# lmb-freiburg/locov

Measured on AMD Instinct MI355X. Metric: proposals/sec through LSM ROI-head (1333x800, 1000 prop, 1203-class text bank), higher is better.
Workload: dtype f32 (Res5 GEMM products formed from f16x2 split operands on the f16 matrix pipe, f32 accumulate; error vs f64 <= 1.5 x the f32-MFMA kernel's + 6e-7 and <= 3e-6 on every tested shape, tests/test_gpu_split_gemm.py)

## Files before the change

### include/locov_hip.h

```cpp
#ifndef LOCOV_HIP_H
#define LOCOV_HIP_H

#include <stdint.h>

#ifdef __cplusplus
extern "C" {
#endif

#define LOCOV_ABI_VERSION 8

#define LOCOV_OK 0
#define LOCOV_ERR_INVALID_ARG (-1)
#define LOCOV_ERR_LAUNCH (-2)
#define LOCOV_ERR_UNSUPPORTED (-3)

#define LOCOV_F32 0
#define LOCOV_BF16 1

#define LOCOV_NORM_NONE 0
#define LOCOV_NORM_L2 1
#define LOCOV_NORM_STANDARDIZE 2

#define LOCOV_EPI_RELU 1u
#define LOCOV_GEMM_A_SPLIT 0x1000u
// ... 45 lines not shown
int64_t locov_roi_align_plan_bytes(int64_t R);
int locov_roi_align_from_nhwc_fwd_ex(const float *feat_nhwc, int N, int H, int W, int C,
                                     const float *rois, int64_t R, int pooled_h, int pooled_w,
                                     float spatial_scale, int sampling_ratio, int aligned, int mode,
                                     void *workspace, int64_t workspace_bytes, float *out,
                                     locov_stream_t stream);

int locov_roi_align_nhwc_fwd(const void *feat, int feat_dtype, int N, int H, int W, int C,
                             const float *rois, int64_t R, int pooled_h, int pooled_w,
                             float spatial_scale, int sampling_ratio, int aligned,
                             int bin_stride, int pos_major, void *out, int out_dtype,
                             locov_stream_t stream);

int locov_roi_align_nhwc_ld_fwd(const void *feat, int feat_dtype, int N, int H, int W, int C,
                                const float *rois, int64_t R, int pooled_h, int pooled_w,
                                float spatial_scale, int sampling_ratio, int aligned,
                                int bin_stride, int pos_major, void *out, int64_t out_ld,
                                int out_dtype, locov_stream_t stream);

int locov_roi_align_nhwc_affine_fwd(const void *feat, int feat_dtype, int N, int H, int W, int C,
                                    int64_t feat_ld, const float *rois, int64_t R, int pooled_h,
                                    int pooled_w, float spatial_scale, int sampling_ratio,
                                    int aligned, int bin_stride, int pos_major,
                                    const float *ch_scale, const float *ch_shift, int relu,
                                    void *out, int64_t out_ld, int out_dtype,
                                    locov_stream_t stream);

int locov_spatial_mean_fwd(const float *x, int64_t R, int C, int HW, int channels_last,
                           float *out, locov_stream_t stream);

int locov_gemm_nt_f32(const float *x, int64_t lda, const float *W, const float *scale,
                      const float *shift, const float *residual, float *y, int64_t ldc,
                      int64_t M, int N, int K, unsigned flags, locov_stream_t stream);

int locov_conv3x3_nhwc_f32(const float *x, int64_t R, int H, int W, int Cin, int pos_major,
                           const float *w_packed, const float *scale, const float *shift,
                           const float *residual, float *y, int N, unsigned flags,
                           locov_stream_t stream);

int locov_pack_conv3x3_weight(const float *w, int N, int Cin, void *out, int out_dtype,
                              locov_stream_t stream);

int64_t locov_winograd_workspace_bytes(int64_t R, int Cin, int N);

int locov_winograd_pack_weight(const float *w, int N, int Cin, float *U, locov_stream_t stream);

int locov_winograd_conv3x3_f32(const float *x, int64_t R, int Cin, const float *U,
                               const float *scale, const float *shift, float *y, int64_t ldy,
                               int N, unsigned flags, void *workspace, int64_t workspace_bytes,
                               locov_stream_t stream);

int locov_winograd_conv3x3_f32_split(const float *x, int64_t R, int Cin, const void *U_split,
                                     float u_scale, float v_scale, const float *scale,
                                     const float *shift, float *y, int64_t ldy, int N, unsigned flags,
                                     void *workspace, int64_t workspace_bytes, unsigned *overflow,
                                     locov_stream_t stream);

int locov_gemm_nt_batched_f32(const float *x, int64_t lda, int64_t stride_x, const float *W,
                              int64_t stride_w, float *y, int64_t ldc, int64_t stride_y,
                              int64_t M, int N, int K, int batch, locov_stream_t stream);

int locov_token_attention_fwd(const float *sim, int64_t R, int Ttot, const int *tok_off,
                              const int *num_tok, int K1, int Tmax, float temperature,
                              int cosine, int hardmax, const float *gmin, float *scores,
                              float *att, locov_stream_t stream);

int locov_token_attention_bwd(const float *sim, int64_t R, int Ttot, const int *tok_off,
                              const int *num_tok, int K1, int Tmax, float temperature,
                              int cosine, int hardmax, const float *gmin, const float *grad_scores,
                              const float *grad_att, float *grad_sim, locov_stream_t stream);

int locov_gemm_nt_bf16(const uint16_t *x, int64_t lda, const uint16_t *W, const float *scale,
                       const float *shift, const float *residual, float *y, int64_t ldc,
                       int64_t M, int N, int K, unsigned flags, locov_stream_t stream);

int locov_conv3x3_nhwc_bf16(const uint16_t *x, int64_t R, int H, int W, int Cin, int pos_major,
                            const uint16_t *w_packed, const float *scale, const float *shift,
                            const float *residual, float *y, int N, unsigned flags,
                            locov_stream_t stream);

int locov_split_f16x2_pack(const float *w, int64_t rows, int K, int64_t ld, float w_scale, void *out,
                           unsigned *overflow, locov_stream_t stream);

int locov_gemm_nt_f32_split(const float *x, int64_t lda, const void *W_split, const float *scale,
                            const float *shift, const float *residual, float *y, int64_t ldc,
                            int64_t M, int N, int K, unsigned flags, float x_scale, float w_scale,
                            unsigned *overflow, locov_stream_t stream);

int locov_gemm_segmean_supported(int64_t lda, int64_t M, int N, int K, int seg, unsigned flags);
int64_t locov_gemm_segmean_workspace_bytes(int64_t M, int N);
int locov_gemm_nt_f32_split_segmean(const float *x, int64_t lda, const void *W_split, const float *scale,
                                    const float *shift, const float *residual, float *out, int64_t M,
                                    int N, int K, int seg, unsigned flags, float x_scale, float w_scale,
                                    void *workspace, int64_t workspace_bytes, unsigned *overflow,
                                    locov_stream_t stream);

int locov_gemm_nt_batched_f32_split(const float *x, int64_t lda, int64_t stride_x, const void *W_split,
                                    int64_t stride_w, float *y, int64_t ldc, int64_t stride_y,
                                    int64_t M, int N, int K, int batch, float x_scale, float w_scale,
                                    unsigned *overflow, locov_stream_t stream);

int locov_gemm_timing_enable(int on);
int locov_gemm_timing_read(int cls, int64_t *launches, double *ms, double *flops);
int locov_gemm_timing_read_ex(int cls, int64_t *launches, double *ms, double *flops, double *bytes);

int locov_frozen_bn_fold(const float *weight, const float *bias, const float *running_mean,
                         const float *running_var, float eps, int C, float *scale, float *shift,
                         locov_stream_t stream);

int locov_rownorm_fwd(const float *x, int64_t R, int D, int mode, float eps, float *y,
                      locov_stream_t stream);

int locov_rownorm_bwd(const float *x, const float *grad_y, int64_t R, int D, int mode, float eps,
                      float *grad_x, locov_stream_t stream);

int locov_f32_to_bf16(const float *x, int64_t n, uint16_t *y, locov_stream_t stream);

int locov_sim_gemm_bf16(const uint16_t *emb, const uint16_t *bank, int64_t R, int D, int K1,
                        float *logits, int64_t ldc, locov_stream_t stream);

#define LOCOV_LABEL_MAX_IMAGES 64
#define LOCOV_LABEL_MAX_THRESHOLDS 6
int locov_label_proposals(const float *boxes, const int *prop_offsets, const float *gt_boxes, const int64_t *gt_classes,
                          const int *gt_offsets, int n_images, const float *thr_lo, const float *thr_hi, const int *thr_label,
                          int n_thresholds, int64_t num_classes, const double *rnd, int64_t *gt_index, int64_t *labels,
                          double *key_pos, double *key_neg, int64_t *rows, locov_stream_t stream);

int locov_sample_proposals(const double *key_pos, const double *key_neg, const int64_t *labels, const int64_t *gt_index,
                           const int64_t *rows, const float *boxes, const float *gt_boxes, const float *field,
                           const int *prop_offsets, const int *gt_offsets, int n_images, int budget, int max_pos,
                           int64_t num_classes, int64_t *picked, float *out_boxes, int64_t *out_classes, float *out_gt_boxes,
                           int64_t *out_fg, float *rois, float *field_out, locov_stream_t stream);

int locov_box_reg_loss(const float *proposal_boxes, const float *gt_boxes, const float *pred_deltas, int64_t ld,
                       const int64_t *gt_classes, int64_t R, int64_t num_classes, float wx, float wy, float ww, float wh,
                       float smooth_l1_beta, float *loss, float *dpred, locov_stream_t stream);

int64_t locov_nms_workspace_bytes(int64_t K);

int locov_nms_sorted(const float *boxes_sorted, int64_t K, float iou_threshold, void *workspace,
                     unsigned char *keep, int *num_keep, locov_stream_t stream);

#define LOCOV_DETECT_MAX_CANDIDATES 8192
#define LOCOV_DETECT_FLAG_NONFINITE 1
#define LOCOV_DETECT_FLAG_OVERFLOW 2
int64_t locov_detect_postprocess_workspace_bytes(int64_t R, int n_images);

int locov_detect_postprocess(const float *probs, int64_t ld_probs, int num_classes, const float *deltas, const float *proposal_boxes,
                             const int *row_offsets, const float *image_hw, int n_images, float wx, float wy, float ww, float wh,
                             float scale_clamp, float score_thresh, float nms_thresh, int topk, void *workspace, int64_t workspace_bytes,
                             float *out_boxes, float *out_scores, int64_t *out_classes, int64_t *out_rows, int *counts_and_flags,
                             locov_stream_t stream);

int64_t locov_detect_postprocess_wide_workspace_bytes(const int *row_offsets, int n_images, int num_classes, int per_class_above);

int locov_detect_postprocess_wide(const float *probs, int64_t ld_probs, int num_classes, const float *deltas, const float *proposal_boxes,
                                  const int *row_offsets, const float *image_hw, int n_images, float wx, float wy, float ww, float wh,
                                  float scale_clamp, float score_thresh, float nms_thresh, int topk, int per_class_above, void *workspace,
                                  int64_t workspace_bytes, float *out_boxes, float *out_scores, int64_t *out_classes, int64_t *out_rows,
                                  int *counts_and_flags, locov_stream_t stream);

int locov_grounding_fwd(const float *S, int B, int T, int NR, const float *caption_mask,
                        const float *region_mask, float temperature, float *cost_w2r,
                        float *cost_r2w, locov_stream_t stream);

int locov_grounding_bwd(const float *S, int B, int T, int NR, const float *caption_mask,
                        const float *region_mask, float temperature, const float *grad_w2r,
                        const float *grad_r2w, float *grad_S, locov_stream_t stream);

#define LOCOV_GROUNDING_CE_MAX_B 64
int locov_grounding_ce_fwd(const float *cost_w2r, const float *cost_r2w, const float *caption_mask, const float *region_mask, int B,
                           int T, int NR, float *out8, locov_stream_t stream);
int locov_grounding_ce_bwd(const float *cost_w2r, const float *cost_r2w, const float *caption_mask, const float *region_mask, int B,
                           int T, int NR, const float *g_w2r_caption, const float *g_w2r_image, const float *g_r2w_caption,
                           const float *g_r2w_image, float *dcost_w2r, float *dcost_r2w, locov_stream_t stream);

int locov_grounding_ce_dist_fwd(const float *cost_w2r, const float *cost_r2w, const float *caption_mask, const float *region_mask, int B,
                                int T, int NR, float *out8, float *pw_w2r, float *pw_r2w, locov_stream_t stream);
int locov_grounding_ce_dist_bwd(const float *cost_w2r, const float *cost_r2w, const float *caption_mask, const float *region_mask, int B,
                                int T, int NR, const float *g_w2r_caption, const float *g_w2r_image, const float *g_r2w_caption,
                                const float *g_r2w_image, const float *g_pw_w2r, const float *g_pw_r2w, float *dcost_w2r, float *dcost_r2w,
                                locov_stream_t stream);

#define LOCOV_DISTILL_KD 0
#define LOCOV_DISTILL_JS 1
#define LOCOV_DISTILL_MSE 2
#define LOCOV_DISTILL_MAX_B 64
int locov_distill_loss_fwd(const float *trans, const float *w2r, const float *r2w, int B, int kind, int transformer_teacher,
                           float temperature, float loss_weight, float *loss, locov_stream_t stream);
int locov_distill_loss_bwd(const float *trans, const float *w2r, const float *r2w, int B, int kind, int transformer_teacher,
                           float temperature, float loss_weight, const float *grad_loss, float *grad_trans, float *grad_w2r,
                           float *grad_r2w, locov_stream_t stream);

int64_t locov_pool_fc_bwd_workspace_bytes(int64_t R, int C5, int D);
int locov_pool_fc_bwd(const float *x, int64_t R, int C5, const float *emb_w, int D, const float *bbox_w,
                      const float *grad_emb, const float *grad_deltas, float *grad_x, float *grad_emb_w,
                      float *grad_emb_b, float *grad_bbox_w, float *grad_bbox_b, void *workspace,
                      int64_t workspace_bytes, locov_stream_t stream);
int64_t locov_sim_gemm_bwd_workspace_bytes(int64_t R, int D, int K1);
int locov_sim_gemm_bwd(const float *grad_logits, const float *emb, const float *bank, int64_t R, int D, int K1,
                       float *grad_emb, float *grad_bank, void *workspace, int64_t workspace_bytes,
                       locov_stream_t stream);

int locov_box_head_fwd(const float *x, int64_t R, int C5, int HW, int channels_last,
                       const float *emb_w, const float *emb_b, const float *bbox_w,
                       const float *bbox_b, const float *bank, const uint16_t *bank_bf16,
                       int D, int K1, int norm_mode, int sim_dtype, float *pooled,
                       float *deltas, float *emb, uint16_t *emb_bf16, float *logits,
                       locov_stream_t stream);

int locov_gemm_nt_f32_ex(const float *x, int64_t lda, const float *W, int64_t ldb, const float *scale,
                         const float *shift, const float *residual, const float *mask, float *y, int64_t ldc,
                         int64_t M, int N, int K, unsigned flags, locov_stream_t stream);

int locov_conv3x3_nhwc_f32_ex(const float *x, int64_t R, int H, int W, int Cin, int pos_major,
                              const float *w_packed, const float *scale, const float *shift,
                              const float *residual, const float *mask, float *y, int N, unsigned flags,
                              locov_stream_t stream);

int locov_winograd_conv3x3_f32_ex(const float *x, int64_t R, int Cin, const float *U, const float *scale,
                                  const float *shift, const float *mask, float *y, int64_t ldy, int N,
                                  unsigned flags, void *workspace, int64_t workspace_bytes,
                                  locov_stream_t stream);

int64_t locov_gemm_tn_workspace_bytes(int64_t M, int N, int K, int batch);
int locov_gemm_tn_f32(const float *a, int64_t lda, int64_t stride_a, const float *b, int64_t ldb,
                      int64_t stride_b, float *out, int64_t ldo, int64_t stride_o, int64_t M, int N, int K,
                      int batch, const float *row_scale, void *workspace, int64_t workspace_bytes,
                      locov_stream_t stream);

int locov_split_scale_from_amax(const float *x, int64_t n, float target_log2, float *scale_out,
                                locov_stream_t stream);
#define LOCOV_AMAX_BOUND_MAX 4
int locov_amax_bound(const float *const *xs, const int64_t *ns, const float *muls, int count, float *slot,
                     locov_stream_t stream);
int locov_split_scale_from_amax_zeroed(const float *x, int64_t n, float target_log2, float *scale_out,
                                       locov_stream_t stream);
int locov_gemm_nt_f32_split_ex(const float *x, int64_t lda, const void *W_split, const float *scale,
                               const float *shift, const float *residual, const float *mask, float *y,
                               int64_t ldc, int64_t M, int N, int K, unsigned flags, float x_scale,
                               const float *x_scale_dev, float w_scale, unsigned *overflow,
                               float *amax_out, locov_stream_t stream);
int locov_gemm_tn_f32_split(const float *a, int64_t lda, int64_t stride_a, const float *b, int64_t ldb,
                            int64_t stride_b, float *out, int64_t ldo, int64_t stride_o, int64_t M, int N,
                            int K, int batch, const float *row_scale, const float *a_scale_dev,
                            float b_scale, unsigned *overflow, void *workspace, int64_t workspace_bytes,
                            locov_stream_t stream);
int locov_winograd_conv3x3_f32_split_ex(const float *x, int64_t R, int Cin, const void *U_split, float u_scale,
                                        float v_scale, int v_scale_auto, const float *scale, const float *shift,
                                        const float *mask, float *y, int64_t ldy, int N, unsigned flags,
                                        float y_split_scale, void *workspace, int64_t workspace_bytes,
                                        unsigned *overflow, float *amax_out, locov_stream_t stream);
int locov_winograd_wgrad_f32_split(const float *x, const float *g, int64_t R, int Cin, int N, unsigned flags,
                                   const float *row_scale, float *dw, unsigned *overflow, void *workspace,
                                   int64_t workspace_bytes, locov_stream_t stream);
int locov_winograd_wgrad_f32_split_v(const float *v_split, const float *g, int64_t R, int Cin, int N, unsigned flags,
                                     const float *row_scale, float *dw, unsigned *overflow, void *workspace,
                                     int64_t workspace_bytes, locov_stream_t stream);
int locov_gemm_tn_f32_split_b(const float *a, int64_t lda, int64_t stride_a, const float *b_split, int64_t ldb,
                              int64_t stride_b, float *out, int64_t ldo, int64_t stride_o, int64_t M, int N,
                              int K, int batch, const float *row_scale, const float *a_scale_dev,
                              float b_scale, unsigned *overflow, void *workspace, int64_t workspace_bytes,
                              locov_stream_t stream);
int64_t locov_conv1x1_winograd_workspace_bytes(int64_t R, int C, int N);
int64_t locov_conv1x1_winograd_workspace_bytes_for(int64_t R, int K, int C, int N, int64_t ldx);
int64_t locov_roi_align_winograd_workspace_bytes(int64_t R, int C, int N);
int locov_roi_align_winograd_conv3x3_f32_split(const float *feat_nhwc, int Nimg, int H, int W, int C, int64_t feat_ld,
                                               const float *rois, int64_t R, int pooled, float spatial_scale,
                                               int sampling_ratio, int aligned, const float *scale1, const float *shift1,
                                               const void *U_split, float u_scale, float v_scale, const float *scale2,
                                               const float *shift2, float *y, int64_t ldy, int N, unsigned flags,
                                               float y_split_scale, void *workspace, int64_t workspace_bytes,
                                               unsigned *overflow, locov_stream_t stream);
int locov_conv1x1_winograd_conv3x3_f32_split(const float *x_split, int64_t ldx, int K, float x_scale, const void *W1_split,
                                             float w1_scale, const float *scale1, const float *shift1, int64_t R, int C,
                                             const void *U_split, float u_scale, float v_scale, const float *scale2,
                                             const float *shift2, float *y, int64_t ldy, int N, unsigned flags,
                                             float y_split_scale, void *workspace, int64_t workspace_bytes,
                                             unsigned *overflow, locov_stream_t stream);

int64_t locov_winograd_wgrad_workspace_bytes(int64_t R, int Cin, int N);
int locov_winograd_wgrad_f32(const float *x, const float *g, int64_t R, int Cin, int N, unsigned flags,
                             const float *row_scale, float *dw, void *workspace, int64_t workspace_bytes,
                             locov_stream_t stream);

#define LOCOV_WEIGHT_PREP_MAX_JOBS 32
enum {
    LOCOV_PREP_PLAIN = 0,
    LOCOV_PREP_TRANSPOSE = 1,
    LOCOV_PREP_IM2COL = 2,
    LOCOV_PREP_IM2COL_FLIP = 3,
    LOCOV_PREP_WINO = 4,
    LOCOV_PREP_WINO_FLIP = 5
};
typedef struct locov_weight_prep_job {
    const float *w;
    const float *row_scale;
    void *out;
    float scale;
    int kind, N, K;
} locov_weight_prep_job;
int locov_res5_weight_prep(const locov_weight_prep_job *jobs, int n_jobs, unsigned *overflow, locov_stream_t stream);

int locov_weight_transpose_scale(const float *w, int N, int K, const float *row_scale, float *out,
                                 locov_stream_t stream);
int locov_conv3x3_weight_flip(const float *w, int N, int Cin, const float *row_scale, float *out,
                              locov_stream_t stream);
int locov_im2col3x3_nhwc(const float *x, int64_t R, int H, int W, int C, float *col, locov_stream_t stream);
int locov_conv3x3_wgrad_unpack(const float *dw_packed, int N, int Cin, const float *row_scale, float *dw,
                               locov_stream_t stream);
int locov_relu_mask(const float *g, const float *act, int64_t n, float *out, float *amax_out, locov_stream_t stream);
#define LOCOV_ZERO_LIST_MAX 24
int locov_zero_if_raised(float *const *tensors, const int64_t *counts, int n_tensors, const unsigned *flag,
                         locov_stream_t stream);

int locov_spatial_mean_bwd(const float *g, const float *act, int64_t R, int C, int HW, float *out,
                           float *amax_out, locov_stream_t stream);
int locov_rows_stride2(const float *src, int N, int H, int W, int C, int forward, float *dst,
                       locov_stream_t stream);
int locov_roi_align_nhwc_bwd(const float *grad_rows, int64_t grad_ld, int N, int H, int W, int C,
                             const float *rois, int64_t R, int pooled_h, int pooled_w, float spatial_scale,
                             int sampling_ratio, int aligned, int bin_stride, int pos_major, float *grad_feat,
                             locov_stream_t stream);

#define LOCOV_REGIONS_MAX_B 64
#define LOCOV_REGIONS_MAX_CANDIDATES 4096
#define LOCOV_REGIONS_GRID 0
#define LOCOV_REGIONS_GRID_ALL 1
#define LOCOV_REGIONS_BOXES 2
#define LOCOV_REGIONS_ROWS 0
#define LOCOV_REGIONS_NCHW 1
int locov_regions_select(const double *keys, int mode, int B, const int *count_host, const int *ext_a_host,
                         const int *ext_b_host, int grid_w, const float *const *boxes_host, int n, int limit, int mask_w,
                         int mvm_w, int64_t *indices, int *src_row, int *inv, uint8_t *mask, float *loc, float *mvm,
                         locov_stream_t stream);
int locov_regions_gather_fwd(const float *src, int layout, int64_t ld, int B, int n, int C, int64_t hw, const int *src_row,
                             float *out, locov_stream_t stream);
int locov_regions_gather_bwd(const float *grad_out, int layout, int64_t ld, int64_t rows, int C, int64_t hw, const int *inv,
                             float *grad_src, locov_stream_t stream);

#ifdef __cplusplus
}
#endif
#endif
```

### locov_amd/_lib.py

```python
from __future__ import annotations

import ctypes
import os
from ctypes import c_char_p, c_float, c_int, c_int64, c_uint, c_void_p, POINTER

HERE = os.path.dirname(os.path.abspath(__file__))
LIB_PATH = os.environ.get("LOCOV_HIP_LIB") or os.path.join(HERE, "liblocov_hip.so")

OK = 0
F32, BF16 = 0, 1
NORM_NONE, NORM_L2, NORM_STANDARDIZE = 0, 1, 2
EPI_RELU = 1
WINO_OUT_ROI_MAJOR = 0x100
WINO_IN_ROI_MAJOR = 0x200
SEGMEAN_RES_ROI_MAJOR = 0x400
GEMM_A_SPLIT = 0x1000
EPI_OUT_SPLIT = 0x2000
EPI_RES_SPLIT = 0x4000
MAX_LEVELS = 8
ZERO_LIST_MAX = 24
LABEL_MAX_IMAGES, LABEL_MAX_THRESHOLDS, SAMPLE_MAX_PROPOSALS = 64, 6, 4096
ABI_VERSION = 8
DETECT_MAX_CANDIDATES, DETECT_FLAG_NONFINITE, DETECT_FLAG_OVERFLOW = 8192, 1, 2
DISTILL_KD, DISTILL_JS, DISTILL_MSE, DISTILL_MAX_B = 0, 1, 2, 64
REGIONS_MAX_B, REGIONS_MAX_CANDIDATES = 64, 4096
REGIONS_GRID, REGIONS_GRID_ALL, REGIONS_BOXES = 0, 1, 2
REGIONS_ROWS, REGIONS_NCHW = 0, 1

_p = c_void_p

WEIGHT_PREP_MAX_JOBS = 32
AMAX_BOUND_MAX = 4
PREP_PLAIN, PREP_TRANSPOSE, PREP_IM2COL, PREP_IM2COL_FLIP, PREP_WINO, PREP_WINO_FLIP = range(6)


class WeightPrepJob(ctypes.Structure):
    _fields_ = [("w", c_void_p), ("row_scale", c_void_p), ("out", c_void_p), ("scale", c_float), ("kind", c_int), ("N", c_int), ("K", c_int)]


SIGNATURES = {
    "locov_abi_version": (c_int, []),
    "locov_last_error": (c_char_p, []),
    "locov_launch_count": (c_int64, []),
    "locov_device_info": (c_int, [POINTER(c_int), POINTER(c_int), POINTER(c_int)]),
    "locov_level_assign": (c_int, [_p, c_int64, c_int, c_int, c_int, c_int, _p, _p]),
    "locov_roi_align_fwd": (c_int, [_p, c_int, c_int, c_int, c_int, _p, c_int64, c_int, c_int, c_float,
                                    c_int, c_int, _p, _p]),
    "locov_roi_align_bwd": (c_int, [_p, c_int, c_int, c_int, c_int, _p, c_int64, c_int, c_int, c_float,
                                    c_int, c_int, _p, _p]),
    "locov_roi_align_levels_fwd": (c_int, [POINTER(c_void_p), POINTER(c_int), POINTER(c_int), POINTER(c_float),
                                           c_int, c_int, c_int, _p, _p, c_int64, c_int, c_int, c_int, c_int,
                                           _p, _p]),
    "locov_nchw_to_nhwc": (c_int, [_p, c_int, c_int, c_int, c_int, _p, c_int, _p]),
    "locov_roi_align_nhwc_fwd": (c_int, [_p, c_int, c_int, c_int, c_int, c_int, _p, c_int64, c_int, c_int,
                                         c_float, c_int, c_int, c_int, c_int, _p, c_int, _p]),
    "locov_roi_align_nhwc_ld_fwd": (c_int, [_p, c_int, c_int, c_int, c_int, c_int, _p, c_int64, c_int, c_int,
                                            c_float, c_int, c_int, c_int, c_int, _p, c_int64, c_int, _p]),
    "locov_roi_align_nhwc_affine_fwd": (c_int, [_p, c_int, c_int, c_int, c_int, c_int, c_int64, _p, c_int64, c_int, c_int,
                                                c_float, c_int, c_int, c_int, c_int, _p, _p, c_int, _p, c_int64, c_int, _p]),
    "locov_roi_align_from_nhwc_fwd": (c_int, [_p, c_int, c_int, c_int, c_int, _p, c_int64, c_int, c_int, c_float,
                                              c_int, c_int, _p, _p]),
    "locov_roi_align_plan_bytes": (c_int64, [c_int64]),
    "locov_roi_align_from_nhwc_fwd_ex": (c_int, [_p, c_int, c_int, c_int, c_int, _p, c_int64, c_int, c_int, c_float,
                                                 c_int, c_int, c_int, _p, c_int64, _p, _p]),
    "locov_spatial_mean_fwd": (c_int, [_p, c_int64, c_int, c_int, c_int, _p, _p]),
    "locov_gemm_nt_f32": (c_int, [_p, c_int64, _p, _p, _p, _p, _p, c_int64, c_int64, c_int, c_int, c_uint, _p]),
    "locov_conv3x3_nhwc_f32": (c_int, [_p, c_int64, c_int, c_int, c_int, c_int, _p, _p, _p, _p, _p, c_int, c_uint,
                                       _p]),
    "locov_pack_conv3x3_weight": (c_int, [_p, c_int, c_int, _p, c_int, _p]),
    "locov_winograd_workspace_bytes": (c_int64, [c_int64, c_int, c_int]),
    "locov_winograd_pack_weight": (c_int, [_p, c_int, c_int, _p, _p]),
    "locov_winograd_conv3x3_f32": (c_int, [_p, c_int64, c_int, _p, _p, _p, _p, c_int64, c_int, c_uint, _p, c_int64, _p]),
    "locov_winograd_conv3x3_f32_split": (c_int, [_p, c_int64, c_int, _p, c_float, c_float, _p, _p, _p, c_int64, c_int, c_uint,
                                                 _p, c_int64, _p, _p]),
    "locov_gemm_nt_batched_f32": (c_int, [_p, c_int64, c_int64, _p, c_int64, _p, c_int64, c_int64, c_int64, c_int,
                                          c_int, c_int, _p]),
    "locov_gemm_timing_enable": (c_int, [c_int]),
    "locov_gemm_timing_read": (c_int, [c_int, _p, _p, _p]),
    "locov_gemm_timing_read_ex": (c_int, [c_int, _p, _p, _p, _p]),
    "locov_frozen_bn_fold": (c_int, [_p, _p, _p, _p, c_float, c_int, _p, _p, _p]),
    "locov_label_proposals": (c_int, [_p, POINTER(c_int), _p, _p, POINTER(c_int), c_int, POINTER(c_float), POINTER(c_float),
                                      POINTER(c_int), c_int, c_int64, _p, _p, _p, _p, _p, _p, _p]),
    "locov_sample_proposals": (c_int, [_p, _p, _p, _p, _p, _p, _p, _p, POINTER(c_int), POINTER(c_int), c_int, c_int, c_int, c_int64,
                                       _p, _p, _p, _p, _p, _p, _p, _p]),
    "locov_box_reg_loss": (c_int, [_p, _p, _p, c_int64, _p, c_int64, c_int64, c_float, c_float, c_float, c_float, c_float, _p, _p, _p]),
    "locov_grounding_ce_fwd": (c_int, [_p, _p, _p, _p, c_int, c_int, c_int, _p, _p]),
    "locov_grounding_ce_bwd": (c_int, [_p, _p, _p, _p, c_int, c_int, c_int, _p, _p, _p, _p, _p, _p, _p]),
    "locov_grounding_ce_dist_fwd": (c_int, [_p, _p, _p, _p, c_int, c_int, c_int, _p, _p, _p, _p]),
    "locov_grounding_ce_dist_bwd": (c_int, [_p, _p, _p, _p, c_int, c_int, c_int, _p, _p, _p, _p, _p, _p, _p, _p, _p]),
    "locov_distill_loss_fwd": (c_int, [_p, _p, _p, c_int, c_int, c_int, c_float, c_float, _p, _p]),
    "locov_distill_loss_bwd": (c_int, [_p, _p, _p, c_int, c_int, c_int, c_float, c_float, _p, _p, _p, _p, _p]),
    "locov_nms_workspace_bytes": (c_int64, [c_int64]),
    "locov_nms_sorted": (c_int, [_p, c_int64, c_float, _p, _p, _p, _p]),
    "locov_detect_postprocess_workspace_bytes": (c_int64, [c_int64, c_int]),
    "locov_detect_postprocess": (c_int, [_p, c_int64, c_int, _p, _p, POINTER(c_int), POINTER(c_float), c_int, c_float, c_float, c_float,
                                         c_float, c_float, c_float, c_float, c_int, _p, c_int64, _p, _p, _p, _p, _p, _p]),
    "locov_detect_postprocess_wide_workspace_bytes": (c_int64, [POINTER(c_int), c_int, c_int, c_int]),
    "locov_detect_postprocess_wide": (c_int, [_p, c_int64, c_int, _p, _p, POINTER(c_int), POINTER(c_float), c_int, c_float, c_float, c_float,
                                              c_float, c_float, c_float, c_float, c_int, c_int, _p, c_int64, _p, _p, _p, _p, _p, _p]),
    "locov_grounding_fwd": (c_int, [_p, c_int, c_int, c_int, _p, _p, c_float, _p, _p, _p]),
    "locov_grounding_bwd": (c_int, [_p, c_int, c_int, c_int, _p, _p, c_float, _p, _p, _p, _p]),
    "locov_token_attention_fwd": (c_int, [_p, c_int64, c_int, _p, _p, c_int, c_int, c_float, c_int, c_int, _p, _p, _p, _p]),
    "locov_token_attention_bwd": (c_int, [_p, c_int64, c_int, _p, _p, c_int, c_int, c_float, c_int, c_int, _p, _p, _p, _p, _p]),
    "locov_rownorm_fwd": (c_int, [_p, c_int64, c_int, c_int, c_float, _p, _p]),
    "locov_rownorm_bwd": (c_int, [_p, _p, c_int64, c_int, c_int, c_float, _p, _p]),
    "locov_pool_fc_bwd_workspace_bytes": (c_int64, [c_int64, c_int, c_int]),
    "locov_pool_fc_bwd": (c_int, [_p, c_int64, c_int, _p, c_int, _p, _p, _p, _p, _p, _p, _p, _p, _p, c_int64, _p]),
    "locov_sim_gemm_bwd_workspace_bytes": (c_int64, [c_int64, c_int, c_int]),
    "locov_sim_gemm_bwd": (c_int, [_p, _p, _p, c_int64, c_int, c_int, _p, _p, _p, c_int64, _p]),
    "locov_f32_to_bf16": (c_int, [_p, c_int64, _p, _p]),
    "locov_gemm_nt_bf16": (c_int, [_p, c_int64, _p, _p, _p, _p, _p, c_int64, c_int64, c_int, c_int, c_uint, _p]),
    "locov_conv3x3_nhwc_bf16": (c_int, [_p, c_int64, c_int, c_int, c_int, c_int, _p, _p, _p, _p, _p, c_int, c_uint, _p]),
    "locov_split_f16x2_pack": (c_int, [_p, c_int64, c_int, c_int64, c_float, _p, _p, _p]),
    "locov_gemm_nt_f32_split": (c_int, [_p, c_int64, _p, _p, _p, _p, _p, c_int64, c_int64, c_int, c_int, c_uint, c_float,
                                        c_float, _p, _p]),
    "locov_gemm_segmean_supported": (c_int, [c_int64, c_int64, c_int, c_int, c_int, c_uint]),
    "locov_gemm_segmean_workspace_bytes": (c_int64, [c_int64, c_int]),
    "locov_gemm_nt_f32_split_segmean": (c_int, [_p, c_int64, _p, _p, _p, _p, _p, c_int64, c_int, c_int, c_int, c_uint, c_float,
                                                c_float, _p, c_int64, _p, _p]),
    "locov_gemm_nt_batched_f32_split": (c_int, [_p, c_int64, c_int64, _p, c_int64, _p, c_int64, c_int64, c_int64, c_int,
                                                c_int, c_int, c_float, c_float, _p, _p]),
    "locov_sim_gemm_bf16": (c_int, [_p, _p, c_int64, c_int, c_int, _p, c_int64, _p]),
    "locov_gemm_nt_f32_ex": (c_int, [_p, c_int64, _p, c_int64, _p, _p, _p, _p, _p, c_int64, c_int64, c_int, c_int, c_uint, _p]),
    "locov_conv3x3_nhwc_f32_ex": (c_int, [_p, c_int64, c_int, c_int, c_int, c_int, _p, _p, _p, _p, _p, _p, c_int, c_uint, _p]),
    "locov_winograd_conv3x3_f32_ex": (c_int, [_p, c_int64, c_int, _p, _p, _p, _p, _p, c_int64, c_int, c_uint, _p, c_int64, _p]),
    "locov_gemm_tn_workspace_bytes": (c_int64, [c_int64, c_int, c_int, c_int]),
    "locov_gemm_tn_f32": (c_int, [_p, c_int64, c_int64, _p, c_int64, c_int64, _p, c_int64, c_int64, c_int64, c_int, c_int, c_int,
                                  _p, _p, c_int64, _p]),
    "locov_split_scale_from_amax": (c_int, [_p, c_int64, c_float, _p, _p]),
    "locov_amax_bound": (c_int, [POINTER(c_void_p), POINTER(c_int64), POINTER(c_float), c_int, _p, _p]),
    "locov_split_scale_from_amax_zeroed": (c_int, [_p, c_int64, c_float, _p, _p]),
    "locov_gemm_nt_f32_split_ex": (c_int, [_p, c_int64, _p, _p, _p, _p, _p, _p, c_int64, c_int64, c_int, c_int, c_uint, c_float, _p,
                                           c_float, _p, _p, _p]),
    "locov_gemm_tn_f32_split": (c_int, [_p, c_int64, c_int64, _p, c_int64, c_int64, _p, c_int64, c_int64, c_int64, c_int, c_int, c_int,
                                        _p, _p, c_float, _p, _p, c_int64, _p]),
    "locov_gemm_tn_f32_split_b": (c_int, [_p, c_int64, c_int64, _p, c_int64, c_int64, _p, c_int64, c_int64, c_int64, c_int, c_int, c_int,
                                        _p, _p, c_float, _p, _p, c_int64, _p]),
    "locov_winograd_conv3x3_f32_split_ex": (c_int, [_p, c_int64, c_int, _p, c_float, c_float, c_int, _p, _p, _p, _p, c_int64, c_int,
                                                    c_uint, c_float, _p, c_int64, _p, _p, _p]),
    "locov_winograd_wgrad_f32_split": (c_int, [_p, _p, c_int64, c_int, c_int, c_uint, _p, _p, _p, _p, c_int64, _p]),
    "locov_winograd_wgrad_f32_split_v": (c_int, [_p, _p, c_int64, c_int, c_int, c_uint, _p, _p, _p, _p, c_int64, _p]),
    "locov_conv1x1_winograd_workspace_bytes": (c_int64, [c_int64, c_int, c_int]),
    "locov_conv1x1_winograd_workspace_bytes_for": (c_int64, [c_int64, c_int, c_int, c_int, c_int64]),
    "locov_roi_align_winograd_workspace_bytes": (c_int64, [c_int64, c_int, c_int]),
    "locov_roi_align_winograd_conv3x3_f32_split": (c_int, [_p, c_int, c_int, c_int, c_int, c_int64, _p, c_int64, c_int, c_float, c_int, c_int,
                                                           _p, _p, _p, c_float, c_float, _p, _p, _p, c_int64, c_int, c_uint, c_float, _p, c_int64,
                                                           _p, _p]),
    "locov_conv1x1_winograd_conv3x3_f32_split": (c_int, [_p, c_int64, c_int, c_float, _p, c_float, _p, _p, c_int64, c_int, _p, c_float, c_float,
                                                         _p, _p, _p, c_int64, c_int, c_uint, c_float, _p, c_int64, _p, _p]),
    "locov_winograd_wgrad_workspace_bytes": (c_int64, [c_int64, c_int, c_int]),
    "locov_winograd_wgrad_f32": (c_int, [_p, _p, c_int64, c_int, c_int, c_uint, _p, _p, _p, c_int64, _p]),
    "locov_res5_weight_prep": (c_int, [POINTER(WeightPrepJob), c_int, _p, _p]),
    "locov_weight_transpose_scale": (c_int, [_p, c_int, c_int, _p, _p, _p]),
    "locov_conv3x3_weight_flip": (c_int, [_p, c_int, c_int, _p, _p, _p]),
    "locov_im2col3x3_nhwc": (c_int, [_p, c_int64, c_int, c_int, c_int, _p, _p]),
    "locov_conv3x3_wgrad_unpack": (c_int, [_p, c_int, c_int, _p, _p, _p]),
    "locov_relu_mask": (c_int, [_p, _p, c_int64, _p, _p, _p]),
    "locov_zero_if_raised": (c_int, [POINTER(c_void_p), POINTER(c_int64), c_int, _p, _p]),
    "locov_spatial_mean_bwd": (c_int, [_p, _p, c_int64, c_int, c_int, _p, _p, _p]),
    "locov_rows_stride2": (c_int, [_p, c_int, c_int, c_int, c_int, c_int, _p, _p]),
    "locov_roi_align_nhwc_bwd": (c_int, [_p, c_int64, c_int, c_int, c_int, c_int, _p, c_int64, c_int, c_int, c_float, c_int, c_int,
                                         c_int, c_int, _p, _p]),
    "locov_box_head_fwd": (c_int, [_p, c_int64, c_int, c_int, c_int, _p, _p, _p, _p, _p, _p, c_int, c_int,
                                   c_int, c_int, _p, _p, _p, _p, _p, _p]),
    "locov_regions_select": (c_int, [_p, c_int, c_int, POINTER(c_int), POINTER(c_int), POINTER(c_int), c_int, POINTER(c_void_p), c_int, c_int,
                                     c_int, c_int, _p, _p, _p, _p, _p, _p, _p]),
    "locov_regions_gather_fwd": (c_int, [_p, c_int, c_int64, c_int, c_int, c_int, c_int64, _p, _p, _p]),
    "locov_regions_gather_bwd": (c_int, [_p, c_int, c_int64, c_int64, c_int, c_int64, _p, _p, _p]),
}

_lib = None


class LocovError(RuntimeError):
    pass


def load() -> ctypes.CDLL:
    global _lib
    if _lib is not None:
        return _lib
    if not os.path.exists(LIB_PATH):
        raise LocovError(
            f"{LIB_PATH} not found: build it with `python -m locov_amd.build` "
            "(or __graft_entry__.build()).  The LSM ROI-head path has no fallback.")
    lib = ctypes.CDLL(LIB_PATH)
    for name, (restype, argtypes) in SIGNATURES.items():
        try:
            fn = getattr(lib, name)
        except AttributeError as e:
            raise LocovError(f"{LIB_PATH} does not export {name}") from e
        fn.restype = restype
        fn.argtypes = argtypes
    if lib.locov_abi_version() != ABI_VERSION:
        raise LocovError(f"ABI version mismatch: library {lib.locov_abi_version()} != binding {ABI_VERSION}")
    _lib = lib
    return lib


def check(rc: int, what: str = "") -> None:
    if rc != OK:
        msg = load().locov_last_error()
        raise LocovError(f"{what or 'liblocov_hip'} failed (code {rc}): {msg.decode() if msg else ''}")
```

### locov_amd/csrc/gemm_nt.h

```cpp
#pragma once
#include "common.h"

namespace locov {

struct Epilogue {
    const float *scale;
    const float *shift;
    const float *residual;
    unsigned flags;
    const float *mask;
    float *amax_out;
};

__device__ __forceinline__ void split_scale_of(const float *slot, float &s, float &inv)
{
    s = slot[0];
    inv = slot[1];
    if (s == 0.f) {
        const float amax = __uint_as_float(reinterpret_cast<const unsigned *>(slot)[2]);
        s = 1.f;
        if (amax > 0.f && amax < 3.0e38f) {
            int e;
            frexpf(amax, &e);
            s = ldexpf(1.f, 13 - e);
        }
        inv = 1.f / s;
    }
}

__device__ __forceinline__ void amax_fold(float *slot, float m)
{
#pragma unroll
    for (int o = 32; o > 0; o >>= 1) m = fmaxf(m, __shfl_xor(m, o));
    if ((threadIdx.x & 63) == 0 && m > 0.f) {
        unsigned *w = reinterpret_cast<unsigned *>(slot) + 2;
        const unsigned bits = __float_as_uint(m);
        if (bits > __hip_atomic_load(w, __ATOMIC_RELAXED, __HIP_MEMORY_SCOPE_AGENT)) atomicMax(w, bits);
    }
}

struct ConvGeom {
    int H, W, Cin, R, group;
};

struct Batch {
    int count;
    int64_t sa, sb, sc;
};

template <typename T, typename TOut>
int launch_gemm_nt(const T *A, int64_t lda, const T *B, int64_t ldb, TOut *C, int64_t ldc, int64_t M, int N, int K,
                   const Epilogue &epi, hipStream_t s, const char *what, const ConvGeom &cg = ConvGeom{0, 0, 0, 0, 0},
                   const Batch &bt = Batch{1, 0, 0, 0});

int timing_begin(hipStream_t s, int cls, double flops, double bytes = 0.0);
void timing_end(int idx, hipStream_t s);

int launch_gemm_split(const float *A, int64_t lda, const void *Wsplit, float *C, int64_t ldc, int64_t M, int N, int K,
                      const Epilogue &epi, float a_scale, float w_scale, hipStream_t s, const char *what,
                      const Batch &bt = Batch{1, 0, 0, 0}, unsigned *overflow = nullptr, const float *a_scale_dev = nullptr);

bool gemm_split_big_applicable(int64_t lda, int64_t ldc, int64_t M, int N, int K, const Epilogue &epi, const Batch &bt,
                               const float *a_scale_dev);
int launch_gemm_split_big(const float *A, int64_t lda, const void *Wsplit, float *C, int64_t ldc, int64_t M, int N, int K,
                          const Epilogue &epi, float a_scale, float w_scale, hipStream_t s, const char *what, const Batch &bt,
                          unsigned *overflow);

bool gemm_split_big_segmean_applicable(int64_t lda, int64_t M, int N, int K, const Epilogue &epi, int seg);
int64_t gemm_split_big_segmean_workspace_bytes(int64_t M, int N);
int launch_gemm_split_big_segmean(const float *A, int64_t lda, const void *Wsplit, int64_t M, int N, int K, const Epilogue &epi, int seg,
                                  float a_scale, float w_scale, float *partial, float *out, hipStream_t s, const char *what, unsigned *overflow);

bool gemm_split_big_wino_applicable(int64_t lda, int64_t M, int N, int K, const Epilogue &epi);
int launch_gemm_split_big_wino(const float *A, int64_t lda, const void *Wsplit, int64_t M, int N, int K, const Epilogue &epi, float a_scale,
                               float w_scale, float *V, float v_scale, hipStream_t s, const char *what, unsigned *overflow);

bool roi_align_nhwc_wino_applicable(int C, int64_t R);
int launch_roi_align_nhwc_wino(const float *feat, int N, int H, int W, int C, int64_t feat_ld, const float *rois, int64_t R, int pooled,
                               float spatial_scale, int sampling_ratio, int aligned, const float *ch_scale, const float *ch_shift, int relu,
                               float *V, float v_scale, unsigned *overflow, hipStream_t s);

int launch_gemm_tn(const float *A, int64_t lda, int64_t sa, const float *B, int64_t ldb, int64_t sb, float *out, int64_t ldo,
                   int64_t so, int64_t M, int N, int K, int batch, const float *row_scale, float *ws, int64_t ws_bytes,
                   hipStream_t s, const char *what);
int64_t gemm_tn_workspace_bytes(int64_t M, int N, int K, int batch);
int launch_gemm_tn_split(const float *A, int64_t lda, int64_t sa, const float *B, int64_t ldb, int64_t sb, float *out, int64_t ldo,
                         int64_t so, int64_t M, int N, int K, int batch, const float *row_scale, const float *a_scale_dev, float b_scale,
                         unsigned *overflow, float *ws, int64_t ws_bytes, hipStream_t s, const char *what, bool b_split = false);

}
```

### locov_amd/csrc/gemm_tn.hip

```cpp
#include "gemm_nt.h"

#include <cstdlib>

namespace locov {

namespace {

typedef float f32x16 __attribute__((ext_vector_type(16)));
typedef float f32x4 __attribute__((ext_vector_type(4)));

constexpr int TBM = 128, TBN = 128, TBK = 32, TNT = 256;
constexpr int PITCH = TBM + 32;
constexpr int TSTAGE = 2 * TBK * PITCH;

__device__ __forceinline__ int tn_xcd_remap(int bid, int nwg)
{
    const int xcd = bid & 7, q = nwg >> 3, r = nwg & 7;
    const int base = xcd < r ? xcd * (q + 1) : r * (q + 1) + (xcd - r) * q;
    return base + (bid >> 3);
}

}

__global__ __launch_bounds__(TNT, 2) void gemm_tn_kernel(const float *__restrict__ A, int64_t lda, const float *__restrict__ B,
                                                         int64_t ldb, float *__restrict__ P, int64_t M, int N, int K,
                                                         int splits, int64_t m_chunk, int64_t sa, int64_t sb)
{
    __shared__ f32x4 lds4[2 * TSTAGE / 4];
    float *const lds = reinterpret_cast<float *>(lds4);

    const int tiles_n = (N + TBM - 1) / TBM, tiles_k = (K + TBN - 1) / TBN, tiles = tiles_n * tiles_k;
    int wg = tn_xcd_remap(blockIdx.x, gridDim.x);
    const int bs = wg / tiles;
    wg -= bs * tiles;
    const int b = bs / splits, s = bs - b * splits;
    const int n0 = (wg / tiles_k) * TBM, k0 = (wg % tiles_k) * TBN;
    const int64_t m_lo = (int64_t)s * m_chunk;
    const int64_t rows = M - m_lo < m_chunk ? M - m_lo : m_chunk;
    const char *a_base = reinterpret_cast<const char *>(A + b * sa + m_lo * lda);
    const char *b_base = reinterpret_cast<const char *>(B + b * sb + m_lo * ldb);
    int64_t a_left = rows * lda * 4, b_left = rows * ldb * 4;

    const int tid = threadIdx.x, lane = tid & 63, wave = tid >> 6;
    const int wm = (wave >> 1) * 64, wn = (wave & 1) * 64;

    unsigned a_off[4], b_off[4];
    int s_off[4];
#pragma unroll
    for (int i = 0; i < 4; i++) {
        const int idx = tid + i * TNT, row = idx >> 5, ch = idx & 31;
        int ca = n0 + ch * 4, cb = k0 + ch * 4;
        ca = ca + 4 <= N ? ca : N - 4;
        cb = cb + 4 <= K ? cb : K - 4;
        a_off[i] = (unsigned)(((int64_t)row * lda + ca) * 4);
        b_off[i] = (unsigned)(((int64_t)row * ldb + cb) * 4);
        s_off[i] = row * PITCH + ch * 4;
    }
    f32x4 ra[4], rb[4];
    auto load = [&]() {
        const unsigned na = a_left > 0 ? (unsigned)a_left : 0u, nb = b_left > 0 ? (unsigned)b_left : 0u;
        const __amdgpu_buffer_rsrc_t r_a = __builtin_amdgcn_make_buffer_rsrc(const_cast<char *>(a_base), 0, na, 0x00020000);
        const __amdgpu_buffer_rsrc_t r_b = __builtin_amdgcn_make_buffer_rsrc(const_cast<char *>(b_base), 0, nb, 0x00020000);
#pragma unroll
        for (int i = 0; i < 4; i++) ra[i] = __builtin_bit_cast(f32x4, __builtin_amdgcn_raw_buffer_load_b128(r_a, a_off[i], 0, 0));
#pragma unroll
        for (int i = 0; i < 4; i++) rb[i] = __builtin_bit_cast(f32x4, __builtin_amdgcn_raw_buffer_load_b128(r_b, b_off[i], 0, 0));
        a_base += (int64_t)TBK * lda * 4;
        b_base += (int64_t)TBK * ldb * 4;
        a_left -= (int64_t)TBK * lda * 4;
        b_left -= (int64_t)TBK * ldb * 4;
    };
    auto store = [&](int stage) {
        float *As = lds + stage * TSTAGE, *Bs = As + TBK * PITCH;
#pragma unroll
        for (int i = 0; i < 4; i++) *reinterpret_cast<f32x4 *>(As + s_off[i]) = ra[i];
#pragma unroll
        for (int i = 0; i < 4; i++) *reinterpret_cast<f32x4 *>(Bs + s_off[i]) = rb[i];
    };

    f32x16 acc[2][2];
#pragma unroll
    for (int i = 0; i < 2; i++)
#pragma unroll
        for (int j = 0; j < 2; j++) acc[i][j] = f32x16{};

    const int fr = lane & 31, fh = lane >> 5;
    auto compute = [&](int stage) {
        const float *As = lds + stage * TSTAGE + fh * PITCH + wm + fr;
        const float *Bs = lds + stage * TSTAGE + TBK * PITCH + fh * PITCH + wn + fr;
#pragma unroll
        for (int kk = 0; kk < TBK / 2; kk++) {
            const float a0 = As[2 * kk * PITCH], a1 = As[2 * kk * PITCH + 32];
            const float b0 = Bs[2 * kk * PITCH], b1 = Bs[2 * kk * PITCH + 32];
            acc[0][0] = __builtin_amdgcn_mfma_f32_32x32x2f32(a0, b0, acc[0][0], 0, 0, 0);
            acc[0][1] = __builtin_amdgcn_mfma_f32_32x32x2f32(a0, b1, acc[0][1], 0, 0, 0);
            acc[1][0] = __builtin_amdgcn_mfma_f32_32x32x2f32(a1, b0, acc[1][0], 0, 0, 0);
            acc[1][1] = __builtin_amdgcn_mfma_f32_32x32x2f32(a1, b1, acc[1][1], 0, 0, 0);
        }
    };

    const int steps = (int)((rows + TBK - 1) / TBK);
    load();
    store(0);
    if (steps > 1) load();
    __syncthreads();
    for (int t = 0; t < steps; t++) {
        const int st = t & 1;
        compute(st);
        if (t + 1 < steps) {
            store(st ^ 1);
            if (t + 2 < steps) load();
        }
        __syncthreads();
    }

    float *out = P + (int64_t)bs * N * K;
#pragma unroll
    for (int i = 0; i < 2; i++)
#pragma unroll
        for (int j = 0; j < 2; j++) {
            const int kc = k0 + wn + j * 32 + fr;
#pragma unroll
            for (int r = 0; r < 16; r++) {
                const int n = n0 + wm + i * 32 + (r & 3) + 8 * (r >> 2) + 4 * fh;
                if (n < N && kc < K) out[(int64_t)n * K + kc] = acc[i][j][r];
            }
        }
}

__global__ __launch_bounds__(256) void gemm_tn_reduce_kernel(const float *__restrict__ P, int N, int K, int splits, int batch,
                                                             const float *__restrict__ row_scale, float *__restrict__ out,
                                                             int64_t ldo, int64_t so)
{
    const int k4 = K >> 2;
    const int64_t per = (int64_t)N * k4, total = per * batch;
    for (int64_t i = (int64_t)blockIdx.x * blockDim.x + threadIdx.x; i < total; i += (int64_t)gridDim.x * blockDim.x) {
        const int64_t b = i / per, rem = i - b * per;
        const int n = (int)(rem / k4), k = (int)(rem - (int64_t)n * k4) * 4;
        f32x4 a = {0.f, 0.f, 0.f, 0.f};
        const float *p = P + (b * splits) * (int64_t)N * K + (int64_t)n * K + k;
        for (int s = 0; s < splits; s++) a += *reinterpret_cast<const f32x4 *>(p + (int64_t)s * N * K);
        if (row_scale) a *= row_scale[n];
        *reinterpret_cast<f32x4 *>(out + b * so + (int64_t)n * ldo + k) = a;
    }
}

void tn_split_plan(int64_t M, int N, int K, int batch, int *splits, int64_t *m_chunk)
{
    const int64_t tiles = ceil_div(N, TBM) * ceil_div(K, TBN) * batch;
    static const int64_t target = [] { const char *e = getenv("LOCOV_TN_WGS"); return e && atoll(e) > 0 ? (int64_t)atoll(e) : (int64_t)1024; }();
    int64_t s = ceil_div(target, tiles);
    const int64_t smax = ceil_div(M, 256);
    if (s > smax) s = smax;
    if (s < 1) s = 1;
    int64_t mc = ceil_div(ceil_div(M, s), TBK) * TBK;
    *m_chunk = mc;
    *splits = (int)ceil_div(M, mc);
}

int launch_tn_reduce(const float *ws, int N, int K, int splits, int batch, const float *row_scale, float *out, int64_t ldo, int64_t so,
                     hipStream_t s, const char *what)
{
    const int64_t total = (int64_t)batch * N * (K / 4);
    const unsigned blocks = (unsigned)(ceil_div(total, 256) < 8192 ? ceil_div(total, 256) : 8192);
    hipLaunchKernelGGL(gemm_tn_reduce_kernel, dim3(blocks), dim3(256), 0, s, ws, N, K, splits, batch, row_scale, out, ldo, so);
    return check_launch(what);
}

int launch_gemm_tn(const float *A, int64_t lda, int64_t sa, const float *B, int64_t ldb, int64_t sb, float *out, int64_t ldo,
                   int64_t so, int64_t M, int N, int K, int batch, const float *row_scale, float *ws, int64_t ws_bytes,
                   hipStream_t s, const char *what)
{
    int splits;
    int64_t m_chunk;
    tn_split_plan(M, N, K, batch, &splits, &m_chunk);
    const int64_t need = (int64_t)batch * splits * N * K * 4;
    if (ws_bytes < need) return set_error(LOCOV_ERR_INVALID_ARG, "%s: workspace too small (%lld < %lld bytes)", what, (long long)ws_bytes, (long long)need);
    if (N % 4 || K % 4 || lda % 4 || ldb % 4 || ldo % 4 || so % 4 || sa % 4 || sb % 4 || N < 4 || K < 4)
        return set_error(LOCOV_ERR_UNSUPPORTED, "%s: N, K, the row pitches and the batch strides must be multiples of 4", what);
    if (((uintptr_t)A | (uintptr_t)B | (uintptr_t)out | (uintptr_t)ws) % 16)
        return set_error(LOCOV_ERR_UNSUPPORTED, "%s: pointers must be 16-byte aligned", what);
    if ((m_chunk + TBK) * (lda > ldb ? lda : ldb) * 4 > 0x7fffffffLL)
        return set_error(LOCOV_ERR_INVALID_ARG, "%s: row pitch too large for 32-bit chunk offsets", what);
    const int64_t wgs = ceil_div(N, TBM) * ceil_div(K, TBN) * splits * batch;
    if (wgs > 0x7fffffffLL) return set_error(LOCOV_ERR_INVALID_ARG, "%s: problem too large", what);
    const bool direct = splits == 1 && row_scale == nullptr && ldo == K && (batch == 1 || so == (int64_t)N * K);
    const int trec = timing_begin(s, 6, 2.0 * (double)M * N * K * batch);
    hipLaunchKernelGGL(gemm_tn_kernel, dim3((unsigned)wgs), dim3(TNT), 0, s, A, lda, B, ldb, direct ? out : ws, M, N, K, splits, m_chunk, sa, sb);
    timing_end(trec, s);
    int rc = check_launch(what);
    if (rc || direct) return rc;
    return launch_tn_reduce(ws, N, K, splits, batch, row_scale, out, ldo, so, s, what);
}

int64_t gemm_tn_workspace_bytes(int64_t M, int N, int K, int batch)
{
    if (M <= 0 || N <= 0 || K <= 0 || batch <= 0) return 0;
    int splits;
    int64_t m_chunk;
    tn_split_plan(M, N, K, batch, &splits, &m_chunk);
    return (int64_t)batch * splits * N * K * 4;
}

}

using namespace locov;

extern "C" {

int64_t locov_gemm_tn_workspace_bytes(int64_t M, int N, int K, int batch) { return gemm_tn_workspace_bytes(M, N, K, batch); }

int locov_gemm_tn_f32(const float *a, int64_t lda, int64_t stride_a, const float *b, int64_t ldb, int64_t stride_b, float *out,
                      int64_t ldo, int64_t stride_o, int64_t M, int N, int K, int batch, const float *row_scale, void *workspace,
                      int64_t workspace_bytes, locov_stream_t stream)
{
    LOCOV_REQUIRE(M >= 0 && N > 0 && K > 0 && batch > 0, "locov_gemm_tn_f32: bad shape M=%lld N=%d K=%d batch=%d", (long long)M, N, K, batch);
    LOCOV_REQUIRE(out, "locov_gemm_tn_f32: null output");
    LOCOV_REQUIRE(lda >= N && ldb >= K && ldo >= K, "locov_gemm_tn_f32: lda < N, ldb < K or ldo < K");
    if (M == 0) {
        for (int bi = 0; bi < batch; bi++) {
            hipError_t e = hipMemset2DAsync(out + bi * stride_o, (size_t)ldo * 4, 0, (size_t)K * 4, (size_t)N, as_stream(stream));
            if (e != hipSuccess) return set_error(LOCOV_ERR_LAUNCH, "locov_gemm_tn_f32: memset failed: %s", hipGetErrorString(e));
        }
        return LOCOV_OK;
    }
    LOCOV_REQUIRE(a && b && workspace, "locov_gemm_tn_f32: null pointer");
    return launch_gemm_tn(a, lda, stride_a, b, ldb, stride_b, out, ldo, stride_o, M, N, K, batch, row_scale,
                          static_cast<float *>(workspace), workspace_bytes, as_stream(stream), "locov_gemm_tn_f32");
}

}
```

### locov_amd/csrc/gemm_tn_split.hip

```cpp
#include "gemm_nt.h"

namespace locov {

namespace {

typedef float f32x4 __attribute__((ext_vector_type(4)));
typedef _Float16 f16x8 __attribute__((ext_vector_type(8)));
typedef unsigned u32x4 __attribute__((ext_vector_type(4)));
typedef unsigned u32x2 __attribute__((ext_vector_type(2)));

constexpr int SBM = 128, SBN = 128, SBK = 32, SNT = 256;
constexpr int SROWB = 128;
constexpr int SSTAGEB = (SBM + SBN) * SROWB;

__device__ __forceinline__ int swz(int row) { return (int)((0x75642031u >> (4 * ((row >> 1) & 7))) & 7u); }

__device__ __forceinline__ int tns_xcd_remap(int bid, int nwg)
{
    const int xcd = bid & 7, q = nwg >> 3, r = nwg & 7;
    const int base = xcd < r ? xcd * (q + 1) : r * (q + 1) + (xcd - r) * q;
    return base + (bid >> 3);
}

__device__ __forceinline__ void split2(float x0, float x1, float s, unsigned &hi, unsigned &lo)
{
    unsigned h, l;
    asm("v_fma_mixlo_f16 %0, %1, %2, 0" : "=v"(h) : "v"(x0), "v"(s));
    asm("v_fma_mixhi_f16 %0, %1, %2, 0" : "+v"(h) : "v"(x1), "v"(s));
    asm("v_fma_mixlo_f16 %0, %1, %2, -%3 op_sel_hi:[0,0,1]" : "=v"(l) : "v"(x0), "v"(s), "v"(h));
    asm("v_fma_mixhi_f16 %0, %1, %2, -%3 op_sel:[0,0,1] op_sel_hi:[0,0,1]" : "+v"(l) : "v"(x1), "v"(s), "v"(h));
    hi = h;
    lo = l;
}

}

template <bool B_SPLIT>
__global__ __launch_bounds__(SNT, 2) void gemm_tn_split_kernel(const float *__restrict__ A, int64_t lda, const float *__restrict__ B,
                                                               int64_t ldb, float *__restrict__ P, int64_t M, int N, int K,
                                                               int splits, int64_t m_chunk, int64_t sa, int64_t sb,
                                                               const float *__restrict__ a_scale_dev, float b_scale,
                                                               unsigned *overflow)
{
    __shared__ u32x4 lds[2 * SSTAGEB / 16];
    char *const ldsb = reinterpret_cast<char *>(lds);

    const int tiles_n = (N + SBM - 1) / SBM, tiles_k = (K + SBN - 1) / SBN, tiles = tiles_n * tiles_k;
    int wg = tns_xcd_remap(blockIdx.x, gridDim.x);
    const int bs = wg / tiles;
    wg -= bs * tiles;
    const int b = bs / splits, s = bs - b * splits;
    const int n0 = (wg / tiles_k) * SBM, k0 = (wg % tiles_k) * SBN;
    const int64_t m_lo = (int64_t)s * m_chunk;
    const int64_t rows = M - m_lo < m_chunk ? M - m_lo : m_chunk;

    const int tid = threadIdx.x, lane = tid & 63, wave = tid >> 6;
    const int wm = (wave >> 1) * 64, wn = (wave & 1) * 64;
    float a_scale, a_inv;
    split_scale_of(a_scale_dev, a_scale, a_inv);
    const float out_scale = a_inv / b_scale;

    const bool is_a = __builtin_amdgcn_readfirstlane(tid >> 6) < 2;
    const int t = tid & 127, cg = t & 31, mg = t >> 5;
    const int ld = (int)(is_a ? lda : ldb);
    const int ncol = is_a ? N : K, c0 = is_a ? n0 : k0;
    int col = c0 + cg * 4;
    col = col + 4 <= ncol ? col : ncol - 4;
    const char *base = reinterpret_cast<const char *>((is_a ? A + b * sa : B + b * sb) + m_lo * (int64_t)ld);
    int64_t left = rows * (int64_t)ld * 4;
    const bool pre = B_SPLIT && !is_a;
    const unsigned voff = (unsigned)((int64_t)(mg * 8) * ld * 4 + (pre ? (col >> 3) * 32 + (col & 4) * 2 : col * 4));
    const unsigned rstep = (unsigned)ld * 4u;
    const float scale = is_a ? a_scale : b_scale;
    int dst[4][2];
#pragma unroll
    for (int j = 0; j < 4; j++) {
        const int row = cg * 4 + j;
#pragma unroll
        for (int hl = 0; hl < 2; hl++) dst[j][hl] = (is_a ? 0 : SBM * SROWB) + row * SROWB + (((2 * mg + hl) ^ swz(row)) * 16);
    }
    f32x4 r[8];
    float amax = 0.f;
    auto load = [&]() {
        const unsigned nrec = left > 0 ? (unsigned)left : 0u;
        const __amdgpu_buffer_rsrc_t rs = __builtin_amdgcn_make_buffer_rsrc(const_cast<char *>(base), 0, nrec, 0x00020000);
        if (B_SPLIT && pre) {
#pragma unroll
            for (int i = 0; i < 8; i++) {
                const u32x2 h = __builtin_bit_cast(u32x2, __builtin_amdgcn_raw_buffer_load_b64(rs, voff + i * rstep, 0, 0));
                const u32x2 l = __builtin_bit_cast(u32x2, __builtin_amdgcn_raw_buffer_load_b64(rs, voff + i * rstep + 16, 0, 0));
                r[i] = __builtin_bit_cast(f32x4, u32x4{h[0], h[1], l[0], l[1]});
            }
        } else {
#pragma unroll
            for (int i = 0; i < 8; i++) r[i] = __builtin_bit_cast(f32x4, __builtin_amdgcn_raw_buffer_load_b128(rs, voff + i * rstep, 0, 0));
        }
        base += (int64_t)SBK * ld * 4;
        left -= (int64_t)SBK * ld * 4;
    };
    auto store_pre = [&](int stage) {
        char *d = ldsb + stage * SSTAGEB;
#pragma unroll
        for (int j = 0; j < 4; j++) {
            u32x4 hi, lo;
            const unsigned sel = (j & 1) ? 0x07060302u : 0x05040100u;
#pragma unroll
            for (int p = 0; p < 4; p++) {
                const u32x4 e = __builtin_bit_cast(u32x4, r[2 * p]), o = __builtin_bit_cast(u32x4, r[2 * p + 1]);
                hi[p] = __builtin_amdgcn_perm(o[j >> 1], e[j >> 1], sel);
                lo[p] = __builtin_amdgcn_perm(o[2 + (j >> 1)], e[2 + (j >> 1)], sel);
            }
            *reinterpret_cast<u32x4 *>(d + dst[j][0]) = hi;
            *reinterpret_cast<u32x4 *>(d + dst[j][1]) = lo;
        }
    };
    auto store = [&](int stage) {
        char *d = ldsb + stage * SSTAGEB;
#pragma unroll
        for (int j = 0; j < 4; j++) {
            u32x4 hi, lo;
#pragma unroll
            for (int p = 0; p < 4; p++) {
                const float x0 = r[2 * p][j], x1 = r[2 * p + 1][j];
                amax = fmaxf(fmaxf(amax, fabsf(x0)), fabsf(x1));
                unsigned h, l;
                split2(x0, x1, scale, h, l);
                hi[p] = h;
                lo[p] = l;
            }
            *reinterpret_cast<u32x4 *>(d + dst[j][0]) = hi;
            *reinterpret_cast<u32x4 *>(d + dst[j][1]) = lo;
        }
    };

    f32x4 acc[4][4];
#pragma unroll
    for (int i = 0; i < 4; i++)
#pragma unroll
        for (int j = 0; j < 4; j++) acc[i][j] = f32x4{0.f, 0.f, 0.f, 0.f};

    const int l16 = lane & 15, kg = lane >> 4;
    int fo[2];
#pragma unroll
    for (int hl = 0; hl < 2; hl++) fo[hl] = l16 * SROWB + (((2 * kg + hl) ^ swz(l16)) * 16);
    auto compute = [&](int stage) {
        const char *As = ldsb + stage * SSTAGEB + wm * SROWB;
        const char *Bs = ldsb + stage * SSTAGEB + SBM * SROWB + wn * SROWB;
        f16x8 fa[4][2], fb[4][2];
#pragma unroll
        for (int i = 0; i < 4; i++) {
            fa[i][0] = *reinterpret_cast<const f16x8 *>(As + i * 16 * SROWB + fo[0]);
            fa[i][1] = *reinterpret_cast<const f16x8 *>(As + i * 16 * SROWB + fo[1]);
            fb[i][0] = *reinterpret_cast<const f16x8 *>(Bs + i * 16 * SROWB + fo[0]);
            fb[i][1] = *reinterpret_cast<const f16x8 *>(Bs + i * 16 * SROWB + fo[1]);
        }
#pragma unroll
        for (int i = 0; i < 4; i++)
#pragma unroll
            for (int j = 0; j < 4; j++) {
                acc[i][j] = __builtin_amdgcn_mfma_f32_16x16x32_f16(fa[i][0], fb[j][0], acc[i][j], 0, 0, 0);
                acc[i][j] = __builtin_amdgcn_mfma_f32_16x16x32_f16(fa[i][0], fb[j][1], acc[i][j], 0, 0, 0);
                acc[i][j] = __builtin_amdgcn_mfma_f32_16x16x32_f16(fa[i][1], fb[j][0], acc[i][j], 0, 0, 0);
            }
    };

    const int steps = (int)((rows + SBK - 1) / SBK);
    load();
    if (pre)
        store_pre(0);
    else
        store(0);
    if (steps > 1) load();
    __syncthreads();
#ifndef LOCOV_TNS_INTERLEAVE
#define LOCOV_TNS_INTERLEAVE 1
#endif
    int tt = 0;
    if (pre) {
        for (; tt + 2 < steps; tt++) {
            const int st = tt & 1;
            compute(st);
            store_pre(st ^ 1);
            if (LOCOV_TNS_INTERLEAVE) {
#pragma unroll
                for (int i = 0; i < 16; i++) __builtin_amdgcn_sched_group_barrier(0x100, 1, 0);
#pragma unroll
                for (int i = 0; i < 48; i++) {
                    __builtin_amdgcn_sched_group_barrier(0x008, 1, 0);
                    __builtin_amdgcn_sched_group_barrier(0x002, 1, 0);
                }
            }
            load();
            __syncthreads();
        }
        for (; tt < steps; tt++) {
            const int st = tt & 1;
            compute(st);
            if (tt + 1 < steps) store_pre(st ^ 1);
            __syncthreads();
        }
    } else {
    for (; tt + 2 < steps; tt++) {
        const int st = tt & 1;
        compute(st);
        store(st ^ 1);
        if (LOCOV_TNS_INTERLEAVE) {
#pragma unroll
            for (int i = 0; i < 16; i++) __builtin_amdgcn_sched_group_barrier(0x100, 1, 0);
#pragma unroll
            for (int i = 0; i < 48; i++) {
                __builtin_amdgcn_sched_group_barrier(0x008, 1, 0);
                __builtin_amdgcn_sched_group_barrier(0x002, 3, 0);
            }
        }
        load();
        __syncthreads();
    }
    for (; tt < steps; tt++) {
        const int st = tt & 1;
        compute(st);
        if (tt + 1 < steps) store(st ^ 1);
        __syncthreads();
    }
    }
    if (overflow != nullptr && amax * scale >= 65504.f) atomicOr(overflow, 1u);

    float *out = P + (int64_t)bs * N * K;
#pragma unroll
    for (int i = 0; i < 4; i++)
#pragma unroll
        for (int j = 0; j < 4; j++) {
            const int kc = k0 + wn + j * 16 + l16;
#pragma unroll
            for (int rg = 0; rg < 4; rg++) {
                const int n = n0 + wm + i * 16 + 4 * kg + rg;
                if (n < N && kc < K) out[(int64_t)n * K + kc] = acc[i][j][rg] * out_scale;
            }
        }
}

void tn_split_plan(int64_t M, int N, int K, int batch, int *splits, int64_t *m_chunk);
int launch_tn_reduce(const float *ws, int N, int K, int splits, int batch, const float *row_scale, float *out, int64_t ldo, int64_t so,
                     hipStream_t s, const char *what);

int launch_gemm_tn_split(const float *A, int64_t lda, int64_t sa, const float *B, int64_t ldb, int64_t sb, float *out, int64_t ldo,
                         int64_t so, int64_t M, int N, int K, int batch, const float *row_scale, const float *a_scale_dev, float b_scale,
                         unsigned *overflow, float *ws, int64_t ws_bytes, hipStream_t s, const char *what, bool b_split)
{
    int splits;
    int64_t m_chunk;
    tn_split_plan(M, N, K, batch, &splits, &m_chunk);
    const int64_t need = (int64_t)batch * splits * N * K * 4;
    if (ws_bytes < need) return set_error(LOCOV_ERR_INVALID_ARG, "%s: workspace too small (%lld < %lld bytes)", what, (long long)ws_bytes, (long long)need);
    if (N % 4 || K % 4 || lda % 4 || ldb % 4 || ldo % 4 || so % 4 || sa % 4 || sb % 4 || N < 4 || K < 4)
        return set_error(LOCOV_ERR_UNSUPPORTED, "%s: N, K, the row pitches and the batch strides must be multiples of 4", what);
    if (((uintptr_t)A | (uintptr_t)B | (uintptr_t)out | (uintptr_t)ws) % 16)
        return set_error(LOCOV_ERR_UNSUPPORTED, "%s: pointers must be 16-byte aligned", what);
    if (!a_scale_dev || !(b_scale > 0.f)) return set_error(LOCOV_ERR_INVALID_ARG, "%s: operand scales missing", what);
    if ((m_chunk + SBK) * (lda > ldb ? lda : ldb) * 4 > 0x7fffffffLL)
        return set_error(LOCOV_ERR_INVALID_ARG, "%s: row pitch too large for 32-bit chunk offsets", what);
    const int64_t wgs = ceil_div(N, SBM) * ceil_div(K, SBN) * splits * batch;
    if (wgs > 0x7fffffffLL) return set_error(LOCOV_ERR_INVALID_ARG, "%s: problem too large", what);
    const bool direct = splits == 1 && row_scale == nullptr && ldo == K && (batch == 1 || so == (int64_t)N * K);
    const int trec = timing_begin(s, 7, 2.0 * (double)M * N * K * batch);
    if (b_split) {
        if (K % 8 || ldb % 8 || sb % 8) return set_error(LOCOV_ERR_UNSUPPORTED, "%s: a pre-split b needs K, ldb and its batch stride to be multiples of 8", what);
        hipLaunchKernelGGL(gemm_tn_split_kernel<true>, dim3((unsigned)wgs), dim3(SNT), 0, s, A, lda, B, ldb, direct ? out : ws, M, N, K, splits, m_chunk, sa,
                           sb, a_scale_dev, b_scale, overflow);
    } else
        hipLaunchKernelGGL(gemm_tn_split_kernel<false>, dim3((unsigned)wgs), dim3(SNT), 0, s, A, lda, B, ldb, direct ? out : ws, M, N, K, splits, m_chunk, sa,
                           sb, a_scale_dev, b_scale, overflow);
    timing_end(trec, s);
    int rc = check_launch(what);
    if (rc || direct) return rc;
    return launch_tn_reduce(ws, N, K, splits, batch, row_scale, out, ldo, so, s, what);
}

}

using namespace locov;

extern "C" {

int locov_gemm_tn_f32_split(const float *a, int64_t lda, int64_t stride_a, const float *b, int64_t ldb, int64_t stride_b, float *out,
                            int64_t ldo, int64_t stride_o, int64_t M, int N, int K, int batch, const float *row_scale,
                            const float *a_scale_dev, float b_scale, unsigned *overflow, void *workspace, int64_t workspace_bytes,
                            locov_stream_t stream)
{
    LOCOV_REQUIRE(M > 0 && N > 0 && K > 0 && batch > 0, "locov_gemm_tn_f32_split: bad shape M=%lld N=%d K=%d batch=%d", (long long)M, N, K, batch);
    LOCOV_REQUIRE(a && b && out && workspace && a_scale_dev, "locov_gemm_tn_f32_split: null pointer");
    LOCOV_REQUIRE(lda >= N && ldb >= K && ldo >= K, "locov_gemm_tn_f32_split: lda < N, ldb < K or ldo < K");
    return launch_gemm_tn_split(a, lda, stride_a, b, ldb, stride_b, out, ldo, stride_o, M, N, K, batch, row_scale, a_scale_dev, b_scale,
                                overflow, static_cast<float *>(workspace), workspace_bytes, as_stream(stream), "locov_gemm_tn_f32_split", false);
}

int locov_gemm_tn_f32_split_b(const float *a, int64_t lda, int64_t stride_a, const float *b_split, int64_t ldb, int64_t stride_b, float *out,
                              int64_t ldo, int64_t stride_o, int64_t M, int N, int K, int batch, const float *row_scale,
                              const float *a_scale_dev, float b_scale, unsigned *overflow, void *workspace, int64_t workspace_bytes,
                              locov_stream_t stream)
{
    LOCOV_REQUIRE(M > 0 && N > 0 && K > 0 && batch > 0, "locov_gemm_tn_f32_split_b: bad shape M=%lld N=%d K=%d batch=%d", (long long)M, N, K, batch);
    LOCOV_REQUIRE(a && b_split && out && workspace && a_scale_dev, "locov_gemm_tn_f32_split_b: null pointer");
    LOCOV_REQUIRE(lda >= N && ldb >= K && ldo >= K, "locov_gemm_tn_f32_split_b: lda < N, ldb < K or ldo < K");
    return launch_gemm_tn_split(a, lda, stride_a, b_split, ldb, stride_b, out, ldo, stride_o, M, N, K, batch, row_scale, a_scale_dev, b_scale,
                                overflow, static_cast<float *>(workspace), workspace_bytes, as_stream(stream), "locov_gemm_tn_f32_split_b", true);
}

}
```

### locov_amd/csrc/winograd.hip

```cpp
#include "winograd_transform.h"
#include "winograd_filter.h"

#include <cstdlib>

#ifndef LOCOV_WINO_THREADS
#define LOCOV_WINO_THREADS 256
#endif
#ifndef LOCOV_WINO_OUT_MINW
#define LOCOV_WINO_OUT_MINW 1
#endif
#ifndef LOCOV_WINO_IN_MINW
#define LOCOV_WINO_IN_MINW 1
#endif

namespace locov {

using wino::AT;
using wino::BT;
using wino::G;
using wino::NF;

__global__ __launch_bounds__(256) void wino_pack_weight_kernel(const float *__restrict__ w, int64_t NC,
                                                               float *__restrict__ U)
{
// ... 179 lines not shown
        for (int b = 0; b < 3; b++) dw[i * 9 + a * 3 + b] = (float)(sc * g[a][b]);
}

static int64_t chunk_rois(int64_t R, int Cin, int N)
{
    static const int64_t forced = [] {
        const char *e = getenv("LOCOV_WINO_CHUNK");
        return e ? (int64_t)atoll(e) : (int64_t)-1;
    }();
    int64_t c = forced >= 0 ? forced : 0;
    if (c <= 0 || c > R) c = R;
    (void)Cin;
    (void)N;
    return c;
}

}

using namespace locov;

extern "C" {

int64_t locov_winograd_workspace_bytes(int64_t R, int Cin, int N)
{
    if (R <= 0 || Cin <= 0 || N <= 0) return 0;
    const int64_t c = chunk_rois(R, Cin, N);
    return (int64_t)NF * NF * c * ((int64_t)Cin + N) * (int64_t)sizeof(float) + 16;
}

int locov_winograd_pack_weight(const float *w, int N, int Cin, float *U, locov_stream_t stream)
{
    LOCOV_REQUIRE(N > 0 && Cin > 0, "locov_winograd_pack_weight: bad shape");
    LOCOV_REQUIRE(w && U, "locov_winograd_pack_weight: null pointer");
    const int64_t NC = (int64_t)N * Cin;
    hipLaunchKernelGGL(wino_pack_weight_kernel, dim3((unsigned)ceil_div(NC, 256)), dim3(256), 0, as_stream(stream), w, NC, U);
    return check_launch("locov_winograd_pack_weight");
}

struct PreConv {
    const float *x;
    int64_t ldx;
    int K;
    float x_scale;
    const void *W;
    float w_scale;
    const float *scale, *shift;
    float *y1;
};

struct PrePool {
    const float *feat;
    int N, H, W;
    int64_t feat_ld;
    const float *rois;
    int pooled;
    float spatial_scale;
    int sampling_ratio, aligned;
    const float *scale, *shift;
    float *y1;
};

static int winograd_conv3x3(const float *x, int64_t R, int Cin, const float *U, float u_scale, float v_scale,
                            const float *scale, const float *shift, float *y, int64_t ldy, int N, unsigned flags,
                            void *workspace, int64_t workspace_bytes, locov_stream_t stream, const float *mask = nullptr,
                            unsigned *overflow = nullptr, bool v_scale_auto = false, float y_split_scale = 0.f,
                            float *amax_out = nullptr, const PreConv *pre = nullptr, const PrePool *pool = nullptr);

int locov_winograd_conv3x3_f32_ex(const float *x, int64_t R, int Cin, const float *U, const float *scale, const float *shift,
                                  const float *mask, float *y, int64_t ldy, int N, unsigned flags, void *workspace,
                                  int64_t workspace_bytes, locov_stream_t stream)
{
    return winograd_conv3x3(x, R, Cin, U, 0.f, 0.f, scale, shift, y, ldy, N, flags, workspace, workspace_bytes, stream, mask);
}

int locov_winograd_conv3x3_f32_split_ex(const float *x, int64_t R, int Cin, const void *U_split, float u_scale, float v_scale,
                                        int v_scale_auto, const float *scale, const float *shift, const float *mask, float *y,
                                        int64_t ldy, int N, unsigned flags, float y_split_scale, void *workspace,
                                        int64_t workspace_bytes, unsigned *overflow, float *amax_out, locov_stream_t stream)
{
    LOCOV_REQUIRE(u_scale > 0.f && (v_scale_auto || v_scale > 0.f), "locov_winograd_conv3x3_f32_split_ex: operand scales must be positive");
    LOCOV_REQUIRE(!amax_out || !(y_split_scale > 0.f), "locov_winograd_conv3x3_f32_split_ex: amax_out is for an fp32 output");
    return winograd_conv3x3(x, R, Cin, static_cast<const float *>(U_split), u_scale, v_scale_auto ? 1.f : v_scale, scale, shift, y, ldy, N,
                            flags, workspace, workspace_bytes, stream, mask, overflow, v_scale_auto != 0, y_split_scale, amax_out);
}

int locov_winograd_conv3x3_f32(const float *x, int64_t R, int Cin, const float *U, const float *scale,
                               const float *shift, float *y, int64_t ldy, int N, unsigned flags, void *workspace,
                               int64_t workspace_bytes, locov_stream_t stream)
{
    return winograd_conv3x3(x, R, Cin, U, 0.f, 0.f, scale, shift, y, ldy, N, flags, workspace, workspace_bytes, stream);
}

int locov_winograd_conv3x3_f32_split(const float *x, int64_t R, int Cin, const void *U_split, float u_scale, float v_scale,
                                     const float *scale, const float *shift, float *y, int64_t ldy, int N,
                                     unsigned flags, void *workspace, int64_t workspace_bytes, unsigned *overflow,
                                     locov_stream_t stream)
{
    LOCOV_REQUIRE(u_scale > 0.f && v_scale > 0.f, "locov_winograd_conv3x3_f32_split: operand scales must be positive");
    return winograd_conv3x3(x, R, Cin, static_cast<const float *>(U_split), u_scale, v_scale, scale, shift, y, ldy, N, flags,
                            workspace, workspace_bytes, stream, nullptr, overflow);
}

int locov_roi_align_winograd_conv3x3_f32_split(const float *feat_nhwc, int Nimg, int H, int W, int C, int64_t feat_ld, const float *rois,
                                               int64_t R, int pooled, float spatial_scale, int sampling_ratio, int aligned,
                                               const float *scale1, const float *shift1, const void *U_split, float u_scale, float v_scale,
                                               const float *scale2, const float *shift2, float *y, int64_t ldy, int N, unsigned flags,
                                               float y_split_scale, void *workspace, int64_t workspace_bytes, unsigned *overflow,
                                               locov_stream_t stream)
{
    LOCOV_REQUIRE(R >= 0 && Nimg > 0 && H > 0 && W > 0 && C > 0 && N > 0, "locov_roi_align_winograd_conv3x3_f32_split: bad shape");
    if (R == 0) return LOCOV_OK;
    LOCOV_REQUIRE(feat_nhwc && rois && U_split && y && workspace, "locov_roi_align_winograd_conv3x3_f32_split: null pointer");
    LOCOV_REQUIRE(pooled == 14 || pooled == 13, "locov_roi_align_winograd_conv3x3_f32_split: the even bins of the pooler must form a 7 x 7 tile");
    LOCOV_REQUIRE(u_scale > 0.f && v_scale > 0.f && spatial_scale > 0.f, "locov_roi_align_winograd_conv3x3_f32_split: scales must be positive");
    LOCOV_REQUIRE(feat_ld >= C && feat_ld % 4 == 0 && C % 4 == 0 && (uintptr_t)feat_nhwc % 16 == 0 && (int64_t)H * W * feat_ld * 4 < 0xffffffffLL,
                  "locov_roi_align_winograd_conv3x3_f32_split: feat_ld >= C, both %% 4, 16-byte pointer, one image below 4 GiB");
    LOCOV_REQUIRE((flags & LOCOV_WINO_IN_ROI_MAJOR) != 0, "locov_roi_align_winograd_conv3x3_f32_split: rows are ROI-major (LOCOV_WINO_IN_ROI_MAJOR)");
    LOCOV_REQUIRE(chunk_rois(R, C, N) == R, "locov_roi_align_winograd_conv3x3_f32_split: one pass only (LOCOV_WINO_CHUNK is set)");
    const int64_t wb = locov_winograd_workspace_bytes(R, C, N);
    LOCOV_REQUIRE(workspace_bytes >= locov_roi_align_winograd_workspace_bytes(R, C, N),
                  "locov_roi_align_winograd_conv3x3_f32_split: workspace too small (%lld bytes)", (long long)workspace_bytes);
    PrePool pool{feat_nhwc, Nimg, H, W, feat_ld, rois, pooled, spatial_scale, sampling_ratio, aligned, scale1, shift1,
                 reinterpret_cast<float *>(static_cast<char *>(workspace) + ((wb + 15) & ~(int64_t)15))};
    return winograd_conv3x3(nullptr, R, C, static_cast<const float *>(U_split), u_scale, v_scale, scale2, shift2, y, ldy, N, flags, workspace, wb,
                            stream, nullptr, overflow, false, y_split_scale, nullptr, nullptr, &pool);
}

int64_t locov_conv1x1_winograd_workspace_bytes(int64_t R, int C, int N)
{
    if (R <= 0 || C <= 0 || N <= 0) return 0;
    return locov_winograd_workspace_bytes(R, C, N) + R * 49 * (int64_t)C * (int64_t)sizeof(float);
}

static bool conv1x1_wino_fused(int64_t R, int K, int C, int64_t ldx)
{
    return gemm_split_big_wino_applicable(ldx, R * 49, C, K, Epilogue{nullptr, nullptr, nullptr, LOCOV_EPI_RELU | LOCOV_GEMM_A_SPLIT});
}

int64_t locov_conv1x1_winograd_workspace_bytes_for(int64_t R, int K, int C, int N, int64_t ldx)
{
    if (R <= 0 || C <= 0 || N <= 0 || K <= 0) return 0;
    const int64_t wb = locov_winograd_workspace_bytes(R, C, N);
    return chunk_rois(R, C, N) == R && conv1x1_wino_fused(R, K, C, ldx) ? wb : locov_conv1x1_winograd_workspace_bytes(R, C, N);
}

int64_t locov_roi_align_winograd_workspace_bytes(int64_t R, int C, int N)
{
    if (R <= 0 || C <= 0 || N <= 0) return 0;
    const int64_t wb = locov_winograd_workspace_bytes(R, C, N);
    return chunk_rois(R, C, N) == R && roi_align_nhwc_wino_applicable(C, R) ? wb : locov_conv1x1_winograd_workspace_bytes(R, C, N);
}

int locov_conv1x1_winograd_conv3x3_f32_split(const float *x_split, int64_t ldx, int K, float x_scale, const void *W1_split, float w1_scale,
                                             const float *scale1, const float *shift1, int64_t R, int C, const void *U_split,
                                             float u_scale, float v_scale, const float *scale2, const float *shift2, float *y,
                                             int64_t ldy, int N, unsigned flags, float y_split_scale, void *workspace,
                                             int64_t workspace_bytes, unsigned *overflow, locov_stream_t stream)
{
    LOCOV_REQUIRE(R >= 0 && K > 0 && C > 0 && N > 0, "locov_conv1x1_winograd_conv3x3_f32_split: bad shape");
    if (R == 0) return LOCOV_OK;
    LOCOV_REQUIRE(x_split && W1_split && U_split && y && workspace, "locov_conv1x1_winograd_conv3x3_f32_split: null pointer");
    LOCOV_REQUIRE(x_scale > 0.f && w1_scale > 0.f && u_scale > 0.f && v_scale > 0.f,
                  "locov_conv1x1_winograd_conv3x3_f32_split: operand scales must be positive");
    LOCOV_REQUIRE(K % 32 == 0 && ldx >= K && ldx % 4 == 0 && (uintptr_t)x_split % 16 == 0 && (uintptr_t)W1_split % 16 == 0,
                  "locov_conv1x1_winograd_conv3x3_f32_split: K %% 32, ldx >= K, ldx %% 4 and 16-byte pointers required");
    LOCOV_REQUIRE((flags & LOCOV_WINO_IN_ROI_MAJOR) != 0, "locov_conv1x1_winograd_conv3x3_f32_split: rows are ROI-major (LOCOV_WINO_IN_ROI_MAJOR)");
    LOCOV_REQUIRE(chunk_rois(R, C, N) == R, "locov_conv1x1_winograd_conv3x3_f32_split: one pass only (LOCOV_WINO_CHUNK is set)");
    const int64_t wb = locov_winograd_workspace_bytes(R, C, N);
    LOCOV_REQUIRE(workspace_bytes >= locov_conv1x1_winograd_workspace_bytes_for(R, K, C, N, ldx),
                  "locov_conv1x1_winograd_conv3x3_f32_split: workspace too small (%lld bytes)", (long long)workspace_bytes);
    PreConv pre{x_split, ldx, K, x_scale, W1_split, w1_scale, scale1, shift1,
                reinterpret_cast<float *>(static_cast<char *>(workspace) + ((wb + 15) & ~(int64_t)15))};
    return winograd_conv3x3(nullptr, R, C, static_cast<const float *>(U_split), u_scale, v_scale, scale2, shift2, y, ldy, N, flags, workspace, wb,
                            stream, nullptr, overflow, false, y_split_scale, nullptr, &pre);
}

static int winograd_conv3x3(const float *x, int64_t R, int Cin, const float *U, float u_scale, float v_scale,
                            const float *scale, const float *shift, float *y, int64_t ldy, int N, unsigned flags,
                            void *workspace, int64_t workspace_bytes, locov_stream_t stream, const float *mask, unsigned *overflow,
                            bool v_scale_auto, float y_split_scale, float *amax_out, const PreConv *pre, const PrePool *pool)
{
    LOCOV_REQUIRE(ldy >= N && ldy % 2 == 0, "locov_winograd_conv3x3_f32: ldy must be >= N and even");
    LOCOV_REQUIRE(R >= 0 && Cin > 0 && N > 0, "locov_winograd_conv3x3_f32: bad shape");
    if (R == 0) return LOCOV_OK;
    LOCOV_REQUIRE((x || pre || pool) && U && y && workspace, "locov_winograd_conv3x3_f32: null pointer");
    LOCOV_REQUIRE(Cin % 32 == 0 && N % 4 == 0, "locov_winograd_conv3x3_f32: Cin %% 32 and N %% 4 must be 0 (got %d, %d)",
                  Cin, N);
    LOCOV_REQUIRE(((uintptr_t)x | (uintptr_t)U | (uintptr_t)y | (uintptr_t)workspace) % 16 == 0,
                  "locov_winograd_conv3x3_f32: misaligned pointer");
    LOCOV_REQUIRE(!(flags & ~(unsigned)(LOCOV_EPI_RELU | LOCOV_WINO_OUT_ROI_MAJOR | LOCOV_WINO_IN_ROI_MAJOR)),
                  "locov_winograd_conv3x3_f32: unsupported flags 0x%x",
                  flags);
    LOCOV_REQUIRE(!(y_split_scale > 0.f) || (N % 32 == 0 && ldy == N && !mask),
                  "locov_winograd_conv3x3_f32_split: a split-layout output needs N %% 32 == 0, ldy == N and no mask");
    LOCOV_REQUIRE(workspace_bytes >= locov_winograd_workspace_bytes(R, Cin, N),
                  "locov_winograd_conv3x3_f32: workspace too small (%lld bytes)", (long long)workspace_bytes);
    const int64_t chunk = chunk_rois(R, Cin, N);
    float *V = static_cast<float *>(workspace);
    float *Mv = V + (int64_t)NF * NF * chunk * Cin;
    hipStream_t s = as_stream(stream);
    for (int64_t r0 = 0; r0 < R; r0 += chunk) {
        const int64_t rc = R - r0 < chunk ? R - r0 : chunk;
        const int64_t tin = rc * (Cin / 2), tout = rc * (N / 2);
        const bool in_roi_major = (flags & LOCOV_WINO_IN_ROI_MAJOR) != 0;
        const bool v_split = u_scale > 0.f && !v_scale_auto;
        bool v_done = false;
        if (pre) {
            Epilogue e1{pre->scale, pre->shift, nullptr, LOCOV_EPI_RELU | LOCOV_GEMM_A_SPLIT};
            int rc1;
            if (gemm_split_big_wino_applicable(pre->ldx, rc * 49, Cin, pre->K, e1)) {
                rc1 = launch_gemm_split_big_wino(pre->x, pre->ldx, pre->W, rc * 49, Cin, pre->K, e1, pre->x_scale, pre->w_scale, V, v_scale, s,
                                                 "locov_conv1x1_winograd_conv3x3_f32_split (1x1 + input transform)", overflow);
                v_done = true;
            } else {
                rc1 = launch_gemm_split(pre->x, pre->ldx, pre->W, pre->y1, (int64_t)Cin, rc * 49, Cin, pre->K, e1, pre->x_scale, pre->w_scale, s,
                                        "locov_conv1x1_winograd_conv3x3_f32_split (1x1)", Batch{1, 0, 0, 0}, overflow);
                x = pre->y1;
            }
            if (rc1) return rc1;
        }
        if (pool) {
            int rc1;
            if (roi_align_nhwc_wino_applicable(Cin, rc)) {
                rc1 = launch_roi_align_nhwc_wino(pool->feat, pool->N, pool->H, pool->W, Cin, pool->feat_ld, pool->rois, rc, pool->pooled,
                                                 pool->spatial_scale, pool->sampling_ratio, pool->aligned, pool->scale, pool->shift, 1, V, v_scale,
                                                 overflow, s);
                v_done = true;
            } else {
                rc1 = locov_roi_align_nhwc_affine_fwd(pool->feat, LOCOV_F32, pool->N, pool->H, pool->W, Cin, pool->feat_ld, pool->rois, rc,
                                                      pool->pooled, pool->pooled, pool->spatial_scale, pool->sampling_ratio, pool->aligned, 2, 0,
                                                      pool->scale, pool->shift, 1, pool->y1, (int64_t)Cin, LOCOV_F32, stream);
                x = pool->y1;
            }
            if (rc1) return rc1;
        }
        if (v_done)
            ;
        else if (v_split)
            hipLaunchKernelGGL((wino_input_kernel<false, true>), dim3((unsigned)ceil_div(tin, 256)), dim3(256), 0, s,
                               x + r0 * (in_roi_major ? 49 : 1) * Cin, in_roi_major ? (int64_t)1 : R,
                               in_roi_major ? (int64_t)49 : (int64_t)1, rc, Cin, V, v_scale, overflow);
        else {
            float *scw = u_scale > 0.f && v_scale_auto ? reinterpret_cast<float *>(static_cast<char *>(workspace) + workspace_bytes - 16) : nullptr;
            if (scw && hipMemsetAsync(scw, 0, 16, s) != hipSuccess) return set_error(LOCOV_ERR_LAUNCH, "locov_winograd_conv3x3_f32_split: memset failed");
            hipLaunchKernelGGL((wino_input_kernel<false, false>), dim3((unsigned)ceil_div(tin, 256)), dim3(256), 0, s,
                               x + r0 * (in_roi_major ? 49 : 1) * Cin, in_roi_major ? (int64_t)1 : R,
                               in_roi_major ? (int64_t)49 : (int64_t)1, rc, Cin, V, 1.f, static_cast<unsigned *>(nullptr), scw);
        }
        int rcode = check_launch("locov_winograd_conv3x3_f32 (input transform)");
        if (rcode) return rcode;
        Epilogue epi{nullptr, nullptr, nullptr, v_split ? LOCOV_GEMM_A_SPLIT : 0u};
        if (u_scale > 0.f) {
            const float *sc = nullptr;
            if (v_scale_auto)
                sc = reinterpret_cast<float *>(static_cast<char *>(workspace) + workspace_bytes - 16);
            rcode = launch_gemm_split(V, (int64_t)Cin, U, Mv, (int64_t)N, rc, N, Cin, epi, v_scale, u_scale, s,
                                      "locov_winograd_conv3x3_f32_split (batched GEMM)",
                                      Batch{NF * NF, rc * Cin, (int64_t)N * Cin, rc * N}, overflow, sc);
        }
        else
            rcode = launch_gemm_nt<float, float>(V, (int64_t)Cin, U, (int64_t)Cin, Mv, (int64_t)N, rc, N, Cin, epi, s,
                                                 "locov_winograd_conv3x3_f32 (batched GEMM)", ConvGeom{0, 0, 0, 0, 0},
                                                 Batch{NF * NF, rc * Cin, (int64_t)N * Cin, rc * N});
        if (rcode) return rcode;
        const bool roi_major = (flags & LOCOV_WINO_OUT_ROI_MAJOR) != 0;
        const bool wide = (uint64_t)rc * N * 4u * NF > 0xffffffffull ||
                          (uint64_t)(roi_major ? rc : R) * 49u * (uint64_t)ldy * 4u > 0xffffffffull;
        const int64_t lp = roi_major ? (int64_t)1 : R, lr = roi_major ? (int64_t)49 : (int64_t)1;
        float *yo = y + r0 * (roi_major ? 49 : 1) * ldy;
        const float *mo = mask ? mask + r0 * (roi_major ? 49 : 1) * ldy : nullptr;
        const int relu_i = (flags & LOCOV_EPI_RELU) ? 1 : 0;
        const dim3 og((unsigned)ceil_div(tout, 256));
#define LOCOV_WINO_OUT(SP, WD, ...) hipLaunchKernelGGL((wino_output_kernel<SP, WD>), og, dim3(256), 0, s, Mv, lp, lr, rc, N, scale, shift, relu_i, yo, ldy, __VA_ARGS__)
#define LOCOV_WINO_OUT_MASKED(WD, ...) hipLaunchKernelGGL((wino_output_kernel<false, WD, true>), og, dim3(256), 0, s, Mv, lp, lr, rc, N, scale, shift, relu_i, yo, ldy, __VA_ARGS__)
        if (y_split_scale > 0.f) {
            if (wide) LOCOV_WINO_OUT(true, true, static_cast<const float *>(nullptr), y_split_scale, overflow, static_cast<float *>(nullptr));
            else LOCOV_WINO_OUT(true, false, static_cast<const float *>(nullptr), y_split_scale, overflow, static_cast<float *>(nullptr));
        } else if (mo != nullptr) {
            if (wide) LOCOV_WINO_OUT_MASKED(true, mo, 1.f, static_cast<unsigned *>(nullptr), amax_out);
            else LOCOV_WINO_OUT_MASKED(false, mo, 1.f, static_cast<unsigned *>(nullptr), amax_out);
        } else {
            unsigned *const chk = y_split_scale < 0.f ? overflow : nullptr;
            const float chk_scale = y_split_scale < 0.f ? -y_split_scale : 1.f;
            if (wide) LOCOV_WINO_OUT(false, true, mo, chk_scale, chk, amax_out);
            else LOCOV_WINO_OUT(false, false, mo, chk_scale, chk, amax_out);
        }
#undef LOCOV_WINO_OUT_MASKED
#undef LOCOV_WINO_OUT
        rcode = check_launch("locov_winograd_conv3x3_f32 (output transform)");
        if (rcode) return rcode;
    }
    return LOCOV_OK;
}

int64_t locov_winograd_wgrad_workspace_bytes(int64_t R, int Cin, int N)
{
    if (R <= 0 || Cin <= 0 || N <= 0) return 0;
    return (int64_t)NF * NF * (R * ((int64_t)Cin + N) + (int64_t)N * Cin) * (int64_t)sizeof(float) +
           gemm_tn_workspace_bytes(R, N, Cin, NF * NF) + 16;
}

static int winograd_wgrad(const float *x, const float *g, int64_t R, int Cin, int N, unsigned flags, const float *row_scale,
                          float *dw, void *workspace, int64_t workspace_bytes, locov_stream_t stream, bool split, unsigned *overflow,
                          const float *v_split = nullptr);

int locov_winograd_wgrad_f32(const float *x, const float *g, int64_t R, int Cin, int N, unsigned flags, const float *row_scale,
                             float *dw, void *workspace, int64_t workspace_bytes, locov_stream_t stream)
{
    return winograd_wgrad(x, g, R, Cin, N, flags, row_scale, dw, workspace, workspace_bytes, stream, false, nullptr);
}

int locov_winograd_wgrad_f32_split(const float *x, const float *g, int64_t R, int Cin, int N, unsigned flags, const float *row_scale,
                                   float *dw, unsigned *overflow, void *workspace, int64_t workspace_bytes, locov_stream_t stream)
{
    return winograd_wgrad(x, g, R, Cin, N, flags, row_scale, dw, workspace, workspace_bytes, stream, true, overflow);
}

int locov_winograd_wgrad_f32_split_v(const float *v_split, const float *g, int64_t R, int Cin, int N, unsigned flags, const float *row_scale,
                                     float *dw, unsigned *overflow, void *workspace, int64_t workspace_bytes, locov_stream_t stream)
{
    LOCOV_REQUIRE(v_split != nullptr || R == 0, "locov_winograd_wgrad_f32_split_v: null transformed input");
    LOCOV_REQUIRE(Cin % 8 == 0, "locov_winograd_wgrad_f32_split_v: Cin must be a multiple of 8 (got %d)", Cin);
    return winograd_wgrad(v_split, g, R, Cin, N, flags, row_scale, dw, workspace, workspace_bytes, stream, true, overflow, v_split);
}

static int winograd_wgrad(const float *x, const float *g, int64_t R, int Cin, int N, unsigned flags, const float *row_scale,
                          float *dw, void *workspace, int64_t workspace_bytes, locov_stream_t stream, bool split, unsigned *overflow,
                          const float *v_split)
{
    LOCOV_REQUIRE(R >= 0 && Cin > 0 && N > 0, "locov_winograd_wgrad_f32: bad shape");
    LOCOV_REQUIRE(dw, "locov_winograd_wgrad_f32: null output");
    hipStream_t s = as_stream(stream);
    if (R == 0) {
        hipError_t e = hipMemsetAsync(dw, 0, (size_t)N * Cin * 9 * sizeof(float), s);
        return e == hipSuccess ? LOCOV_OK : set_error(LOCOV_ERR_LAUNCH, "locov_winograd_wgrad_f32: memset failed");
    }
    LOCOV_REQUIRE(x && g && workspace, "locov_winograd_wgrad_f32: null pointer");
    LOCOV_REQUIRE(Cin % 4 == 0 && N % 4 == 0, "locov_winograd_wgrad_f32: Cin and N must be multiples of 4 (got %d, %d)", Cin, N);
    LOCOV_REQUIRE(((uintptr_t)x | (uintptr_t)g | (uintptr_t)dw | (uintptr_t)workspace) % 16 == 0, "locov_winograd_wgrad_f32: misaligned pointer");
    LOCOV_REQUIRE(!(flags & ~(unsigned)LOCOV_WINO_IN_ROI_MAJOR), "locov_winograd_wgrad_f32: unsupported flags 0x%x", flags);
    LOCOV_REQUIRE(workspace_bytes >= locov_winograd_wgrad_workspace_bytes(R, Cin, N), "locov_winograd_wgrad_f32: workspace too small (%lld bytes)",
                  (long long)workspace_bytes);
    float *V = static_cast<float *>(workspace);
    float *dM = V + (int64_t)NF * NF * R * Cin;
    float *dU = dM + (int64_t)NF * NF * R * N;
    float *tn_ws = dU + (int64_t)NF * NF * N * Cin;
    const bool rm = (flags & LOCOV_WINO_IN_ROI_MAJOR) != 0;
    const int64_t ld_pos = rm ? 1 : R, ld_roi = rm ? 49 : 1;
    int rc = LOCOV_OK;
    if (v_split == nullptr) {
        hipLaunchKernelGGL(wino_input_kernel<false>, dim3((unsigned)ceil_div(R * (Cin / 2), 256)), dim3(256), 0, s, x, ld_pos, ld_roi, R, Cin, V);
        rc = check_launch("locov_winograd_wgrad_f32 (input transform)");
        if (rc) return rc;
    } else
        LOCOV_REQUIRE((uintptr_t)v_split % 16 == 0, "locov_winograd_wgrad_f32_split_v: misaligned transformed input");
    float *dm_slot = split ? reinterpret_cast<float *>(static_cast<char *>(workspace) + workspace_bytes - 16) : nullptr;
    if (dm_slot && hipMemsetAsync(dm_slot, 0, 16, s) != hipSuccess) return set_error(LOCOV_ERR_LAUNCH, "locov_winograd_wgrad_f32_split: memset failed");
    hipLaunchKernelGGL(wino_input_kernel<true>, dim3((unsigned)ceil_div(R * (N / 2), 256)), dim3(256), 0, s, g, ld_pos, ld_roi, R, N, dM, 1.f,
                       static_cast<unsigned *>(nullptr), dm_slot);
    rc = check_launch("locov_winograd_wgrad_f32 (gradient transform)");
    if (rc) return rc;
    const int64_t tn_bytes = workspace_bytes - (int64_t)((char *)tn_ws - (char *)workspace) - 16;
    if (split) {
        float *sc = dm_slot;
        rc = launch_gemm_tn_split(dM, (int64_t)N, R * N, v_split ? v_split : V, (int64_t)Cin, R * Cin, dU, (int64_t)Cin, (int64_t)N * Cin, R, N, Cin,
                                  NF * NF, nullptr, sc, 0.25f, overflow, tn_ws, tn_bytes, s, "locov_winograd_wgrad_f32_split (batched TN GEMM)",
                                  v_split != nullptr);
    } else
        rc = launch_gemm_tn(dM, (int64_t)N, R * N, V, (int64_t)Cin, R * Cin, dU, (int64_t)Cin, (int64_t)N * Cin, R, N, Cin, NF * NF, nullptr,
                            tn_ws, tn_bytes, s, "locov_winograd_wgrad_f32 (batched TN GEMM)");
    if (rc) return rc;
    const int64_t NC = (int64_t)N * Cin;
    hipLaunchKernelGGL(wino_unpack_wgrad_kernel, dim3((unsigned)ceil_div(NC, 256)), dim3(256), 0, s, dU, NC, Cin, row_scale, dw);
    return check_launch("locov_winograd_wgrad_f32 (filter transform)");
}

int locov_gemm_nt_batched_f32(const float *x, int64_t lda, int64_t stride_x, const float *W, int64_t stride_w, float *y,
                              int64_t ldc, int64_t stride_y, int64_t M, int N, int K, int batch, locov_stream_t stream)
{
    LOCOV_REQUIRE(M >= 0 && N > 0 && K > 0 && batch > 0, "locov_gemm_nt_batched_f32: bad shape");
    if (M == 0) return LOCOV_OK;
    LOCOV_REQUIRE(x && W && y, "locov_gemm_nt_batched_f32: null pointer");
    LOCOV_REQUIRE(K % 4 == 0 && lda % 4 == 0 && stride_x % 4 == 0 && stride_w % 4 == 0,
                  "locov_gemm_nt_batched_f32: K, lda and the operand strides must be multiples of 4");
    LOCOV_REQUIRE(lda >= K && ldc >= N, "locov_gemm_nt_batched_f32: lda < K or ldc < N");
    LOCOV_REQUIRE((uintptr_t)x % 16 == 0 && (uintptr_t)W % 16 == 0, "locov_gemm_nt_batched_f32: misaligned pointer");
    Epilogue epi{nullptr, nullptr, nullptr, 0u};
    return launch_gemm_nt<float, float>(x, lda, W, (int64_t)K, y, ldc, M, N, K, epi, as_stream(stream),
                                        "locov_gemm_nt_batched_f32", ConvGeom{0, 0, 0, 0, 0},
                                        Batch{batch, stride_x, stride_w, stride_y});
}

}
```

### locov_amd/ops.py

```python
from __future__ import annotations

import ctypes
import itertools
import math
import threading
from typing import NamedTuple, Optional, Sequence, Tuple

import torch
from torch.autograd.function import once_differentiable

from . import _lib
from ._lib import BF16, F32, NORM_L2, NORM_NONE, NORM_STANDARDIZE, LocovError, check

__all__ = [
    "level_assign", "roi_align", "roi_align_levels", "nchw_to_nhwc", "roi_align_nhwc", "spatial_mean",
    "linear", "rownorm", "to_bf16", "sim_gemm_bf16", "box_head", "NORM_NONE", "NORM_L2",
    "NORM_STANDARDIZE", "F32", "BF16",
]


def _dev(t: torch.Tensor, name: str, dtype=torch.float32) -> torch.Tensor:
    if not isinstance(t, torch.Tensor):
        raise TypeError(f"{name} must be a torch.Tensor")
    if not t.is_cuda:
# ... 644 lines not shown
    if K == 0:
        return torch.zeros((0,), dtype=torch.int64, device=boxes.device)
    order = torch.argsort(scores, descending=True, stable=True)
    sorted_boxes = boxes[order].contiguous()
    lib = _lib.load()
    ws = _workspace("nms", boxes, int(lib.locov_nms_workspace_bytes(K)))
    keep = torch.empty((K,), dtype=torch.uint8, device=boxes.device)
    num = torch.empty((1,), dtype=torch.int32, device=boxes.device)
    with torch.cuda.device(boxes.device):
        check(lib.locov_nms_sorted(_ptr(sorted_boxes), K, float(iou_threshold), _ptr(ws), _ptr(keep), _ptr(num),
                                   _stream(boxes)), "locov_nms_sorted")
    return order[keep.bool()]


DETECT_MAX_IMAGES = _lib.LABEL_MAX_IMAGES
DETECT_MAX_ROWS_PER_IMAGE, DETECT_MAX_CLASSES, DETECT_MAX_TOPK = (1 << 14) - 1, (1 << 15) - 1, _lib.DETECT_MAX_CANDIDATES
_DETECT_PINNED = {}


def detect_postprocess(probs: torch.Tensor, deltas: torch.Tensor, proposal_boxes: torch.Tensor, sizes, image_shapes, weights,
                       scale_clamp: float, score_thresh: float, nms_thresh: float, topk: int):
    out, flags = _detect_postprocess_flags(probs, deltas, proposal_boxes, sizes, image_shapes, weights, scale_clamp, score_thresh,
                                           nms_thresh, topk)
    return None if flags else out


def _detect_postprocess_flags(probs, deltas, proposal_boxes, sizes, image_shapes, weights, scale_clamp, score_thresh, nms_thresh, topk,
                              per_class_above=None):
    probs, deltas, proposal_boxes = _dev(probs, "probs"), _dev(deltas, "deltas"), _dev(proposal_boxes, "proposal_boxes")
    B, R, K = len(sizes), probs.shape[0], probs.shape[1] - 1
    if not (tuple(deltas.shape) == (R, 4) and tuple(proposal_boxes.shape) == (R, 4) and sum(sizes) == R and len(image_shapes) == B):
        raise ValueError("detect_postprocess: inconsistent shapes")
    if not (0 < B <= DETECT_MAX_IMAGES and 1 <= K <= DETECT_MAX_CLASSES and 1 <= topk <= DETECT_MAX_TOPK
            and max(sizes, default=0) <= DETECT_MAX_ROWS_PER_IMAGE):
        raise ValueError("detect_postprocess: outside the kernels' limits (images, classes, rows per image or top-k)")
    lib = _lib.load()
    dev = probs.device
    offs = (ctypes.c_int * (B + 1))(0, *itertools.accumulate(int(n) for n in sizes))
    hw = (ctypes.c_float * (2 * B))(*[float(v) for shape in image_shapes for v in shape[:2]])
    if per_class_above is None:
        nbytes = int(lib.locov_detect_postprocess_workspace_bytes(max(R, 1), B))
    else:
        per_class_above = max(min(int(per_class_above), 2 ** 31 - 1), -2 ** 31)
        nbytes = int(lib.locov_detect_postprocess_wide_workspace_bytes(offs, B, K, per_class_above))
        if nbytes < 0:
            check(nbytes, "locov_detect_postprocess_wide_workspace_bytes")
    ws = _workspace("detect", probs, nbytes)
    out_boxes = torch.empty((B, topk, 4), dtype=torch.float32, device=dev)
    out_scores = torch.empty((B, topk), dtype=torch.float32, device=dev)
    out_classes = torch.empty((B, topk), dtype=torch.int64, device=dev)
    out_rows = torch.empty((B, topk), dtype=torch.int64, device=dev)
    counts = torch.empty((B + 1,), dtype=torch.int32, device=dev)
    wx, wy, ww, wh = (float(w) for w in weights)
    with torch.cuda.device(dev):
        if per_class_above is None:
            check(lib.locov_detect_postprocess(_ptr(probs), probs.stride(0), K, _ptr(deltas), _ptr(proposal_boxes), offs, hw, B, wx, wy, ww,
                                               wh, float(scale_clamp), float(score_thresh), float(nms_thresh), int(topk), _ptr(ws),
                                               ws.numel(), _ptr(out_boxes), _ptr(out_scores), _ptr(out_classes), _ptr(out_rows),
                                               _ptr(counts), _stream(probs)), "locov_detect_postprocess")
        else:
            check(lib.locov_detect_postprocess_wide(_ptr(probs), probs.stride(0), K, _ptr(deltas), _ptr(proposal_boxes), offs, hw, B, wx,
                                                    wy, ww, wh, float(scale_clamp), float(score_thresh), float(nms_thresh), int(topk),
                                                    per_class_above, _ptr(ws), ws.numel(), _ptr(out_boxes), _ptr(out_scores),
                                                    _ptr(out_classes), _ptr(out_rows), _ptr(counts), _stream(probs)),
                  "locov_detect_postprocess_wide")
    key = (dev, torch.cuda.current_stream(dev).cuda_stream)
    host = _DETECT_PINNED.get(key)
    if host is None or host.numel() < B + 1:
        host = _DETECT_PINNED[key] = torch.empty(max(B + 1, DETECT_MAX_IMAGES + 1), dtype=torch.int32).pin_memory()
    host[:B + 1].copy_(counts, non_blocking=True)
    ev = torch.cuda.Event()
    ev.record(torch.cuda.current_stream(dev))
    ev.synchronize()
    vals = host[:B + 1].tolist()
    return (out_boxes, out_scores, out_classes, out_rows, vals[:B]), vals[B]


def detect_postprocess_wide(probs: torch.Tensor, deltas: torch.Tensor, proposal_boxes: torch.Tensor, sizes, image_shapes, weights,
                            scale_clamp: float, score_thresh: float, nms_thresh: float, topk: int, per_class_above: int):
    out, flags = _detect_postprocess_flags(probs, deltas, proposal_boxes, sizes, image_shapes, weights, scale_clamp, score_thresh,
                                           nms_thresh, topk, per_class_above=per_class_above)
    return None if flags else out


_WS = {}


def _workspace(tag: str, ref: torch.Tensor, nbytes: int) -> torch.Tensor:
    key = (tag, ref.device, torch.cuda.current_stream(ref.device).cuda_stream)
    ws = _WS.get(key)
    if ws is None or ws.numel() < nbytes:
        _WS.pop(key, None)
        ws = _WS[key] = torch.empty(max(int(nbytes), 16), dtype=torch.uint8, device=ref.device)
    return ws


def linear_ex(x: torch.Tensor, weight: torch.Tensor, bias: Optional[torch.Tensor] = None, *, scale=None, residual=None,
              mask=None, relu: bool = False, out: Optional[torch.Tensor] = None) -> torch.Tensor:
    x = _rows(x, "x")
    weight = _rows(weight, "weight")
    M, K = x.shape
    N = weight.shape[0]
    if weight.shape[1] != K or K % 4:
        raise ValueError(f"linear_ex: x {tuple(x.shape)} weight {tuple(weight.shape)} (K must be a multiple of 4)")
    bias = _dev(bias, "bias") if bias is not None else None
    scale = _dev(scale, "scale") if scale is not None else None
    residual = _dev(residual, "residual") if residual is not None else None
    mask = _dev(mask, "mask") if mask is not None else None
    for t, name in ((residual, "residual"), (mask, "mask")):
        if t is not None and tuple(t.shape) != (M, N):
            raise ValueError(f"linear_ex: {name} must be [M,N]")
    y = torch.empty((M, N), dtype=torch.float32, device=x.device) if out is None else out
    if tuple(y.shape) != (M, N) or not y.is_contiguous():
        raise ValueError("linear_ex: out must be a contiguous [M,N] tensor")
    with torch.cuda.device(x.device):
        check(_lib.load().locov_gemm_nt_f32_ex(_ptr(x), x.stride(0) if M else K, _ptr(weight), weight.stride(0), _ptr(scale),
                                               _ptr(bias), _ptr(residual), _ptr(mask), _ptr(y), N, M, N, K,
                                               _lib.EPI_RELU if relu else 0, _stream(x)), "locov_gemm_nt_f32_ex")
    return y


def conv3x3_nhwc_ex(x: torch.Tensor, w_packed: torch.Tensor, H: int, W: int, *, scale=None, shift=None, residual=None,
                    mask=None, relu: bool = False, pos_major: bool = False) -> torch.Tensor:
    x = _dev(x, "x")
    w_packed = _dev(w_packed, "w_packed")
    M, Cin = x.shape
    N = w_packed.shape[0]
    if w_packed.shape[1] != 9 * Cin or M % (H * W) != 0:
        raise ValueError("conv3x3_nhwc_ex: inconsistent shapes")
    scale = _dev(scale, "scale") if scale is not None else None
    shift = _dev(shift, "shift") if shift is not None else None
    residual = _dev(residual, "residual") if residual is not None else None
    mask = _dev(mask, "mask") if mask is not None else None
    y = torch.empty((M, N), dtype=torch.float32, device=x.device)
    with torch.cuda.device(x.device):
        check(_lib.load().locov_conv3x3_nhwc_f32_ex(_ptr(x), M // (H * W), H, W, Cin, int(pos_major), _ptr(w_packed), _ptr(scale),
                                                    _ptr(shift), _ptr(residual), _ptr(mask), _ptr(y), N,
                                                    _lib.EPI_RELU if relu else 0, _stream(x)), "locov_conv3x3_nhwc_f32_ex")
    return y


def winograd_conv3x3_ex(x: torch.Tensor, U: torch.Tensor, *, scale=None, shift=None, mask=None, relu: bool = False,
                        roi_major: bool = True, out: Optional[torch.Tensor] = None) -> torch.Tensor:
    x = _dev(x, "x")
    U = _dev(U, "U")
    M, Cin = x.shape
    if U.dim() != 3 or U.shape[0] != 121 or U.shape[2] != Cin or M % 49 != 0:
        raise ValueError("winograd_conv3x3_ex: inconsistent shapes")
    N, R = U.shape[1], M // 49
    scale = _dev(scale, "scale") if scale is not None else None
    shift = _dev(shift, "shift") if shift is not None else None
    mask = _dev(mask, "mask") if mask is not None else None
    if mask is not None and tuple(mask.shape) != (M, N):
        raise ValueError("winograd_conv3x3_ex: mask must be [49*R, N]")
    y = _out(out, (M, N), x, "winograd_conv3x3_ex")
    lib = _lib.load()
    ws = _workspace("wino", x, int(lib.locov_winograd_workspace_bytes(R, Cin, N)))
    flags = (_lib.EPI_RELU if relu else 0) | ((_lib.WINO_OUT_ROI_MAJOR | _lib.WINO_IN_ROI_MAJOR) if roi_major else 0)
    with torch.cuda.device(x.device):
        check(lib.locov_winograd_conv3x3_f32_ex(_ptr(x), R, Cin, _ptr(U), _ptr(scale), _ptr(shift), _ptr(mask), _ptr(y), N, N,
                                                flags, _ptr(ws), ws.numel(), _stream(x)), "locov_winograd_conv3x3_f32_ex")
    return y


def gemm_tn(a: torch.Tensor, b: torch.Tensor, row_scale: Optional[torch.Tensor] = None) -> torch.Tensor:
    a, b = _rows(a, "a"), _rows(b, "b")
    M, N = a.shape
    K = b.shape[1]
    if b.shape[0] != M or N % 4 or K % 4:
        raise ValueError(f"gemm_tn: a {tuple(a.shape)} b {tuple(b.shape)} (N, K must be multiples of 4)")
    row_scale = _dev(row_scale, "row_scale") if row_scale is not None else None
    out = torch.empty((N, K), dtype=torch.float32, device=a.device)
    lib = _lib.load()
    ws = _workspace("tn", a, int(lib.locov_gemm_tn_workspace_bytes(M, N, K, 1)))
    with torch.cuda.device(a.device):
        check(lib.locov_gemm_tn_f32(_ptr(a), a.stride(0) if M else N, 0, _ptr(b), b.stride(0) if M else K, 0, _ptr(out), K, 0,
                                    M, N, K, 1, _ptr(row_scale), _ptr(ws), ws.numel(), _stream(a)), "locov_gemm_tn_f32")
    return out


def winograd_wgrad(x: torch.Tensor, g: torch.Tensor, row_scale: Optional[torch.Tensor] = None,
                   roi_major: bool = True, split: bool = False, v_split: Optional[torch.Tensor] = None) -> torch.Tensor:
    x, g = _dev(x, "x"), _dev(g, "g")
    M, Cin = x.shape
    N = g.shape[1]
    if g.shape[0] != M or M % 49 or Cin % 4 or N % 4:
        raise ValueError("winograd_wgrad: inconsistent shapes")
    R = M // 49
    if v_split is not None and not (split and R > 0 and Cin % 8 == 0 and v_split.is_cuda and v_split.device == x.device
                                    and v_split.numel() * v_split.element_size() >= 121 * R * Cin * 4 and v_split.data_ptr() % 16 == 0):
        raise ValueError("winograd_wgrad: v_split needs the split arithmetic, Cin % 8 == 0 and the forward's workspace of the same x")
    row_scale = _dev(row_scale, "row_scale") if row_scale is not None else None
    dw = torch.empty((N, Cin, 3, 3), dtype=torch.float32, device=x.device)
    lib = _lib.load()
    ws = _workspace("wino_wgrad", x, int(lib.locov_winograd_wgrad_workspace_bytes(R, Cin, N)))
    with torch.cuda.device(x.device):
        if v_split is not None:
            check(lib.locov_winograd_wgrad_f32_split_v(_ptr(v_split), _ptr(g), R, Cin, N, _lib.WINO_IN_ROI_MAJOR if roi_major else 0,
                                                       _ptr(row_scale), _ptr(dw), _ptr(_overflow_word(x)), _ptr(ws), ws.numel(),
                                                       _stream(x)), "locov_winograd_wgrad_f32_split_v")
        elif split and R > 0:
            check(lib.locov_winograd_wgrad_f32_split(_ptr(x), _ptr(g), R, Cin, N, _lib.WINO_IN_ROI_MAJOR if roi_major else 0,
                                                     _ptr(row_scale), _ptr(dw), _ptr(_overflow_word(x)), _ptr(ws), ws.numel(),
                                                     _stream(x)), "locov_winograd_wgrad_f32_split")
        else:
            check(lib.locov_winograd_wgrad_f32(_ptr(x), _ptr(g), R, Cin, N, _lib.WINO_IN_ROI_MAJOR if roi_major else 0,
                                               _ptr(row_scale), _ptr(dw), _ptr(ws), ws.numel(), _stream(x)),
                  "locov_winograd_wgrad_f32")
    return dw


def split_scale_from_amax(x: torch.Tensor, target_log2: float = 13.0) -> torch.Tensor:
    x = _dev(x, "x")
    if x.numel() % 4:
        raise ValueError("split_scale_from_amax: numel must be a multiple of 4")
    out = _scale_slot(x)
    with torch.cuda.device(x.device):
        check(_lib.load().locov_split_scale_from_amax_zeroed(_ptr(x), x.numel(), float(target_log2), _ptr(out), _stream(x)),
              "locov_split_scale_from_amax_zeroed")
    return out


def amax_bound(tensors, muls, slot: Optional[torch.Tensor] = None) -> torch.Tensor:
    ts = [(_dev(t, "tensor"), float(m)) for t, m in zip(tensors, muls) if t is not None and t.numel() > 0]
    if not ts:
        raise ValueError("amax_bound: no tensor")
    if len(ts) > _lib.AMAX_BOUND_MAX or any(t.numel() % 4 for t, _ in ts):
        raise ValueError(f"amax_bound: at most {_lib.AMAX_BOUND_MAX} tensors, numel % 4 == 0")
    if slot is None:
        slot = _scale_slot(ts[0][0], lazy=True)
    ptrs = (ctypes.c_void_p * len(ts))(*[t.data_ptr() for t, _ in ts])
    ns = (ctypes.c_int64 * len(ts))(*[t.numel() for t, _ in ts])
    ms = (ctypes.c_float * len(ts))(*[m for _, m in ts])
    with torch.cuda.device(slot.device):
        check(_lib.load().locov_amax_bound(ptrs, ns, ms, len(ts), _ptr(slot), _stream(slot)), "locov_amax_bound")
    return slot


_SCALE_SLOTS = {}


def _scale_slot(ref: torch.Tensor, lazy: bool = False) -> torch.Tensor:
    key = (ref.device, torch.cuda.current_stream(ref.device).cuda_stream)
    ring = _SCALE_SLOTS.get(key)
    if ring is None:
        ring = _SCALE_SLOTS[key] = [torch.zeros(2048, 4, dtype=torch.float32, device=ref.device), 0, False]
    i = ring[1]
    if i == 0 and ring[2]:
        ring[0].zero_()
        ring[2] = False
    ring[1] = (i + 1) % ring[0].shape[0]
    ring[2] = True
    return ring[0][i]


def scale_slot(ref: torch.Tensor) -> torch.Tensor:
    return _scale_slot(_dev(ref, "ref"), lazy=True)


def linear_split_ex(x: torch.Tensor, weight: SplitWeight, bias: Optional[torch.Tensor] = None, *, scale=None, residual=None,
                    mask=None, relu: bool = False, x_scale: float = 16.0, x_scale_dev: Optional[torch.Tensor] = None,
                    amax_out: Optional[torch.Tensor] = None, out: Optional[torch.Tensor] = None) -> torch.Tensor:
    x = _rows(x, "x")
    wd = _dev(weight.data, "weight")
    M, K = x.shape
    N = wd.shape[0]
    if wd.shape[1] != K or K % 32 or N % 4:
        raise ValueError(f"linear_split_ex: x {tuple(x.shape)} weight {tuple(wd.shape)} (K % 32 == 0, N % 4 == 0)")
    bias = _dev(bias, "bias") if bias is not None else None
    scale = _dev(scale, "scale") if scale is not None else None
    residual = _dev(residual, "residual") if residual is not None else None
    mask = _dev(mask, "mask") if mask is not None else None
    for t_, name in ((residual, "residual"), (mask, "mask")):
        if t_ is not None and tuple(t_.shape) != (M, N):
            raise ValueError(f"linear_split_ex: {name} must be [M,N]")
    y = _out(out, (M, N), x, "linear_split_ex")
    with torch.cuda.device(x.device):
        check(_lib.load().locov_gemm_nt_f32_split_ex(_ptr(x), x.stride(0) if M else K, _ptr(wd), _ptr(scale), _ptr(bias), _ptr(residual),
                                                     _ptr(mask), _ptr(y), N, M, N, K, _lib.EPI_RELU if relu else 0, float(x_scale),
                                                     _ptr(x_scale_dev), weight.scale, _ptr(_overflow_word(x)), _ptr(amax_out), _stream(x)),
              "locov_gemm_nt_f32_split_ex")
    return y


def gemm_tn_split(a: torch.Tensor, b: torch.Tensor, row_scale: Optional[torch.Tensor], a_scale_dev: torch.Tensor,
                  b_scale: float = 16.0, b_is_split: bool = False) -> torch.Tensor:
    a, b = _rows(a, "a"), _rows(b, "b")
    M, N = a.shape
    K = b.shape[1]
    if b.shape[0] != M or N % 4 or K % 4 or M == 0 or (b_is_split and (K % 8 or b.stride(0) % 8)):
        raise ValueError(f"gemm_tn_split: a {tuple(a.shape)} b {tuple(b.shape)} (N, K multiples of 4 -- 8 for a pre-split b --, M > 0)")
    row_scale = _dev(row_scale, "row_scale") if row_scale is not None else None
    out = torch.empty((N, K), dtype=torch.float32, device=a.device)
    lib = _lib.load()
    ws = _workspace("tn", a, int(lib.locov_gemm_tn_workspace_bytes(M, N, K, 1)))
    with torch.cuda.device(a.device):
        fn = lib.locov_gemm_tn_f32_split_b if b_is_split else lib.locov_gemm_tn_f32_split
        check(fn(_ptr(a), a.stride(0), 0, _ptr(b), b.stride(0), 0, _ptr(out), K, 0, M, N, K, 1, _ptr(row_scale),
                 _ptr(a_scale_dev), float(b_scale), _ptr(_overflow_word(a)), _ptr(ws), ws.numel(), _stream(a)),
              "locov_gemm_tn_f32_split_b" if b_is_split else "locov_gemm_tn_f32_split")
    return out


def winograd_conv3x3_split_ex(x: torch.Tensor, U: SplitWeight, *, scale=None, shift=None, mask=None, relu: bool = False,
                              roi_major: bool = True, v_scale: Optional[float] = None,
                              amax_out: Optional[torch.Tensor] = None, out: Optional[torch.Tensor] = None) -> torch.Tensor:
    x = _dev(x, "x")
    Ud = _dev(U.data, "U")
    M, Cin = x.shape
    if Ud.dim() != 3 or Ud.shape[0] != 121 or Ud.shape[2] != Cin or M % 49 != 0:
        raise ValueError("winograd_conv3x3_split_ex: inconsistent shapes")
    N, R = Ud.shape[1], M // 49
    scale = _dev(scale, "scale") if scale is not None else None
    shift = _dev(shift, "shift") if shift is not None else None
    mask = _dev(mask, "mask") if mask is not None else None
    if mask is not None and tuple(mask.shape) != (M, N):
        raise ValueError("winograd_conv3x3_split_ex: mask must be [49*R, N]")
    y = _out(out, (M, N), x, "winograd_conv3x3_split_ex")
    lib = _lib.load()
    ws = _workspace("wino", x, int(lib.locov_winograd_workspace_bytes(R, Cin, N)))
    flags = (_lib.EPI_RELU if relu else 0) | ((_lib.WINO_OUT_ROI_MAJOR | _lib.WINO_IN_ROI_MAJOR) if roi_major else 0)
    with torch.cuda.device(x.device):
        check(lib.locov_winograd_conv3x3_f32_split_ex(_ptr(x), R, Cin, _ptr(Ud), U.scale, float(v_scale or 1.0), int(v_scale is None),
                                                      _ptr(scale), _ptr(shift), _ptr(mask), _ptr(y), N, N, flags, 0.0, _ptr(ws), ws.numel(),
                                                      _ptr(_overflow_word(x)), _ptr(amax_out), _stream(x)), "locov_winograd_conv3x3_f32_split_ex")
    return y


def winograd_scale_slot(x: torch.Tensor, R: int, Cin: int, N: int, wgrad: bool = False) -> torch.Tensor:
    lib = _lib.load()
    if wgrad:
        ws = _workspace("wino_wgrad", x, int(lib.locov_winograd_wgrad_workspace_bytes(R, Cin, N)))
    else:
        ws = _workspace("wino", x, int(lib.locov_winograd_workspace_bytes(R, Cin, N)))
    return ws[ws.numel() - 16:].view(torch.float32)


PREP_KINDS = {"plain": _lib.PREP_PLAIN, "t": _lib.PREP_TRANSPOSE, "col": _lib.PREP_IM2COL, "flip9": _lib.PREP_IM2COL_FLIP,
              "wino": _lib.PREP_WINO, "uflip": _lib.PREP_WINO_FLIP}


def prep_shape(kind: str, w: torch.Tensor) -> Tuple[int, ...]:
    N, C = w.shape[0], w.shape[1]
    return {"plain": (N, C), "t": (C, N), "col": (N, 9 * C), "flip9": (C, 9 * N), "wino": (121, N, C), "uflip": (121, C, N)}[kind]


def res5_weight_prep(jobs) -> None:
    if not jobs:
        return
    lib = _lib.load()
    ref = jobs[0][1]
    for i in range(0, len(jobs), _lib.WEIGHT_PREP_MAX_JOBS):
        chunk = jobs[i:i + _lib.WEIGHT_PREP_MAX_JOBS]
        arr = (_lib.WeightPrepJob * len(chunk))()
        for a, (kind, w, rs, out, scale) in zip(arr, chunk):
            w = _dev(w, "weight")
            if tuple(out.shape) != prep_shape(kind, w) or out.dtype != torch.float32 or not out.is_contiguous() or out.device != w.device:
                raise ValueError(f"res5_weight_prep: out of a {kind!r} job must be a contiguous fp32 {prep_shape(kind, w)} tensor")
            a.w, a.row_scale, a.out = w.data_ptr(), (_dev(rs, "row_scale").data_ptr() if rs is not None else None), out.data_ptr()
            a.scale, a.kind, a.N, a.K = float(scale), PREP_KINDS[kind], int(w.shape[0]), int(w.shape[1])
        with torch.cuda.device(ref.device):
            check(lib.locov_res5_weight_prep(arr, len(chunk), _ptr(_overflow_word(ref)), _stream(ref)), "locov_res5_weight_prep")


def weight_transpose_scale(w: torch.Tensor, row_scale: Optional[torch.Tensor] = None) -> torch.Tensor:
    w = _dev(w, "w")
    N, K = w.shape
    row_scale = _dev(row_scale, "row_scale") if row_scale is not None else None
    out = torch.empty((K, N), dtype=torch.float32, device=w.device)
    with torch.cuda.device(w.device):
        check(_lib.load().locov_weight_transpose_scale(_ptr(w), N, K, _ptr(row_scale), _ptr(out), _stream(w)),
              "locov_weight_transpose_scale")
    return out


def conv3x3_weight_flip(w: torch.Tensor, row_scale: Optional[torch.Tensor] = None) -> torch.Tensor:
    w = _dev(w, "w")
    N, Cin = w.shape[:2]
    row_scale = _dev(row_scale, "row_scale") if row_scale is not None else None
    out = torch.empty((Cin, N, 3, 3), dtype=torch.float32, device=w.device)
    with torch.cuda.device(w.device):
        check(_lib.load().locov_conv3x3_weight_flip(_ptr(w), N, Cin, _ptr(row_scale), _ptr(out), _stream(w)),
              "locov_conv3x3_weight_flip")
    return out


def im2col3x3(x: torch.Tensor, H: int, W: int) -> torch.Tensor:
    x = _dev(x, "x")
    M, C = x.shape
    if M % (H * W) or C % 4:
        raise ValueError("im2col3x3: inconsistent shapes")
    col = torch.empty((M, 9 * C), dtype=torch.float32, device=x.device)
    with torch.cuda.device(x.device):
        check(_lib.load().locov_im2col3x3_nhwc(_ptr(x), M // (H * W), H, W, C, _ptr(col), _stream(x)), "locov_im2col3x3_nhwc")
    return col


def conv3x3_wgrad_unpack(dw_packed: torch.Tensor, row_scale: Optional[torch.Tensor] = None) -> torch.Tensor:
    dw_packed = _dev(dw_packed, "dw_packed")
    N, K9 = dw_packed.shape
    Cin = K9 // 9
    row_scale = _dev(row_scale, "row_scale") if row_scale is not None else None
    dw = torch.empty((N, Cin, 3, 3), dtype=torch.float32, device=dw_packed.device)
    with torch.cuda.device(dw.device):
        check(_lib.load().locov_conv3x3_wgrad_unpack(_ptr(dw_packed), N, Cin, _ptr(row_scale), _ptr(dw), _stream(dw)),
              "locov_conv3x3_wgrad_unpack")
    return dw


def relu_mask(g: torch.Tensor, act: torch.Tensor, amax_out: Optional[torch.Tensor] = None, out: Optional[torch.Tensor] = None) -> torch.Tensor:
    g, act = _dev(g, "g"), _dev(act, "act")
    if g.shape != act.shape or g.numel() % 4:
        raise ValueError("relu_mask: shapes must match, numel % 4 == 0")
    out = _out(out, tuple(g.shape), g, "relu_mask")
    with torch.cuda.device(g.device):
        check(_lib.load().locov_relu_mask(_ptr(g), _ptr(act), g.numel(), _ptr(out), _ptr(amax_out), _stream(g)), "locov_relu_mask")
    return out


LABEL_MAX_IMAGES, LABEL_MAX_THRESHOLDS = _lib.LABEL_MAX_IMAGES, _lib.LABEL_MAX_THRESHOLDS
AMAX_BOUND_MAX = _lib.AMAX_BOUND_MAX


def label_proposals(boxes: torch.Tensor, n_props, gt_boxes: torch.Tensor, gt_classes: torch.Tensor, n_gt, thresholds, labels_of,
                    num_classes: int, rnd: torch.Tensor):
    boxes = _dev(boxes, "boxes")
    B, total = len(n_props), int(sum(n_props))
    if B > _lib.LABEL_MAX_IMAGES or len(labels_of) > _lib.LABEL_MAX_THRESHOLDS or boxes.shape[0] != total:
        raise ValueError("label_proposals: too many images / matcher intervals, or counts that do not add up")
    dev = boxes.device
    gt_boxes = _dev(gt_boxes, "gt_boxes") if sum(n_gt) else None
    gt_classes = _dev(gt_classes, "gt_classes", torch.int64) if sum(n_gt) else None
    rnd = _dev(rnd, "rnd", torch.float64)
    gt_index = torch.empty(total, dtype=torch.int64, device=dev)
    labels = torch.empty(total, dtype=torch.int64, device=dev)
    keys = torch.empty((2, total), dtype=torch.float64, device=dev)
    rows = torch.zeros((B, 4), dtype=torch.int64, device=dev)
    roff = (ctypes.c_int * (B + 1))(*([0] + list(itertools.accumulate(int(n) for n in n_props))))
    goff = (ctypes.c_int * (B + 1))(*([0] + list(itertools.accumulate(int(n) for n in n_gt))))
    nt = len(labels_of)
    lo = (ctypes.c_float * max(nt, 1))(*[float(v) for v in thresholds[:-1]])
    hi = (ctypes.c_float * max(nt, 1))(*[float(v) for v in thresholds[1:]])
    lab = (ctypes.c_int * max(nt, 1))(*[int(v) for v in labels_of])
    with torch.cuda.device(dev):
        check(_lib.load().locov_label_proposals(_ptr(boxes), roff, _ptr(gt_boxes), _ptr(gt_classes), goff, B, lo, hi, lab, nt,
                                                int(num_classes), _ptr(rnd), _ptr(gt_index), _ptr(labels), _ptr(keys[0]), _ptr(keys[1]),
                                                _ptr(rows), _stream(boxes)), "locov_label_proposals")
    return gt_index, labels, keys[0], keys[1], rows


SAMPLE_MAX_PROPOSALS = _lib.SAMPLE_MAX_PROPOSALS


def sample_proposals(key_pos: torch.Tensor, key_neg: torch.Tensor, labels: torch.Tensor, gt_index: torch.Tensor, rows: torch.Tensor,
                     boxes: torch.Tensor, gt_boxes: Optional[torch.Tensor], n_props, n_gt, budget: int, max_pos: int, num_classes: int,
                     field: Optional[torch.Tensor] = None):
    boxes = _dev(boxes, "boxes")
    B, total = len(n_props), int(sum(n_props))
    if B > _lib.LABEL_MAX_IMAGES or boxes.shape[0] != total or not n_props or max(n_props) > SAMPLE_MAX_PROPOSALS or min(n_props) < 1:
        raise ValueError("sample_proposals: 1..64 images of 1..4096 proposals each, counts that add up")
    dev = boxes.device
    key_pos, key_neg = _dev(key_pos, "key_pos", torch.float64), _dev(key_neg, "key_neg", torch.float64)
    labels, gt_index, rows = _dev(labels, "labels", torch.int64), _dev(gt_index, "gt_index", torch.int64), _dev(rows, "rows", torch.int64)
    gt_boxes = _dev(gt_boxes, "gt_boxes") if sum(n_gt) else None
    field = _dev(field, "field") if field is not None else None
    n = B * int(budget)
    picked = torch.empty(n, dtype=torch.int64, device=dev)
    out_boxes = torch.empty((n, 4), dtype=torch.float32, device=dev)
    classes = torch.empty(n, dtype=torch.int64, device=dev)
    out_gt = torch.empty((n, 4), dtype=torch.float32, device=dev)
    fg = torch.empty(n, dtype=torch.int64, device=dev)
    rois = torch.empty((n, 5), dtype=torch.float32, device=dev)
    field_out = torch.empty(n, dtype=torch.float32, device=dev) if field is not None else None
    roff = (ctypes.c_int * (B + 1))(*([0] + list(itertools.accumulate(int(v) for v in n_props))))
    goff = (ctypes.c_int * (B + 1))(*([0] + list(itertools.accumulate(int(v) for v in n_gt))))
    with torch.cuda.device(dev):
        check(_lib.load().locov_sample_proposals(_ptr(key_pos), _ptr(key_neg), _ptr(labels), _ptr(gt_index), _ptr(rows), _ptr(boxes),
                                                 _ptr(gt_boxes), _ptr(field), roff, goff, B, int(budget), int(max_pos), int(num_classes),
                                                 _ptr(picked), _ptr(out_boxes), _ptr(classes), _ptr(out_gt), _ptr(fg), _ptr(rois),
                                                 _ptr(field_out), _stream(boxes)), "locov_sample_proposals")
    return picked, out_boxes, classes, out_gt, fg, rois, field_out


def zero_if_raised(tensors, word: torch.Tensor) -> None:
    ts = [t for t in tensors if t is not None and t.numel() > 0]
    if not ts:
        return
    for t in ts:
        if not (t.is_cuda and t.dtype == torch.float32 and t.is_contiguous()):
            raise LocovError("zero_if_raised: contiguous fp32 device tensors only")
    lib = _lib.load()
    with torch.cuda.device(word.device):
        for i in range(0, len(ts), _lib.ZERO_LIST_MAX):
            chunk = ts[i:i + _lib.ZERO_LIST_MAX]
            ptrs = (ctypes.c_void_p * len(chunk))(*[t.data_ptr() for t in chunk])
            counts = (ctypes.c_int64 * len(chunk))(*[t.numel() for t in chunk])
            check(lib.locov_zero_if_raised(ptrs, counts, len(chunk), _ptr(word), _stream(word)), "locov_zero_if_raised")


def spatial_mean_bwd(g: torch.Tensor, act: Optional[torch.Tensor], hw: int, amax_out: Optional[torch.Tensor] = None,
                     out: Optional[torch.Tensor] = None) -> torch.Tensor:
    g = _dev(g, "g")
    R, C = g.shape
    act = _dev(act, "act") if act is not None else None
    if act is not None and tuple(act.shape) != (R * hw, C):
        raise ValueError("spatial_mean_bwd: act must be [R*hw, C]")
    out = _out(out, (R * hw, C), g, "spatial_mean_bwd")
    with torch.cuda.device(g.device):
        check(_lib.load().locov_spatial_mean_bwd(_ptr(g), _ptr(act), R, C, hw, _ptr(out), _ptr(amax_out), _stream(g)), "locov_spatial_mean_bwd")
    return out


def rows_stride2(src: torch.Tensor, N: int, H: int, W: int, forward: bool, out: Optional[torch.Tensor] = None) -> torch.Tensor:
    src = _dev(src, "src")
    C = src.shape[-1]
    OH, OW = (H + 1) // 2, (W + 1) // 2
    out = _out(out, (N * OH * OW, C) if forward else (N, H, W, C), src, "rows_stride2")
    with torch.cuda.device(src.device):
        check(_lib.load().locov_rows_stride2(_ptr(src), N, H, W, C, int(forward), _ptr(out), _stream(src)), "locov_rows_stride2")
    return out


def roi_align_nhwc_bwd(grad_rows: torch.Tensor, feat_shape, rois: torch.Tensor, output_size: int, spatial_scale: float,
                       sampling_ratio: int = 0, aligned: bool = True, bin_stride: int = 1, pos_major: bool = False,
                       accumulate_into: Optional[torch.Tensor] = None) -> torch.Tensor:
    grad_rows = _rows(grad_rows, "grad_rows")
    rois = _dev(rois, "rois")
    N, H, W, C = feat_shape
    if accumulate_into is None:
        gf = torch.zeros((N, H, W, C), dtype=torch.float32, device=grad_rows.device)
    else:
        gf = _out(accumulate_into, (N, H, W, C), grad_rows, "roi_align_nhwc_bwd")
    with torch.cuda.device(gf.device):
        check(_lib.load().locov_roi_align_nhwc_bwd(_ptr(grad_rows), grad_rows.stride(0) if grad_rows.shape[0] else C, N, H, W, C,
                                                   _ptr(rois), rois.shape[0], output_size, output_size, float(spatial_scale),
                                                   int(sampling_ratio), int(aligned), int(bin_stride), int(pos_major), _ptr(gf),
                                                   _stream(gf)), "locov_roi_align_nhwc_bwd")
    return gf


def nhwc_to_nchw(x: torch.Tensor) -> torch.Tensor:
    x = _dev(x, "x")
    N, H, W, C = x.shape
    out = torch.empty((N, C, H, W), dtype=torch.float32, device=x.device)
    with torch.cuda.device(x.device):
        check(_lib.load().locov_nchw_to_nhwc(_ptr(x), N, H * W, C, 1, _ptr(out), F32, _stream(x)), "locov_nchw_to_nhwc")
    return out


class _LinearFn(torch.autograd.Function):

    @staticmethod
    def forward(ctx, x, weight, bias):
        ctx.save_for_backward(x, weight)
        ctx.has_bias = bias is not None
        return linear(x, weight, bias)

    @staticmethod
    def backward(ctx, g):
        x, weight = ctx.saved_tensors
        g = g.contiguous()
        gx = gw = gb = None
        N, K = weight.shape
        if ctx.needs_input_grad[0]:
            gx = linear(g, weight_transpose_scale(weight.detach()))
        if ctx.needs_input_grad[1]:
            if N % 4 == 0 and K % 4 == 0:
                gw = gemm_tn(g, x)
            else:
                gw = linear(g.t().contiguous(), x.t().contiguous())
        if ctx.has_bias and ctx.needs_input_grad[2]:
            gb = g.sum(dim=0)
        return gx, gw, gb


def linear_autograd(x: torch.Tensor, weight: torch.Tensor, bias: Optional[torch.Tensor] = None) -> torch.Tensor:
    if torch.is_grad_enabled() and (x.requires_grad or weight.requires_grad or (bias is not None and bias.requires_grad)):
        return _LinearFn.apply(x, weight, bias)
    return linear(x.detach(), weight.detach(), bias.detach() if bias is not None else None)


class _GroundingFn(torch.autograd.Function):
    @staticmethod
    def forward(ctx, S, cmask, rmask, B, T, NR, temperature):
        S = _dev(S, "S")
        cmask, rmask = _dev(cmask, "caption_mask"), _dev(rmask, "region_mask")
        w2r = torch.empty((B, B), dtype=torch.float32, device=S.device)
        r2w = torch.empty((B, B), dtype=torch.float32, device=S.device)
        with torch.cuda.device(S.device):
            check(_lib.load().locov_grounding_fwd(_ptr(S), B, T, NR, _ptr(cmask), _ptr(rmask), float(temperature),
                                                  _ptr(w2r), _ptr(r2w), _stream(S)), "locov_grounding_fwd")
        ctx.save_for_backward(S, cmask, rmask)
        ctx.dims = (B, T, NR, temperature)
        return w2r, r2w

    @staticmethod
    def backward(ctx, g_w2r, g_r2w):
        S, cmask, rmask = ctx.saved_tensors
        B, T, NR, temperature = ctx.dims
        g_w2r = _dev(g_w2r if g_w2r is not None else torch.zeros(B, B, device=S.device), "grad_w2r")
        g_r2w = _dev(g_r2w if g_r2w is not None else torch.zeros(B, B, device=S.device), "grad_r2w")
        dS = torch.empty_like(S)
        with torch.cuda.device(S.device):
            check(_lib.load().locov_grounding_bwd(_ptr(S), B, T, NR, _ptr(cmask), _ptr(rmask), float(temperature),
                                                  _ptr(g_w2r), _ptr(g_r2w), _ptr(dS), _stream(S)),
                  "locov_grounding_bwd")
# ... 562 lines not shown
```

### locov_amd/res5_train.py

```python
from __future__ import annotations

import os
from typing import List, NamedTuple, Optional, Sequence, Tuple

import torch

from . import ops

__all__ = ["res5_rows", "res5_grid", "res5_rois", "roi_align_even_rows", "to_nhwc", "Res5BlockFn", "Res5OutputFn", "Res5Step", "Segment",
           "saved_activations"]

_BWD_STREAMS = bool(int(os.environ.get("LOCOV_RES5_BWD_STREAMS", "1")))
_SIDE_STREAMS = {}


def _side_stream(device) -> "torch.cuda.Stream":
    key = (torch.device(device), torch.cuda.current_stream(device).cuda_stream)
    st = _SIDE_STREAMS.get(key)
    if st is None:
        st = _SIDE_STREAMS[key] = torch.cuda.Stream(device=device)
    return st


_KEEP_V = bool(int(os.environ.get("LOCOV_RES5_KEEP_V", "1")))
_NO_WINO_BWD = bool(int(os.environ.get("LOCOV_RES5_BWD_DIRECT", "0")))
_BWD_F32 = bool(int(os.environ.get("LOCOV_RES5_BWD_F32", "0")))


def _wino_ok(H: int, W: int, cin: int, cout: int) -> bool:
    return H == 7 and W == 7 and cin % 32 == 0 and cout % 4 == 0


class Segment(NamedTuple):
    row0: int
    n: int
    H: int
    W: int

    @property
    def rows(self) -> int:
        return self.n * self.H * self.W

    @property
    def wino(self) -> bool:
        return self.H == 7 and self.W == 7


class Res5Step:

    def __init__(self, stage, split: bool, device, capacity_rows: int, grid: bool = True, rois: bool = True):
        self.stage, self.split, self.device = stage, bool(split), torch.device(device)
        self.operands = stage.train_operands(self.split, grid=grid, rois=rois)
        self.capacity = int(capacity_rows)
        self.segments: List[Segment] = []
        self.filled = 0
        self._pending: List[int] = []
        new = lambda c: torch.empty((self.capacity, c), dtype=torch.float32, device=self.device)
        self.x0 = new(stage[0].conv1.in_channels)
        self.act = [(new(b.conv1.out_channels), new(b.conv2.out_channels), new(b.conv3.out_channels)) for b in stage]
        self.cols = {}
        self.wino_ws = {}

    def input_rows(self, rows: int) -> torch.Tensor:
        row0 = self.filled + sum(self._pending)
        if row0 + rows > self.capacity:
            raise ValueError(f"Res5Step: {row0} + {rows} rows exceed the capacity of {self.capacity}")
        self._pending.append(rows)
        return self.x0[row0:row0 + rows]

    @torch.no_grad()
    def forward(self, n: int, H: int, W: int, on_range_final=None) -> Segment:
        return self.forward_segments([(n, H, W)], on_range_final)[0]

    @torch.no_grad()
    def forward_segments(self, geoms: Sequence[Tuple[int, int, int]], on_range_final=None) -> List[Segment]:
        assert [g[0] * g[1] * g[2] for g in geoms] == self._pending, "Res5Step.forward: input_rows() of every segment first"
        new = []
        for (n, H, W) in geoms:
            seg = Segment(self.filled, n, H, W)
            new.append((len(self.segments), seg))
            self.segments.append(seg)
            self.filled += seg.rows
        self._pending = []
        live = [(si, seg) for si, seg in new if seg.rows > 0]
        if not live:
            return [seg for _, seg in new]
        stage, T = self.stage, self.operands
        lo, hi = live[0][1].row0, live[-1][1].row0 + live[-1][1].rows
        joint = slice(lo, hi)
        x = self.x0[joint]
        nb = len(stage)
        for bi, blk in enumerate(stage):
            Y1, Y2, OUT = self.act[bi]
            s1, b1 = stage.operands.fold(blk.conv1)
            s2, b2 = stage.operands.fold(blk.conv2)
            s3, b3 = stage.operands.fold(blk.conv3)
            c2 = blk.conv2
            _linear(x, T.get(blk.conv1, "plain"), b1, scale=s1, relu=True, out=Y1[joint])
            if blk.shortcut is not None:
                ss, bs = stage.operands.fold(blk.shortcut)
                sc = _linear(x, T.get(blk.shortcut, "plain"), bs, scale=ss)
            else:
                sc = x
            last = bi == nb - 1
            w3 = T.get(blk.conv3, "plain")
            order = sorted(live, key=lambda it: self.seg_wino(it[1], c2)) if last else live
            for si, seg in order:
                sl = slice(seg.row0, seg.row0 + seg.rows)
                early = False
                if self.seg_wino(seg, c2):
                    u2 = T.get(c2, "wino")
                    early = (on_range_final is not None and last and blk.shortcut is None
                             and isinstance(u2, ops.SplitWeight) and isinstance(w3, ops.SplitWeight))
                    keep = None
                    if _KEEP_V and isinstance(u2, ops.SplitWeight) and c2.in_channels % 8 == 0 and seg.n > 0:
                        ws_bytes = ops.winograd_workspace_bytes(seg.n, c2.in_channels, c2.out_channels)
                        if ws_bytes == 121 * seg.n * (c2.in_channels + c2.out_channels) * 4 + 16:
                            keep = self.wino_ws[(bi, si)] = torch.empty(ws_bytes, dtype=torch.uint8, device=self.device)
                    ops.winograd_conv3x3(Y1[sl], u2, scale=s2, shift=b2, relu=True, roi_major=True, in_roi_major=True, out=Y2[sl],
                                         range_check_scale=16.0 if early else None, workspace=keep)
                    if early:
                        on_range_final()
                        on_range_final = None
                else:
                    col = self.cols[(bi, si)] = ops.im2col3x3(Y1[sl], seg.H, seg.W)
                    _linear(col, T.get(c2, "col"), b2, scale=s2, relu=True, out=Y2[sl])
                if last and len(live) > 1:
                    _linear(Y2[sl], w3, b3, scale=s3, residual=sc[sl.start - lo:sl.stop - lo], relu=True, out=OUT[sl])
            if not (last and len(live) > 1):
                _linear(Y2[joint], w3, b3, scale=s3, residual=sc, relu=True, out=OUT[joint])
            x = OUT[joint]
        return [seg for _, seg in new]

    def seg_wino(self, seg: Segment, c2) -> bool:
        return seg.wino and _wino_ok(seg.H, seg.W, c2.in_channels, c2.out_channels)

    def outputs(self, inputs: Sequence[torch.Tensor], pooled: Sequence[bool]) -> List[torch.Tensor]:
        assert len(inputs) == len(pooled) == len(self.segments) and not self._pending
        active = ops.active_guard(self.device) if self.split else None
        self.skip_words = [getattr(active, "step_word", active.word)] if active is not None and getattr(active, "deferred", False) else []
        self.bwd_split = self.split and not _BWD_F32
        self._carry = None
        self._prefetched = False
        self.need_x0 = any(t.requires_grad for t in inputs)
        h = None
        for bi, blk in enumerate(self.stage):
            head_w = (blk.conv1.weight,) + ((blk.shortcut.weight,) if blk.shortcut is not None else ())
            y1 = Res5BlockFn.apply(self, bi, "head", len(inputs), *inputs, *head_w) if bi == 0 else Res5BlockFn.apply(self, bi, "head", 1, h, *head_w)
            h = Res5BlockFn.apply(self, bi, "tail", 1, y1, blk.conv2.weight, blk.conv3.weight)
        outs = Res5OutputFn.apply(self, tuple(bool(p) for p in pooled), h)
        return list(outs) if isinstance(outs, tuple) else [outs]

    def _bwd_operands(self):
        sp = self.bwd_split
        return self.operands if self.operands.split == bool(sp) else self.stage.train_operands(bool(sp))

    def _bwd_guarded(self, fn):
        if not self.bwd_split:
            grads = fn()
            for w in self.skip_words:
                ops.zero_if_raised(grads, w)
            return grads
        guard = self.stage.range_guard("bwd", self.device)
        with ops.range_guard(guard):
            self._prefetch_bwd_operands()
            grads = fn()
        ops.zero_if_raised(grads, guard.word)
        for w in self.skip_words:
            ops.zero_if_raised(grads, w)
        return grads

    def _prefetch_bwd_operands(self) -> None:
        if self._prefetched:
            return
        self._prefetched = True
        T = self._bwd_operands()
        if not T.split:
            return
        live = [seg for seg in self.segments if seg.rows > 0]
        for bi, blk in enumerate(self.stage):
            c2 = blk.conv2
            want = [(blk.conv3, "t")]
            if bi > 0 or self.need_x0:
                want.append((blk.conv1, "t"))
                if blk.shortcut is not None:
                    want.append((blk.shortcut, "t"))
            for seg in live:
                want.append((c2, "uflip" if _wino_ok(seg.H, seg.W, c2.out_channels, c2.in_channels) and not _NO_WINO_BWD else "flip9"))
            for conv, tag in want:
                if (conv, tag) not in T.ready:
                    T.get(conv, tag)


def _linear(x, W, bias=None, **kw):
    if isinstance(W, ops.SplitWeight):
        return ops.linear_split(x, W, bias, **kw)
    return ops.linear(x, W, bias, **kw)


_BACKWARD_MARK = None


def _mark(kind: str, bi: int = -1) -> None:
    if _BACKWARD_MARK is not None:
        _BACKWARD_MARK(kind, bi)


class Res5OutputFn(torch.autograd.Function):

    @staticmethod
    def forward(ctx, step, pooled, h):
        ctx.step, ctx.pooled = step, pooled
        last = step.act[-1][2]
        ctx.save_for_backward(last[:step.filled])
        outs = []
        for seg, pool in zip(step.segments, pooled):
            o = last[seg.row0:seg.row0 + seg.rows]
            if pool:
                o = ops.spatial_mean(o.view(seg.n, seg.H, seg.W, o.shape[1]), channels_last=1) if seg.rows else o.new_zeros((0, o.shape[1]))
            outs.append(o)
        return tuple(outs)

    @staticmethod
    def backward(ctx, *grad_outs):
        step = ctx.step
        _mark("backward_begin")
        (out_last,) = ctx.saved_tensors
        rows = step.filled
        sp = step.bwd_split
        g = torch.empty((rows, out_last.shape[1]), dtype=torch.float32, device=step.device)
        if rows == 0:
            step._carry = ("tail", g, None)
            return None, None, g
        bound_of, bound_mul = [], []
        for seg, pool, go in zip(step.segments, ctx.pooled, grad_outs):
            if seg.rows == 0:
                continue
            sl = slice(seg.row0, seg.row0 + seg.rows)
            if go is None:
                g[sl].zero_()
                continue
            go = ops._dev(go, "grad_out")
            if pool:
                ops.spatial_mean_bwd(go, out_last[sl], seg.H * seg.W, out=g[sl])
            else:
                ops.relu_mask(go, out_last[sl], out=g[sl])
            bound_of.append(go)
            bound_mul.append(1.0 / (seg.H * seg.W) if pool else 1.0)
        if not sp:
            sg = None
        elif bound_of and len(bound_of) <= ops.AMAX_BOUND_MAX and all(t.numel() % 4 == 0 for t in bound_of):
            sg = ops.amax_bound(bound_of, bound_mul)
        else:
            sg = ops.split_scale_from_amax(g)
        for w in step.skip_words:
            ops.zero_if_raised([g], w)
        step._carry = ("tail", g, sg)
        return None, None, g


class Res5BlockFn(torch.autograd.Function):

    @staticmethod
    def forward(ctx, step, bi, half, n_in, *args):
        rows = step.filled
        ctx.step, ctx.bi, ctx.half, ctx.n_in = step, bi, half, n_in
        ctx.nw = len(args) - n_in
        y1, y2, out = step.act[bi]
        if half == "head":
            x = step.x0 if bi == 0 else step.act[bi - 1][2]
            ctx.save_for_backward(x[:rows], y1[:rows])
            return y1[:rows]
        ctx.save_for_backward(y1[:rows], y2[:rows], out[:rows])
        return out[:rows]

    @staticmethod
    def backward(ctx, g):
        step = ctx.step
        if ctx.half == "tail":
            _mark("block_begin", ctx.bi)
        fn = Res5BlockFn._backward_tail if ctx.half == "tail" else Res5BlockFn._backward_head
        grads = step._bwd_guarded(lambda: fn(ctx, g))
        _mark("block_mid" if ctx.half == "tail" else "block_end", ctx.bi)
        return (None, None, None, None) + tuple(grads)

    @staticmethod
    def _take_carry(step, g, what):
        carry, step._carry = step._carry, None
        if carry is None or carry[0] != what or carry[1].data_ptr() != g.data_ptr() or carry[1].shape != g.shape:
            raise RuntimeError("Res5BlockFn.backward: the gradient of a node's output must come from the node behind it "
                               "(the tensors between two Res5 nodes are internal to Res5Step.outputs)")
        return carry[1:]

    @staticmethod
    def _helpers(ctx):
        step = ctx.step
        sp = step.bwd_split
        T = step._bwd_operands()
        slot = (lambda ref: ops.scale_slot(ref)) if sp else (lambda ref: None)

        def wgrad_1x1(g_, sg_, x_, s_):
            if sp and g_.shape[1] % 4 == 0 and x_.shape[1] % 4 == 0 and g_.shape[0] > 0:
                return ops.gemm_tn_split(g_, x_, s_, sg_, 16.0)
            return ops.gemm_tn(g_, x_, s_)

        def dgrad_1x1(g_, sg_, conv, tag="t", amax_out=None, wt=None, **kw):
            if wt is None:
                wt = T.get(conv, tag)
            if isinstance(wt, ops.SplitWeight):
                return ops.linear_split_ex(g_, wt, x_scale_dev=sg_, amax_out=amax_out, **kw), amax_out
            y_ = ops.linear_ex(g_, wt, **kw)
            return y_, (ops.split_scale_from_amax(y_) if sp and amax_out is not None else None)

        return sp, T, slot, wgrad_1x1, dgrad_1x1

    @staticmethod
    def _backward_tail(ctx, g):
        step, bi = ctx.step, ctx.bi
        stage, segs = step.stage, step.segments
        rows = step.filled
        blk = stage[bi]
        need_w = ctx.needs_input_grad[5:]
        gw: List[Optional[torch.Tensor]] = [None, None]
        if rows == 0:
            g1 = g.new_empty((0, blk.conv1.out_channels))
            step._carry = ("head", g1, None, g, None)
            return (g1,) + tuple(torch.zeros_like(w) if need else None for w, need in zip((blk.conv2.weight, blk.conv3.weight), need_w))
        g, sg = Res5BlockFn._take_carry(step, g, "tail")
        sp, T, slot, wgrad_1x1, dgrad_1x1 = Res5BlockFn._helpers(ctx)
        y1, y2, _ = ctx.saved_tensors
        s2, s3 = stage.operands.fold(blk.conv2)[0], stage.operands.fold(blk.conv3)[0]
        c2 = blk.conv2
        if need_w[1]:
            gw[1] = wgrad_1x1(g, sg, y2, s3).view_as(blk.conv3.weight)
        g2, sg2 = dgrad_1x1(g, sg, blk.conv3, amax_out=slot(g), mask=y2)
        g1 = torch.empty((rows, y1.shape[1]), dtype=torch.float32, device=step.device)
        sg1 = slot(g2)
        live = [(si, seg) for si, seg in enumerate(segs) if seg.rows > 0]
        side = _side_stream(step.device) if _BWD_STREAMS and len(live) == 2 and sum(step.seg_wino(sg_, c2) for _, sg_ in live) == 1 else None
        main = torch.cuda.current_stream(step.device)
        flipped = {}
        for _, seg in live:
            tag = "uflip" if _wino_ok(seg.H, seg.W, c2.out_channels, c2.in_channels) and not _NO_WINO_BWD else "flip9"
            if tag not in flipped:
                flipped[tag] = T.get(c2, tag)
        parts = []
        for si, seg in live:
            sl = slice(seg.row0, seg.row0 + seg.rows)
            wino = step.seg_wino(seg, c2)
            on_side = side is not None and not wino
            if on_side:
                side.wait_stream(main)
                for t_ in (g1, g2, y1):
                    t_.record_stream(side)
            with torch.cuda.stream(side if on_side else main):
                part = None
                if need_w[0]:
                    if wino and c2.out_channels % 4 == 0 and not _NO_WINO_BWD:
                        part = ops.winograd_wgrad(y1[sl], g2[sl], s2, roi_major=True, split=sp, v_split=step.wino_ws.get((bi, si)) if sp else None)
                    else:
                        colw = step.cols.get((bi, si))
                        if colw is None:
                            colw = ops.im2col3x3(y1[sl], seg.H, seg.W)
                        elif on_side:
                            colw.record_stream(side)
                        if sp:
                            part = ops.conv3x3_wgrad_unpack(ops.gemm_tn_split(g2[sl], colw, None, sg2, 16.0), s2)
                        else:
                            part = ops.conv3x3_wgrad_unpack(ops.gemm_tn(g2[sl], colw), s2)
                    if on_side:
                        part.record_stream(main)
                    parts.append(part)
                if _wino_ok(seg.H, seg.W, c2.out_channels, c2.in_channels) and not _NO_WINO_BWD:
                    uflip = flipped["uflip"]
                    if isinstance(uflip, ops.SplitWeight):
                        ops.winograd_conv3x3_split_ex(g2[sl], uflip, mask=y1[sl], roi_major=True, amax_out=sg1, out=g1[sl])
                    else:
                        ops.winograd_conv3x3_ex(g2[sl], uflip, mask=y1[sl], roi_major=True, out=g1[sl])
                        if sp and g1[sl].numel() % 4 == 0:
                            ops.amax_bound([g1[sl]], [1.0], slot=sg1)
                else:
                    _, got = dgrad_1x1(ops.im2col3x3(g2[sl], seg.H, seg.W), sg2, c2, "flip9", amax_out=sg1, wt=flipped["flip9"],
                                       mask=y1[sl], out=g1[sl])
                    if sp and got is not sg1 and g1[sl].numel() % 4 == 0:
                        ops.amax_bound([g1[sl]], [1.0], slot=sg1)
        if side is not None:
            main.wait_stream(side)
        if need_w[0]:
            dw2 = parts[0]
            for part in parts[1:]:
                dw2 = dw2.add_(part)
            gw[0] = dw2
        step._carry = ("head", g1, sg1, g, sg)
        return (g1,) + tuple(gw)

    @staticmethod
    def _backward_head(ctx, g1):
        step, bi, n_in = ctx.step, ctx.bi, ctx.n_in
        stage, segs = step.stage, step.segments
        rows = step.filled
        blk = stage[bi]
        has_sc = blk.shortcut is not None
        first = bi == 0
        need_x = any(ctx.needs_input_grad[4:4 + n_in])
        need_w = ctx.needs_input_grad[4 + n_in:]
        gw: List[Optional[torch.Tensor]] = [None] * ctx.nw
        weights = (blk.conv1.weight,) + ((blk.shortcut.weight,) if has_sc else ())
        if rows == 0:
            step._carry = None
            if not first:
                gx = torch.empty((0, blk.conv1.in_channels), dtype=torch.float32, device=step.device)
                step._carry = ("tail", gx, None)
                return (gx,) + tuple(torch.zeros_like(w) if need else None for w, need in zip(weights, need_w))
            return tuple(None for _ in range(n_in)) + tuple(torch.zeros_like(w) if need else None for w, need in zip(weights, need_w))
        g1, sg1, g, sg = Res5BlockFn._take_carry(step, g1, "head")
        sp, T, slot, wgrad_1x1, dgrad_1x1 = Res5BlockFn._helpers(ctx)
        x, _ = ctx.saved_tensors
        s1 = stage.operands.fold(blk.conv1)[0]
        if need_w[0]:
            gw[0] = wgrad_1x1(g1, sg1, x, s1).view_as(blk.conv1.weight)
        if has_sc:
            ss = stage.operands.fold(blk.shortcut)[0]
            if need_w[1]:
                gw[1] = wgrad_1x1(g, sg, x, ss).view_as(blk.shortcut.weight)
        if not need_x:
            return tuple(None for _ in range(n_in)) + tuple(gw)
        mask = None if first else x
        gx, sgx = dgrad_1x1(g1, sg1, blk.conv1, amax_out=None if (first or has_sc) else slot(g1),
                            residual=None if has_sc else g, mask=None if has_sc else mask)
        if has_sc:
            gx, sgx = dgrad_1x1(g, sg, blk.shortcut, amax_out=None if first else slot(g), residual=gx, mask=mask)
        if not first:
            step._carry = ("tail", gx, sgx)
            return (gx,) + tuple(gw)
        gxs = [None] * n_in
        for i, seg in enumerate(segs):
            if ctx.needs_input_grad[4 + i]:
                gxs[i] = gx[seg.row0:seg.row0 + seg.rows]
        return tuple(gxs) + tuple(gw)


def saved_activations(out: torch.Tensor) -> List[torch.Tensor]:
    found, stack, seen = {}, [out.grad_fn], set()
    while stack:
        n = stack.pop()
        if n is None or id(n) in seen:
            continue
        seen.add(id(n))
        if "Res5BlockFn" in type(n).__name__:
            found[(n.bi, n.half)] = n
        stack += [f for f, _ in n.next_functions]
    saved = []
    for bi in sorted({k[0] for k in found}):
        x, y1 = found[(bi, "head")].saved_tensors
        _, y2, o = found[(bi, "tail")].saved_tensors
        saved += [x, y1, y2, o]
    return saved


def _guarded(stage, split, guard, device, build):
    own = None
    if split and guard is not None and ops.active_guard(device) is None:
        own = stage.range_guard("fwd", device)
        own.reset()
    with ops.range_guard(own):
        step = build(split)
    if own is not None and own.raised():
        stage.forget_scales()
        if guard[0] is not None:
            guard[0]()
        del step
        step = build(False)
    return step


def res5_rows(stage, x0: torch.Tensor, R: int, H: int, W: int, pooled: bool = False, split: bool = True,
              overflow_check: bool = True, on_overflow=None) -> torch.Tensor:
    assert stage.supports_rows_path(), "the rows path needs FrozenBN, STRIDE_IN_1X1 and ungrouped convolutions"
    xd = ops._dev(x0.detach(), "x0")

    def build(sp):
        step = Res5Step(stage, sp, xd.device, R * H * W, grid=not (H == 7 and W == 7), rois=H == 7 and W == 7)
        step.input_rows(R * H * W).copy_(xd)
        step.forward(R, H, W)
        return step
    step = _guarded(stage, split, (on_overflow,) if overflow_check else None, xd.device, build)
    return step.outputs([x0], [pooled])[0]


class _ToNHWC(torch.autograd.Function):
    @staticmethod
    def forward(ctx, x):
        return ops.nchw_to_nhwc(x.detach())

    @staticmethod
    def backward(ctx, g):
        return ops.nhwc_to_nchw(g)


class _ToNCHW(torch.autograd.Function):
    @staticmethod
    def forward(ctx, x):
        return ops.nhwc_to_nchw(x.detach())

    @staticmethod
    def backward(ctx, g):
        return ops.nchw_to_nhwc(g)


def to_nhwc(x: torch.Tensor) -> torch.Tensor:
    return _ToNHWC.apply(x)


class _RoiAlignEvenRows(torch.autograd.Function):

    @staticmethod
    def forward(ctx, nhwc, rois, P, scale, sampling_ratio, aligned, step=None):
        o = (P + 1) // 2
        dst = step.input_rows(o * o * rois.shape[0]) if step is not None else None
        out = ops.roi_align_nhwc(nhwc.detach(), rois, P, scale, sampling_ratio, aligned, bin_stride=2, pos_major=False, out=dst)
        ctx.save_for_backward(rois)
        ctx.args = (tuple(nhwc.shape), P, scale, sampling_ratio, aligned)
        return out.view(-1, nhwc.shape[3])

    @staticmethod
    def backward(ctx, g):
        (rois,) = ctx.saved_tensors
        shape, P, scale, sampling_ratio, aligned = ctx.args
        return ops.roi_align_nhwc_bwd(g, shape, rois, P, scale, sampling_ratio, aligned, bin_stride=2, pos_major=False), \
            None, None, None, None, None, None


def roi_align_even_rows(nhwc, rois, P, scale, sampling_ratio, aligned, step=None) -> torch.Tensor:
    return _RoiAlignEvenRows.apply(nhwc, rois, int(P), float(scale), int(sampling_ratio), bool(aligned), step)


class _Stride2Rows(torch.autograd.Function):
    @staticmethod
    def forward(ctx, nhwc, step=None):
        N, H, W, _ = nhwc.shape
        ctx.dims = (N, H, W)
        dst = step.input_rows(N * ((H + 1) // 2) * ((W + 1) // 2)) if step is not None else None
        return ops.rows_stride2(nhwc.detach(), N, H, W, True, out=dst)

    @staticmethod
    def backward(ctx, g):
        N, H, W = ctx.dims
        return ops.rows_stride2(g, N, H, W, False), None


def grid_rows(nhwc: torch.Tensor, step=None) -> torch.Tensor:
    return _Stride2Rows.apply(nhwc, step)


def grid_segment(step: "Res5Step", nhwc: torch.Tensor) -> torch.Tensor:
    N, H, W, _ = nhwc.shape
    rows = grid_rows(nhwc, step)
    step.forward(N, (H + 1) // 2, (W + 1) // 2)
    return rows


def roi_segment(step: "Res5Step", nhwc: torch.Tensor, rois: torch.Tensor, P: int, scale: float, sampling_ratio: int, aligned: bool,
                on_range_final=None) -> torch.Tensor:
    x0 = roi_align_even_rows(nhwc, rois, P, scale, sampling_ratio, aligned, step)
    o = (int(P) + 1) // 2
    step.forward(rois.shape[0], o, o, on_range_final=on_range_final)
    return x0


def grid_and_roi_segments(step: "Res5Step", nhwc: torch.Tensor, rois: torch.Tensor, P: int, scale: float, sampling_ratio: int, aligned: bool,
                          on_range_final=None):
    N, H, W, _ = nhwc.shape
    rows = grid_rows(nhwc, step)
    x0 = roi_align_even_rows(nhwc, rois, P, scale, sampling_ratio, aligned, step)
    o = (int(P) + 1) // 2
    step.forward_segments([(N, (H + 1) // 2, (W + 1) // 2), (rois.shape[0], o, o)], on_range_final=on_range_final)
    return rows, x0


def grid_capacity(nhwc: torch.Tensor) -> int:
    N, H, W, _ = nhwc.shape
    return N * ((H + 1) // 2) * ((W + 1) // 2)


def to_nchw(rows: torch.Tensor, N: int, OH: int, OW: int, channels_last: bool = False) -> torch.Tensor:
    if channels_last:
        return rows.view(N, OH, OW, rows.shape[1]).permute(0, 3, 1, 2)
    return _ToNCHW.apply(rows.view(N, OH, OW, rows.shape[1]))


def res5_grid(stage, nhwc: torch.Tensor, split: bool = True, overflow_check: bool = True, on_overflow=None,
              channels_last: bool = False) -> torch.Tensor:
    N, H, W, _ = nhwc.shape
    assert stage.supports_rows_path() and stage[0].stride == 2 and stage[0].stride_in_1x1
    OH, OW = (H + 1) // 2, (W + 1) // 2
    made = {}

    def build(sp):
        step = Res5Step(stage, sp, nhwc.device, N * OH * OW, rois=False)
        made["rows"] = grid_segment(step, nhwc)
        return step
    step = _guarded(stage, split, (on_overflow,) if overflow_check else None, nhwc.device, build)
    return to_nchw(step.outputs([made["rows"]], [False])[0], N, OH, OW, channels_last=channels_last)


def res5_rois(stage, nhwc: torch.Tensor, rois: torch.Tensor, P: int, scale: float, sampling_ratio: int, aligned: bool,
              pooled: bool = False, split: bool = True, overflow_check: bool = True, on_overflow=None) -> torch.Tensor:
    assert stage.supports_rows_path() and stage[0].stride == 2 and stage[0].stride_in_1x1
    o = (int(P) + 1) // 2
    made = {}

    def build(sp):
        step = Res5Step(stage, sp, nhwc.device, o * o * rois.shape[0], grid=False, rois=o == 7)
        made["x0"] = roi_segment(step, nhwc, rois, P, scale, sampling_ratio, aligned)
        return step
    step = _guarded(stage, split, (on_overflow,) if overflow_check else None, nhwc.device, build)
    return step.outputs([made["x0"]], [pooled])[0]
```

Baseline: 386,700.

## Batch split-K weight-gradient reductions into one multi-job reduce kernel

Weight-gradient GEMMs in the Res5 backward now leave their split-K partials in workspace instead of each launching its own reduce. A single multi-job reduce kernel then sums them, applies row scales, and folds in the 3x3 unpack or Winograd output transform. When both Winograd and im2col partials exist, it adds them in the same pass. This removes separate reduce, unpack and transform launches, but each partial now needs its own tagged workspace and the output transform runs inside a generic reduce kernel.

Result: no change. 387,400, median of 3 (+0.2%).

```diff
diff --git a/include/locov_hip.h b/include/locov_hip.h
--- a/include/locov_hip.h
+++ b/include/locov_hip.h
@@ -371,6 +371,29 @@
 } locov_weight_prep_job;
 int locov_res5_weight_prep(const locov_weight_prep_job *jobs, int n_jobs, unsigned *overflow, locov_stream_t stream);
 
+#define LOCOV_TN_REDUCE_MAX_JOBS 8
+enum {
+    LOCOV_TN_MAP_PLAIN = 0,
+    LOCOV_TN_MAP_CONV3X3 = 1,
+    LOCOV_TN_MAP_WINO = 2
+};
+typedef struct locov_tn_reduce_job {
+    const float *partials;
+    const float *partials2;
+    const float *row_scale;
+    float *out;
+    int64_t ldo, stride_o;
+    int N, K, splits, batch, map, splits2;
+} locov_tn_reduce_job;
+int locov_gemm_tn_partials(const float *a, int64_t lda, const float *b, int64_t ldb, int64_t M, int N, int K,
+                           const float *a_scale_dev, float b_scale, int b_is_split, unsigned *overflow,
+                           void *partials, int64_t partials_bytes, int *splits_out, locov_stream_t stream);
+int locov_winograd_wgrad_partials(const float *x, const float *v_split, const float *g, int64_t R, int Cin, int N,
+                                  unsigned flags, int split, unsigned *overflow, void *workspace,
+                                  int64_t workspace_bytes, const float **partials_out, int *splits_out,
+                                  locov_stream_t stream);
+int locov_gemm_tn_reduce(const locov_tn_reduce_job *jobs, int n_jobs, locov_stream_t stream);
+
 int locov_weight_transpose_scale(const float *w, int N, int K, const float *row_scale, float *out,
                                  locov_stream_t stream);
 int locov_conv3x3_weight_flip(const float *w, int N, int Cin, const float *row_scale, float *out,
diff --git a/locov_amd/_lib.py b/locov_amd/_lib.py
--- a/locov_amd/_lib.py
+++ b/locov_amd/_lib.py
@@ -36,6 +36,15 @@
 
 class WeightPrepJob(ctypes.Structure):
     _fields_ = [("w", c_void_p), ("row_scale", c_void_p), ("out", c_void_p), ("scale", c_float), ("kind", c_int), ("N", c_int), ("K", c_int)]
+
+
+TN_REDUCE_MAX_JOBS = 8
+TN_MAP_PLAIN, TN_MAP_CONV3X3, TN_MAP_WINO = range(3)
+
+
+class TnReduceJob(ctypes.Structure):
+    _fields_ = [("partials", c_void_p), ("partials2", c_void_p), ("row_scale", c_void_p), ("out", c_void_p), ("ldo", c_int64),
+                ("stride_o", c_int64), ("N", c_int), ("K", c_int), ("splits", c_int), ("batch", c_int), ("map", c_int), ("splits2", c_int)]
 
 
 SIGNATURES = {
@@ -151,6 +160,10 @@
     "locov_winograd_wgrad_workspace_bytes": (c_int64, [c_int64, c_int, c_int]),
     "locov_winograd_wgrad_f32": (c_int, [_p, _p, c_int64, c_int, c_int, c_uint, _p, _p, _p, c_int64, _p]),
     "locov_res5_weight_prep": (c_int, [POINTER(WeightPrepJob), c_int, _p, _p]),
+    "locov_gemm_tn_partials": (c_int, [_p, c_int64, _p, c_int64, c_int64, c_int, c_int, _p, c_float, c_int, _p, _p, c_int64, POINTER(c_int), _p]),
+    "locov_winograd_wgrad_partials": (c_int, [_p, _p, _p, c_int64, c_int, c_int, c_uint, c_int, _p, _p, c_int64, POINTER(c_void_p),
+                                              POINTER(c_int), _p]),
+    "locov_gemm_tn_reduce": (c_int, [POINTER(TnReduceJob), c_int, _p]),
     "locov_weight_transpose_scale": (c_int, [_p, c_int, c_int, _p, _p, _p]),
     "locov_conv3x3_weight_flip": (c_int, [_p, c_int, c_int, _p, _p, _p]),
     "locov_im2col3x3_nhwc": (c_int, [_p, c_int64, c_int, c_int, c_int, _p, _p]),
diff --git a/locov_amd/csrc/gemm_nt.h b/locov_amd/csrc/gemm_nt.h
--- a/locov_amd/csrc/gemm_nt.h
+++ b/locov_amd/csrc/gemm_nt.h
@@ -80,12 +80,18 @@
                                float spatial_scale, int sampling_ratio, int aligned, const float *ch_scale, const float *ch_shift, int relu,
                                float *V, float v_scale, unsigned *overflow, hipStream_t s);
 
+struct TnPartials {
+    const float *at;
+    int splits;
+};
 int launch_gemm_tn(const float *A, int64_t lda, int64_t sa, const float *B, int64_t ldb, int64_t sb, float *out, int64_t ldo,
                    int64_t so, int64_t M, int N, int K, int batch, const float *row_scale, float *ws, int64_t ws_bytes,
-                   hipStream_t s, const char *what);
+                   hipStream_t s, const char *what, TnPartials *partials = nullptr);
+int launch_tn_reduce_jobs(const locov_tn_reduce_job *jobs, int n_jobs, hipStream_t s, const char *what);
 int64_t gemm_tn_workspace_bytes(int64_t M, int N, int K, int batch);
 int launch_gemm_tn_split(const float *A, int64_t lda, int64_t sa, const float *B, int64_t ldb, int64_t sb, float *out, int64_t ldo,
                          int64_t so, int64_t M, int N, int K, int batch, const float *row_scale, const float *a_scale_dev, float b_scale,
-                         unsigned *overflow, float *ws, int64_t ws_bytes, hipStream_t s, const char *what, bool b_split = false);
+                         unsigned *overflow, float *ws, int64_t ws_bytes, hipStream_t s, const char *what, bool b_split = false,
+                         TnPartials *partials = nullptr);
 
 }
diff --git a/locov_amd/csrc/gemm_tn.hip b/locov_amd/csrc/gemm_tn.hip
--- a/locov_amd/csrc/gemm_tn.hip
+++ b/locov_amd/csrc/gemm_tn.hip
@@ -1,4 +1,5 @@
 #include "gemm_nt.h"
+#include "winograd_tables.h"
 
 #include <cstdlib>
 
@@ -128,20 +129,104 @@
         }
 }
 
-__global__ __launch_bounds__(256) void gemm_tn_reduce_kernel(const float *__restrict__ P, int N, int K, int splits, int batch,
-                                                             const float *__restrict__ row_scale, float *__restrict__ out,
-                                                             int64_t ldo, int64_t so)
-{
-    const int k4 = K >> 2;
-    const int64_t per = (int64_t)N * k4, total = per * batch;
-    for (int64_t i = (int64_t)blockIdx.x * blockDim.x + threadIdx.x; i < total; i += (int64_t)gridDim.x * blockDim.x) {
-        const int64_t b = i / per, rem = i - b * per;
-        const int n = (int)(rem / k4), k = (int)(rem - (int64_t)n * k4) * 4;
-        f32x4 a = {0.f, 0.f, 0.f, 0.f};
-        const float *p = P + (b * splits) * (int64_t)N * K + (int64_t)n * K + k;
-        for (int s = 0; s < splits; s++) a += *reinterpret_cast<const f32x4 *>(p + (int64_t)s * N * K);
-        if (row_scale) a *= row_scale[n];
-        *reinterpret_cast<f32x4 *>(out + b * so + (int64_t)n * ldo + k) = a;
+struct TnReduceJobs {
+    locov_tn_reduce_job job[LOCOV_TN_REDUCE_MAX_JOBS];
+};
+
+template <int CNT>
+__device__ __forceinline__ void tn_chunk_sums(float (&a)[CNT], const float *__restrict__ p, int64_t elem_stride, int splits, int64_t chunk_stride)
+{
+#pragma unroll
+    for (int e = 0; e < CNT; e++) a[e] = 0.f;
+    for (int s = 0; s < splits; s++) {
+        float v[CNT];
+#pragma unroll
+        for (int e = 0; e < CNT; e++) v[e] = p[e * elem_stride + s * chunk_stride];
+#pragma unroll
+        for (int e = 0; e < CNT; e++) a[e] += v[e];
+    }
+}
+
+__global__ __launch_bounds__(256) void gemm_tn_reduce_kernel(TnReduceJobs jobs)
+{
+    const locov_tn_reduce_job &j = jobs.job[blockIdx.y];
+    const float *__restrict__ P = j.partials;
+    const float *__restrict__ row_scale = j.row_scale;
+    float *__restrict__ out = j.out;
+    const int N = j.N, K = j.K, splits = j.splits;
+    const int64_t NK = (int64_t)N * K;
+    const int64_t i0 = (int64_t)blockIdx.x * blockDim.x + threadIdx.x, istep = (int64_t)gridDim.x * blockDim.x;
+    if (j.map == LOCOV_TN_MAP_PLAIN) {
+        const int k4 = K >> 2;
+        const int64_t per = (int64_t)N * k4, total = per * j.batch;
+        for (int64_t i = i0; i < total; i += istep) {
+            const int64_t b = i / per, rem = i - b * per;
+            const int n = (int)(rem / k4), k = (int)(rem - (int64_t)n * k4) * 4;
+            f32x4 a = {0.f, 0.f, 0.f, 0.f};
+            const float *p = P + (b * splits) * NK + (int64_t)n * K + k;
+            int s = 0;
+            for (; s + 4 <= splits; s += 4) {
+                f32x4 v[4];
+#pragma unroll
+                for (int e = 0; e < 4; e++) v[e] = *reinterpret_cast<const f32x4 *>(p + (int64_t)(s + e) * NK);
+#pragma unroll
+                for (int e = 0; e < 4; e++) a += v[e];
+            }
+            for (; s < splits; s++) a += *reinterpret_cast<const f32x4 *>(p + (int64_t)s * NK);
+            if (row_scale) a *= row_scale[n];
+            *reinterpret_cast<f32x4 *>(out + b * j.stride_o + (int64_t)n * j.ldo + k) = a;
+        }
+        return;
+    }
+    const int Cin = j.map == LOCOV_TN_MAP_WINO ? K : K / 9;
+    const int64_t NC = (int64_t)N * Cin;
+    for (int64_t i = i0; i < NC; i += istep) {
+        const int64_t n = i / Cin;
+        const int c = (int)(i - n * Cin);
+        const float sc = row_scale ? row_scale[n] : 1.f;
+        float w[9];
+        if (j.map == LOCOV_TN_MAP_CONV3X3) {
+            tn_chunk_sums<9>(w, P + n * K + c, Cin, splits, NK);
+#pragma unroll
+            for (int t = 0; t < 9; t++) w[t] *= sc;
+        } else {
+            using wino::G;
+            using wino::NF;
+            double g[3][3] = {{0, 0, 0}, {0, 0, 0}, {0, 0, 0}};
+#pragma unroll
+            for (int fy = 0; fy < NF; fy++) {
+                float u[NF];
+                if (splits == 1) {
+#pragma unroll
+                    for (int fx = 0; fx < NF; fx++) u[fx] = P[(int64_t)(fy * NF + fx) * NC + i];
+                } else
+                    tn_chunk_sums<NF>(u, P + (int64_t)fy * NF * splits * NC + i, (int64_t)splits * NC, splits, NC);
+                double t[3] = {0, 0, 0};
+#pragma unroll
+                for (int fx = 0; fx < NF; fx++)
+#pragma unroll
+                    for (int b = 0; b < 3; b++) t[b] = fma(G[fx][b], (double)u[fx], t[b]);
+#pragma unroll
+                for (int a = 0; a < 3; a++)
+#pragma unroll
+                    for (int b = 0; b < 3; b++) g[a][b] = fma(G[fy][a], t[b], g[a][b]);
+            }
+            const double scd = row_scale ? (double)row_scale[n] : 1.0;
+#pragma unroll
+            for (int t = 0; t < 9; t++) w[t] = (float)(scd * g[t / 3][t % 3]);
+            if (j.partials2 != nullptr) {
+                float v[9];
+                tn_chunk_sums<9>(v, j.partials2 + n * 9 * Cin + c, Cin, j.splits2, NC * 9);
+#pragma unroll
+                for (int t = 0; t < 9; t++) {
+                    v[t] *= sc;
+                    asm volatile("" : "+v"(v[t]));
+                    w[t] += v[t];
+                }
+            }
+        }
+#pragma unroll
+        for (int t = 0; t < 9; t++) out[i * 9 + t] = w[t];
     }
 }
 
@@ -158,18 +243,37 @@
     *splits = (int)ceil_div(M, mc);
 }
 
+static int64_t tn_reduce_items(const locov_tn_reduce_job &j)
+{
+    if (j.map == LOCOV_TN_MAP_PLAIN) return (int64_t)j.batch * j.N * (j.K / 4);
+    return (int64_t)j.N * (j.map == LOCOV_TN_MAP_WINO ? j.K : j.K / 9);
+}
+
+int launch_tn_reduce_jobs(const locov_tn_reduce_job *jobs, int n_jobs, hipStream_t s, const char *what)
+{
+    TnReduceJobs list{};
+    int64_t most = 0;
+    for (int i = 0; i < n_jobs; i++) {
+        list.job[i] = jobs[i];
+        const int64_t items = tn_reduce_items(jobs[i]);
+        most = items > most ? items : most;
+    }
+    if (most == 0) return LOCOV_OK;
+    const unsigned blocks = (unsigned)(ceil_div(most, 256) < 8192 ? ceil_div(most, 256) : 8192);
+    hipLaunchKernelGGL(gemm_tn_reduce_kernel, dim3(blocks, (unsigned)n_jobs), dim3(256), 0, s, list);
+    return check_launch(what);
+}
+
 int launch_tn_reduce(const float *ws, int N, int K, int splits, int batch, const float *row_scale, float *out, int64_t ldo, int64_t so,
                      hipStream_t s, const char *what)
 {
-    const int64_t total = (int64_t)batch * N * (K / 4);
-    const unsigned blocks = (unsigned)(ceil_div(total, 256) < 8192 ? ceil_div(total, 256) : 8192);
-    hipLaunchKernelGGL(gemm_tn_reduce_kernel, dim3(blocks), dim3(256), 0, s, ws, N, K, splits, batch, row_scale, out, ldo, so);
-    return check_launch(what);
+    const locov_tn_reduce_job job{ws, nullptr, row_scale, out, ldo, so, N, K, splits, batch, LOCOV_TN_MAP_PLAIN, 0};
+    return launch_tn_reduce_jobs(&job, 1, s, what);
 }
 
 int launch_gemm_tn(const float *A, int64_t lda, int64_t sa, const float *B, int64_t ldb, int64_t sb, float *out, int64_t ldo,
                    int64_t so, int64_t M, int N, int K, int batch, const float *row_scale, float *ws, int64_t ws_bytes,
-                   hipStream_t s, const char *what)
+                   hipStream_t s, const char *what, TnPartials *partials)
 {
     int splits;
     int64_t m_chunk;
@@ -189,6 +293,11 @@
     hipLaunchKernelGGL(gemm_tn_kernel, dim3((unsigned)wgs), dim3(TNT), 0, s, A, lda, B, ldb, direct ? out : ws, M, N, K, splits, m_chunk, sa, sb);
     timing_end(trec, s);
     int rc = check_launch(what);
+    if (partials != nullptr) {
+        partials->at = direct ? out : ws;
+        partials->splits = splits;
+        return rc;
+    }
     if (rc || direct) return rc;
     return launch_tn_reduce(ws, N, K, splits, batch, row_scale, out, ldo, so, s, what);
 }
@@ -229,4 +338,48 @@
                           static_cast<float *>(workspace), workspace_bytes, as_stream(stream), "locov_gemm_tn_f32");
 }
 
-}
+int locov_gemm_tn_partials(const float *a, int64_t lda, const float *b, int64_t ldb, int64_t M, int N, int K, const float *a_scale_dev,
+                           float b_scale, int b_is_split, unsigned *overflow, void *partials, int64_t partials_bytes, int *splits_out,
+                           locov_stream_t stream)
+{
+    LOCOV_REQUIRE(M > 0 && N > 0 && K > 0, "locov_gemm_tn_partials: bad shape M=%lld N=%d K=%d", (long long)M, N, K);
+    LOCOV_REQUIRE(a && b && partials && splits_out, "locov_gemm_tn_partials: null pointer");
+    LOCOV_REQUIRE(lda >= N && ldb >= K, "locov_gemm_tn_partials: lda < N or ldb < K");
+    LOCOV_REQUIRE(a_scale_dev || !b_is_split, "locov_gemm_tn_partials: a pre-split b needs the split arithmetic (a_scale_dev)");
+    float *ws = static_cast<float *>(partials);
+    TnPartials got{nullptr, 0};
+    const int rc = a_scale_dev
+        ? launch_gemm_tn_split(a, lda, 0, b, ldb, 0, ws, (int64_t)K, 0, M, N, K, 1, nullptr, a_scale_dev, b_scale, overflow, ws, partials_bytes,
+                               as_stream(stream), "locov_gemm_tn_partials", b_is_split != 0, &got)
+        : launch_gemm_tn(a, lda, 0, b, ldb, 0, ws, (int64_t)K, 0, M, N, K, 1, nullptr, ws, partials_bytes, as_stream(stream),
+                         "locov_gemm_tn_partials", &got);
+    *splits_out = got.splits;
+    return rc;
+}
+
+int locov_gemm_tn_reduce(const locov_tn_reduce_job *jobs, int n_jobs, locov_stream_t stream)
+{
+    LOCOV_REQUIRE(n_jobs >= 0 && n_jobs <= LOCOV_TN_REDUCE_MAX_JOBS, "locov_gemm_tn_reduce: 0..%d jobs per call", LOCOV_TN_REDUCE_MAX_JOBS);
+    if (n_jobs == 0) return LOCOV_OK;
+    LOCOV_REQUIRE(jobs, "locov_gemm_tn_reduce: null job list");
+    for (int i = 0; i < n_jobs; i++) {
+        const locov_tn_reduce_job &j = jobs[i];
+        LOCOV_REQUIRE(j.map == LOCOV_TN_MAP_PLAIN || j.map == LOCOV_TN_MAP_CONV3X3 || j.map == LOCOV_TN_MAP_WINO,
+                      "locov_gemm_tn_reduce: job %d: unknown map %d", i, j.map);
+        LOCOV_REQUIRE(j.N > 0 && j.K > 0 && j.splits > 0 && j.batch > 0, "locov_gemm_tn_reduce: job %d: bad shape", i);
+        LOCOV_REQUIRE(j.partials && j.out, "locov_gemm_tn_reduce: job %d: null pointer", i);
+        LOCOV_REQUIRE(((uintptr_t)j.partials | (uintptr_t)j.partials2 | (uintptr_t)j.out) % 16 == 0, "locov_gemm_tn_reduce: job %d: misaligned pointer", i);
+        if (j.map == LOCOV_TN_MAP_PLAIN)
+            LOCOV_REQUIRE(j.K % 4 == 0 && j.ldo % 4 == 0 && j.stride_o % 4 == 0 && j.ldo >= j.K,
+                          "locov_gemm_tn_reduce: job %d: K, ldo and stride_o must be multiples of 4, ldo >= K", i);
+        if (j.map == LOCOV_TN_MAP_CONV3X3)
+            LOCOV_REQUIRE(j.K % 9 == 0 && j.batch == 1, "locov_gemm_tn_reduce: job %d: the 3x3 mapping needs K = 9 Cin and one problem", i);
+        if (j.map == LOCOV_TN_MAP_WINO)
+            LOCOV_REQUIRE(j.batch == wino::NF * wino::NF, "locov_gemm_tn_reduce: job %d: the Winograd mapping takes %d problems", i, wino::NF * wino::NF);
+        LOCOV_REQUIRE(j.partials2 == nullptr || (j.map == LOCOV_TN_MAP_WINO && j.splits2 > 0),
+                      "locov_gemm_tn_reduce: job %d: partials2 goes with the Winograd mapping and splits2 > 0", i);
+    }
+    return launch_tn_reduce_jobs(jobs, n_jobs, as_stream(stream), "locov_gemm_tn_reduce");
+}
+
+}
diff --git a/locov_amd/csrc/gemm_tn_split.hip b/locov_amd/csrc/gemm_tn_split.hip
--- a/locov_amd/csrc/gemm_tn_split.hip
+++ b/locov_amd/csrc/gemm_tn_split.hip
@@ -245,7 +245,7 @@
 
 int launch_gemm_tn_split(const float *A, int64_t lda, int64_t sa, const float *B, int64_t ldb, int64_t sb, float *out, int64_t ldo,
                          int64_t so, int64_t M, int N, int K, int batch, const float *row_scale, const float *a_scale_dev, float b_scale,
-                         unsigned *overflow, float *ws, int64_t ws_bytes, hipStream_t s, const char *what, bool b_split)
+                         unsigned *overflow, float *ws, int64_t ws_bytes, hipStream_t s, const char *what, bool b_split, TnPartials *partials)
 {
     int splits;
     int64_t m_chunk;
@@ -272,6 +272,11 @@
                            sb, a_scale_dev, b_scale, overflow);
     timing_end(trec, s);
     int rc = check_launch(what);
+    if (partials != nullptr) {
+        partials->at = direct ? out : ws;
+        partials->splits = splits;
+        return rc;
+    }
     if (rc || direct) return rc;
     return launch_tn_reduce(ws, N, K, splits, batch, row_scale, out, ldo, so, s, what);
 }
diff --git a/locov_amd/csrc/winograd.hip b/locov_amd/csrc/winograd.hip
--- a/locov_amd/csrc/winograd.hip
+++ b/locov_amd/csrc/winograd.hip
@@ -505,7 +505,7 @@
 
 static int winograd_wgrad(const float *x, const float *g, int64_t R, int Cin, int N, unsigned flags, const float *row_scale,
                           float *dw, void *workspace, int64_t workspace_bytes, locov_stream_t stream, bool split, unsigned *overflow,
-                          const float *v_split = nullptr);
+                          const float *v_split = nullptr, TnPartials *partials = nullptr);
 
 int locov_winograd_wgrad_f32(const float *x, const float *g, int64_t R, int Cin, int N, unsigned flags, const float *row_scale,
                              float *dw, void *workspace, int64_t workspace_bytes, locov_stream_t stream)
@@ -527,12 +527,28 @@
     return winograd_wgrad(v_split, g, R, Cin, N, flags, row_scale, dw, workspace, workspace_bytes, stream, true, overflow, v_split);
 }
 
+int locov_winograd_wgrad_partials(const float *x, const float *v_split, const float *g, int64_t R, int Cin, int N, unsigned flags, int split,
+                                  unsigned *overflow, void *workspace, int64_t workspace_bytes, const float **partials_out, int *splits_out,
+                                  locov_stream_t stream)
+{
+    LOCOV_REQUIRE(R > 0, "locov_winograd_wgrad_partials: no tiles");
+    LOCOV_REQUIRE(partials_out && splits_out, "locov_winograd_wgrad_partials: null pointer");
+    LOCOV_REQUIRE((x != nullptr) != (v_split != nullptr), "locov_winograd_wgrad_partials: exactly one of x and v_split");
+    LOCOV_REQUIRE(v_split == nullptr || (split && Cin % 8 == 0), "locov_winograd_wgrad_partials: v_split needs the split arithmetic and Cin % 8 == 0");
+    TnPartials got{nullptr, 0};
+    const int rc = winograd_wgrad(v_split ? v_split : x, g, R, Cin, N, flags, nullptr, nullptr, workspace, workspace_bytes, stream, split != 0,
+                                  overflow, v_split, &got);
+    *partials_out = got.at;
+    *splits_out = got.splits;
+    return rc;
+}
+
 static int winograd_wgrad(const float *x, const float *g, int64_t R, int Cin, int N, unsigned flags, const float *row_scale,
                           float *dw, void *workspace, int64_t workspace_bytes, locov_stream_t stream, bool split, unsigned *overflow,
-                          const float *v_split)
+                          const float *v_split, TnPartials *partials)
 {
     LOCOV_REQUIRE(R >= 0 && Cin > 0 && N > 0, "locov_winograd_wgrad_f32: bad shape");
-    LOCOV_REQUIRE(dw, "locov_winograd_wgrad_f32: null output");
+    LOCOV_REQUIRE(dw || partials, "locov_winograd_wgrad_f32: null output");
     hipStream_t s = as_stream(stream);
     if (R == 0) {
         hipError_t e = hipMemsetAsync(dw, 0, (size_t)N * Cin * 9 * sizeof(float), s);
@@ -568,11 +584,11 @@
         float *sc = dm_slot;
         rc = launch_gemm_tn_split(dM, (int64_t)N, R * N, v_split ? v_split : V, (int64_t)Cin, R * Cin, dU, (int64_t)Cin, (int64_t)N * Cin, R, N, Cin,
                                   NF * NF, nullptr, sc, 0.25f, overflow, tn_ws, tn_bytes, s, "locov_winograd_wgrad_f32_split (batched TN GEMM)",
-                                  v_split != nullptr);
+                                  v_split != nullptr, partials);
     } else
         rc = launch_gemm_tn(dM, (int64_t)N, R * N, V, (int64_t)Cin, R * Cin, dU, (int64_t)Cin, (int64_t)N * Cin, R, N, Cin, NF * NF, nullptr,
-                            tn_ws, tn_bytes, s, "locov_winograd_wgrad_f32 (batched TN GEMM)");
-    if (rc) return rc;
+                            tn_ws, tn_bytes, s, "locov_winograd_wgrad_f32 (batched TN GEMM)", partials);
+    if (rc || partials) return rc;
     const int64_t NC = (int64_t)N * Cin;
     hipLaunchKernelGGL(wino_unpack_wgrad_kernel, dim3((unsigned)ceil_div(NC, 256)), dim3(256), 0, s, dU, NC, Cin, row_scale, dw);
     return check_launch("locov_winograd_wgrad_f32 (filter transform)");
diff --git a/locov_amd/ops.py b/locov_amd/ops.py
--- a/locov_amd/ops.py
+++ b/locov_amd/ops.py
@@ -970,6 +970,83 @@
     return out
 
 
+class TnPartials(NamedTuple):
+    ptr: int
+    splits: int
+    N: int
+    K: int
+    batch: int
+    keep: torch.Tensor
+
+
+def gemm_tn_partials(a: torch.Tensor, b: torch.Tensor, a_scale_dev: Optional[torch.Tensor] = None, b_scale: float = 16.0,
+                     b_is_split: bool = False, tag: str = "tn_part") -> TnPartials:
+    a, b = _rows(a, "a"), _rows(b, "b")
+    M, N = a.shape
+    K = b.shape[1]
+    if b.shape[0] != M or N % 4 or K % 4 or M == 0 or (b_is_split and (K % 8 or b.stride(0) % 8)):
+        raise ValueError(f"gemm_tn_partials: a {tuple(a.shape)} b {tuple(b.shape)} (N, K multiples of 4 -- 8 for a pre-split b --, M > 0)")
+    lib = _lib.load()
+    ws = _workspace(tag, a, int(lib.locov_gemm_tn_workspace_bytes(M, N, K, 1)))
+    splits = ctypes.c_int(0)
+    with torch.cuda.device(a.device):
+        check(lib.locov_gemm_tn_partials(_ptr(a), a.stride(0), _ptr(b), b.stride(0), M, N, K, _ptr(a_scale_dev), float(b_scale),
+                                         int(b_is_split), _ptr(_overflow_word(a)) if a_scale_dev is not None else None, _ptr(ws),
+                                         ws.numel(), ctypes.byref(splits), _stream(a)), "locov_gemm_tn_partials")
+    return TnPartials(ws.data_ptr(), splits.value, N, K, 1, ws)
+
+
+def winograd_wgrad_partials(x: torch.Tensor, g: torch.Tensor, roi_major: bool = True, split: bool = False,
+                            v_split: Optional[torch.Tensor] = None, tag: str = "wino_wgrad_part") -> TnPartials:
+    x, g = _dev(x, "x"), _dev(g, "g")
+    M, Cin = x.shape
+    N = g.shape[1]
+    if g.shape[0] != M or M % 49 or M == 0 or Cin % 4 or N % 4:
+        raise ValueError("winograd_wgrad_partials: inconsistent shapes")
+    R = M // 49
+    if v_split is not None and not (split and Cin % 8 == 0 and v_split.is_cuda and v_split.device == x.device
+                                    and v_split.numel() * v_split.element_size() >= 121 * R * Cin * 4 and v_split.data_ptr() % 16 == 0):
+        raise ValueError("winograd_wgrad_partials: v_split needs the split arithmetic, Cin % 8 == 0 and the forward's workspace of the same x")
+    lib = _lib.load()
+    ws = _workspace(tag, x, int(lib.locov_winograd_wgrad_workspace_bytes(R, Cin, N)))
+    at, splits = ctypes.c_void_p(0), ctypes.c_int(0)
+    with torch.cuda.device(x.device):
+        check(lib.locov_winograd_wgrad_partials(None if v_split is not None else _ptr(x), _ptr(v_split), _ptr(g), R, Cin, N,
+                                                _lib.WINO_IN_ROI_MAJOR if roi_major else 0, int(bool(split)),
+                                                _ptr(_overflow_word(x)) if split else None, _ptr(ws), ws.numel(), ctypes.byref(at),
+                                                ctypes.byref(splits), _stream(x)), "locov_winograd_wgrad_partials")
+    return TnPartials(at.value, splits.value, N, Cin, 121, ws)
+
+
+def tn_reduce(jobs) -> None:
+    jobs = list(jobs)
+    if not jobs:
+        return
+    if len(jobs) > _lib.TN_REDUCE_MAX_JOBS:
+        tn_reduce(jobs[:_lib.TN_REDUCE_MAX_JOBS])
+        return tn_reduce(jobs[_lib.TN_REDUCE_MAX_JOBS:])
+    arr = (_lib.TnReduceJob * len(jobs))()
+    maps = {"plain": _lib.TN_MAP_PLAIN, "conv3x3": _lib.TN_MAP_CONV3X3, "wino": _lib.TN_MAP_WINO}
+    for j, (mapping, part, row_scale, out, *more) in zip(arr, jobs):
+        second = more[0] if more else None
+        cin = part.K // 9 if mapping == "conv3x3" else part.K
+        shape = (part.N, part.K) if mapping == "plain" else (part.N, cin, 3, 3)
+        if (tuple(out.shape) != shape or out.dtype != torch.float32 or not out.is_cuda or not out.is_contiguous()
+                or (mapping == "conv3x3" and part.K % 9) or (mapping == "wino") != (part.batch == 121)):
+            raise ValueError(f"tn_reduce: a {mapping} job of N={part.N} K={part.K} batch={part.batch} cannot write {tuple(out.shape)}")
+        if second is not None and (mapping != "wino" or second.N != part.N or second.K != 9 * part.K or second.batch != 1):
+            raise ValueError("tn_reduce: the added gradient must be the conv3x3 form of the same weight")
+        row_scale = _dev(row_scale, "row_scale") if row_scale is not None else None
+        j.partials, j.partials2 = part.ptr, second.ptr if second is not None else None
+        j.row_scale, j.out = (row_scale.data_ptr() if row_scale is not None else None), out.data_ptr()
+        j.ldo, j.stride_o = part.K, 0
+        j.N, j.K, j.splits, j.batch, j.map = part.N, part.K, part.splits, part.batch, maps[mapping]
+        j.splits2 = second.splits if second is not None else 0
+    ref = jobs[0][3]
+    with torch.cuda.device(ref.device):
+        check(_lib.load().locov_gemm_tn_reduce(arr, len(jobs), _stream(ref)), "locov_gemm_tn_reduce")
+
+
 def winograd_conv3x3_split_ex(x: torch.Tensor, U: SplitWeight, *, scale=None, shift=None, mask=None, relu: bool = False,
                               roi_major: bool = True, v_scale: Optional[float] = None,
                               amax_out: Optional[torch.Tensor] = None, out: Optional[torch.Tensor] = None) -> torch.Tensor:
diff --git a/locov_amd/res5_train.py b/locov_amd/res5_train.py
--- a/locov_amd/res5_train.py
+++ b/locov_amd/res5_train.py
@@ -299,10 +299,16 @@
         T = step._bwd_operands()
         slot = (lambda ref: ops.scale_slot(ref)) if sp else (lambda ref: None)
 
+        jobs = []
+
         def wgrad_1x1(g_, sg_, x_, s_):
-            if sp and g_.shape[1] % 4 == 0 and x_.shape[1] % 4 == 0 and g_.shape[0] > 0:
-                return ops.gemm_tn_split(g_, x_, s_, sg_, 16.0)
-            return ops.gemm_tn(g_, x_, s_)
+            if g_.shape[0] == 0:
+                return ops.gemm_tn(g_, x_, s_)
+            split_ = sp and g_.shape[1] % 4 == 0 and x_.shape[1] % 4 == 0
+            part = ops.gemm_tn_partials(g_, x_, sg_ if split_ else None, 16.0, tag=f"tn_part{len(jobs)}")
+            dw = torch.empty((part.N, part.K), dtype=torch.float32, device=step.device)
+            jobs.append(("plain", part, s_, dw))
+            return dw
 
         def dgrad_1x1(g_, sg_, conv, tag="t", amax_out=None, wt=None, **kw):
             if wt is None:
@@ -312,7 +318,7 @@
             y_ = ops.linear_ex(g_, wt, **kw)
             return y_, (ops.split_scale_from_amax(y_) if sp and amax_out is not None else None)
 
-        return sp, T, slot, wgrad_1x1, dgrad_1x1
+        return sp, T, slot, wgrad_1x1, dgrad_1x1, jobs
 
     @staticmethod
     def _backward_tail(ctx, g):
@@ -327,7 +333,7 @@
             step._carry = ("head", g1, None, g, None)
             return (g1,) + tuple(torch.zeros_like(w) if need else None for w, need in zip((blk.conv2.weight, blk.conv3.weight), need_w))
         g, sg = Res5BlockFn._take_carry(step, g, "tail")
-        sp, T, slot, wgrad_1x1, dgrad_1x1 = Res5BlockFn._helpers(ctx)
+        sp, T, slot, wgrad_1x1, dgrad_1x1, jobs = Res5BlockFn._helpers(ctx)
         y1, y2, _ = ctx.saved_tensors
         s2, s3 = stage.operands.fold(blk.conv2)[0], stage.operands.fold(blk.conv3)[0]
         c2 = blk.conv2
@@ -354,23 +360,18 @@
                 for t_ in (g1, g2, y1):
                     t_.record_stream(side)
             with torch.cuda.stream(side if on_side else main):
-                part = None
                 if need_w[0]:
+                    tag = f"wgrad3x3_part{len(parts)}"
                     if wino and c2.out_channels % 4 == 0 and not _NO_WINO_BWD:
-                        part = ops.winograd_wgrad(y1[sl], g2[sl], s2, roi_major=True, split=sp, v_split=step.wino_ws.get((bi, si)) if sp else None)
+                        parts.append(("wino", ops.winograd_wgrad_partials(y1[sl], g2[sl], roi_major=True, split=sp, tag=tag,
+                                                                          v_split=step.wino_ws.get((bi, si)) if sp else None)))
                     else:
                         colw = step.cols.get((bi, si))
                         if colw is None:
                             colw = ops.im2col3x3(y1[sl], seg.H, seg.W)
                         elif on_side:
                             colw.record_stream(side)
-                        if sp:
-                            part = ops.conv3x3_wgrad_unpack(ops.gemm_tn_split(g2[sl], colw, None, sg2, 16.0), s2)
-                        else:
-                            part = ops.conv3x3_wgrad_unpack(ops.gemm_tn(g2[sl], colw), s2)
-                    if on_side:
-                        part.record_stream(main)
-                    parts.append(part)
+                        parts.append(("conv3x3", ops.gemm_tn_partials(g2[sl], colw, sg2 if sp else None, 16.0, tag=tag)))
                 if _wino_ok(seg.H, seg.W, c2.out_channels, c2.in_channels) and not _NO_WINO_BWD:
                     uflip = flipped["uflip"]
                     if isinstance(uflip, ops.SplitWeight):
@@ -387,8 +388,18 @@
         if side is not None:
             main.wait_stream(side)
         if need_w[0]:
-            dw2 = parts[0]
-            for part in parts[1:]:
+            new_dw2 = lambda: torch.empty((c2.out_channels, c2.in_channels, 3, 3), dtype=torch.float32, device=step.device)
+            if sorted(k for k, _ in parts) == ["conv3x3", "wino"]:
+                dw2s = [new_dw2()]
+                by = dict(parts)
+                jobs.append(("wino", by["wino"], s2, dw2s[0], by["conv3x3"]))
+            else:
+                dw2s = [new_dw2() for _ in parts]
+                jobs.extend((kind, part, s2, dw) for (kind, part), dw in zip(parts, dw2s))
+        ops.tn_reduce(jobs)
+        if need_w[0]:
+            dw2 = dw2s[0]
+            for part in dw2s[1:]:
                 dw2 = dw2.add_(part)
             gw[0] = dw2
         step._carry = ("head", g1, sg1, g, sg)
@@ -414,7 +425,7 @@
                 return (gx,) + tuple(torch.zeros_like(w) if need else None for w, need in zip(weights, need_w))
             return tuple(None for _ in range(n_in)) + tuple(torch.zeros_like(w) if need else None for w, need in zip(weights, need_w))
         g1, sg1, g, sg = Res5BlockFn._take_carry(step, g1, "head")
-        sp, T, slot, wgrad_1x1, dgrad_1x1 = Res5BlockFn._helpers(ctx)
+        sp, T, slot, wgrad_1x1, dgrad_1x1, jobs = Res5BlockFn._helpers(ctx)
         x, _ = ctx.saved_tensors
         s1 = stage.operands.fold(blk.conv1)[0]
         if need_w[0]:
@@ -423,6 +434,7 @@
             ss = stage.operands.fold(blk.shortcut)[0]
             if need_w[1]:
                 gw[1] = wgrad_1x1(g, sg, x, ss).view_as(blk.shortcut.weight)
+        ops.tn_reduce(jobs)
         if not need_x:
             return tuple(None for _ in range(n_in)) + tuple(gw)
         mask = None if first else x
```
